# DTolm/VkResample

Measured on AMD Instinct MI355X. Metric: frames/s, 2048x1024->4096x2048 fp32 FFT upscale (R2C+zero-pad+C2R+sharpen), higher is better.
Workload: dtype f32; 1 GPU; 2048x1024->4096x2048 -u 2 -p 0, 1024 frames/step/GPU, ring of 8 resident planar fp32 frames/GPU; preset=config2, kernels=tuned, streams=3, device=AMD Radeon Graphics, wisdom=built-in only (private cache dir)

## Files before the change

vkresample_amd/csrc/fftup_info.hip:

```cpp
#include <hip/hip_runtime.h>

#include <cstdio>
#include <cstring>
#include <string>

#include "plan.hpp"

static thread_local std::string g_last_error;

int fail(int code, const std::string& msg)
{
    g_last_error = msg;
    return code;
}

static const char* device_label(const hipDeviceProp_t& prop) { return prop.name[0] ? prop.name : prop.gcnArchName; }

extern "C" {

int fftup_device_count(void)
{
    int n = 0;
    if (hipGetDeviceCount(&n) != hipSuccess) return 0;
    return n;
}

int fftup_device_name(int device, char* buf, size_t buflen)
{
    if (!buf || buflen == 0) return fail(FFTUP_E_INVALID_ARG, "null buffer");
    hipDeviceProp_t prop;
    if (device < 0 || device >= fftup_device_count()) return fail(FFTUP_E_NO_DEVICE, "bad device id");
    HIP_TRY(hipGetDeviceProperties(&prop, device));
    snprintf(buf, buflen, "%s", device_label(prop));
    return FFTUP_OK;
}

int fftup_device_pci_bus_id(int device, char* buf, size_t buflen)
{
    if (!buf || buflen < 16) return fail(FFTUP_E_INVALID_ARG, "buffer of at least 16 bytes needed");
    if (device < 0 || device >= fftup_device_count()) return fail(FFTUP_E_NO_DEVICE, "bad device id");
    HIP_TRY(hipDeviceGetPCIBusId(buf, (int)buflen, device));
    return FFTUP_OK;
}

int fftup_plan_describe(const fftup_plan* P, char* buf, size_t buflen)
{
    if (!P || !buf || !buflen) return fail(FFTUP_E_INVALID_ARG, "null argument");
    std::string s;
    using Family = fftup_plan::Family;
    const std::string half = P->half ? ", half storage" : "", tiles = std::to_string(P->TK);
    const std::string resampled = " (size-generic kernels, " + std::to_string(P->ncols) + " spectrum columns, LDS ping-pong, run-time radix lists, column tiles of " + tiles + ")" + half;
    const std::string rows_cols = ", rows " + std::to_string(P->W) + "->" + std::to_string(P->uW) + ", columns " + std::to_string(P->H) + "->" + std::to_string(P->uH);
    switch (P->family) {
    case Family::dct:
        s = std::string(P->down ? "downscale: dct: size-generic DCT-II / truncate / DCT-III kernels" : "dct: size-generic DCT-II / zero-pad / DCT-III kernels")
            + " (LDS ping-pong, run-time radix lists, column tiles of " + tiles + " column pairs)" + half;
        break;
    case Family::view: {
        char t[320];
        snprintf(t, sizeof t, "view%s: chirp-z resampling, rows %u->%u origin %.17g span %.17g (kmax %d, L=%u), columns %u->%u origin %.17g span %.17g (kmax %d, L=%u)",
                 P->mirror ? ", mirror (even reflection, period 2N)" : "", P->W, P->uW, P->vw.origin_x, P->vw.span_x, P->vx.kmax, P->vx.L, P->H, P->uH, P->vw.origin_y, P->vw.span_y, P->vy.kmax, P->vy.L);
        s = t + resampled;
        break;
    }
    case Family::odd:
        if (P->exact) s = "exact size: exact trigonometric resampling" + rows_cols + (P->align == FFTUP_ALIGN_CENTRE ? ", pixel centres aligned" : ", pixel 0 on pixel 0") + resampled;
        else s = std::string(P->down ? "downscale: " : "") + "odd sizes: exact trigonometric resampling" + rows_cols + resampled;
        break;
    case Family::down:
        s = "downscale: size-generic kernels, spectrum cropped to " + std::to_string(P->ncols) + " columns at the row stage (LDS ping-pong, "
            "run-time radix lists, column tiles of " + tiles + ")" + half;
        break;
    case Family::mixed_jit: s = "specialised at plan time: " + fftup_jit::describe(P->jit->choice); break;
    case Family::tuned:
        s = "ahead-of-time power-of-two kernels (radix 8, 8 points per thread; fused C2R+sharpen " + std::string(P->fused ? "on" : "off") + ")"
            + "; column kernel with digit-swap exchanges";
        break;
    case Family::mixed_aot:
        s = std::string("ahead-of-time mixed-radix kernels: ") + (P->mixed == 1 ? "row 15*8*16, col 9*10*12, fused 16*16*15" : "row 5*16*16, col 9*8*10, fused 16*16*10");
        break;
    case Family::cplx: s = "size-generic kernels, non-R2C path (full complex transforms)"; break;
    case Family::generic: case Family::f64:
        s = std::string("size-generic kernels (") + ((P->inplaceF || P->inplaceI || P->inplaceC) ? "in place in one LDS buffer" : "LDS ping-pong") + ", run-time radix lists"
            + (P->poly ? ", polyphase column pass)" : ")")
            + (P->dbl ? ", double" : "");
        break;
    }
    auto four = [&](const char* what, const fftup_plan::Four& f) {
        if (f.on) s += std::string("; ") + what + " in four steps " + std::to_string(f.n1) + "*" + std::to_string(f.n2) + " (tiles of " + std::to_string(f.tka) + " / " + std::to_string(f.tkb) + ")";
    };
    four("forward rows", P->fourF); four("inverse rows", P->fourI); four("forward columns", P->colF); four("inverse columns", P->colI);
    if (P->bz && P->family == Family::view) {
        if (P->bzW.L) s += "; forward rows bluestein L=" + std::to_string(P->bzW.L);
        if (P->bzH.L) s += "; forward columns bluestein L=" + std::to_string(P->bzH.L);
    }
    else if (P->bz) {
        auto axis = [&](const char* what, uint32_t n, uint32_t un, const BzPlan& f, const BzPlan& i) {
            if (!f.L && !i.L) return;
            s += std::string("; ") + what + " " + std::to_string(n) + "->" + std::to_string(un) + " bluestein L=" + (f.L ? std::to_string(f.L) : std::string("-")) + "/"
                 + (i.L ? std::to_string(i.L) : std::string("-"));
        };
        axis("rows", P->W, P->uW, P->bzW, P->bzUW);
        axis("columns", P->H, P->uH, P->bzH, P->bzUH);
        s += "; column tiles of " + std::to_string(P->TK);
    }
    if (P->u8out) s += "; fused 8-bit RGB store";
    snprintf(buf, buflen, "%s", s.c_str());
    return FFTUP_OK;
}

int fftup_plan_info(const fftup_plan* P, fftup_info* info)
{
    if (!P || !info) return fail(FFTUP_E_INVALID_ARG, "null argument");
    memset(info, 0, sizeof *info);
    info->out_width = P->uW;
    info->out_height = P->uH;
    info->num_kernels = P->fused ? 3 : 4;
    info->tuned = P->mixed == 3 ? 2 : ((P->tuned || P->mixed) ? 1 : 0);
    const double C = 3.0, W = P->W, H = P->H, uW = P->uW, uH = P->uH;
    const bool fused_u8 = fuse_u8(P);
    const double b_in = fused_u8 ? 1.0 : (double)P->esz;
    const double b_r = (double)P->esz, b_out = P->u8out ? 1.0 : b_r, b_c = (double)P->csz;
    const double in = C * W * H * b_in;
    const double S1 = C * P->ncols * H * b_c;
    const double S2 = C * P->ncols * uH * b_c;
    const double R = C * uW * uH * (P->cplx ? b_c : b_r);
    const double o = C * uW * uH * b_out;
    info->alg_bytes_per_frame = in + 2 * S1 + 2 * S2 + 2 * R + o;
    info->kernel_alg_bytes[0] = in + S1;
    info->kernel_alg_bytes[1] = S1 + S2;
    info->kernel_alg_bytes[2] = P->fused ? S2 + 2 * R + o : S2 + R;
    info->kernel_alg_bytes[3] = P->fused ? 0.0 : R + o;
    {
        const bool poly = (P->tuned || P->mixed) && P->U >= 2;
        const double S2w = poly ? S1 * (P->U - 1) : S2;
        const double halo = P->fused ? (double)(P->pairs_per_strip + 1) / P->pairs_per_strip : 1.0;
        info->kernel_min_bytes[0] = in + S1;
        info->kernel_min_bytes[1] = S1 + S2w;
        info->kernel_min_bytes[2] = P->fused ? S2 * halo + o : S2 + R;
        info->kernel_min_bytes[3] = P->fused ? 0.0 : R + o;
    }
    if (P->dct) {
        const double D1 = C * W * H * 4.0, D2 = C * W * uH * 4.0;
        info->alg_bytes_per_frame = in + 2 * D1 + 2 * D2 + 2 * R + o;
        const double k[FFTUP_NUM_KERNELS] = {in + D1, D1 + D2, D2 + R, R + o};
        for (int i = 0; i < FFTUP_NUM_KERNELS; i++) info->kernel_alg_bytes[i] = info->kernel_min_bytes[i] = k[i];
    }
    info->device_bytes = P->device_bytes;
    info->abi_version = FFTUP_ABI_VERSION;
    info->u8_store = P->u8out ? 1 : 0;
    snprintf(info->device_name, sizeof info->device_name, "%s", device_label(P->prop));
    const bool crop_rows = P->exact ? P->uW < P->W : P->down, crop_cols = P->exact ? P->uH < P->H : P->down;
    const bool is_dct = P->family == fftup_plan::Family::dct, is_cplx = P->family == fftup_plan::Family::cplx;
    snprintf(info->kernel_names[0], 64, is_dct ? "dct_row" : crop_rows ? "row_r2c_crop" : is_cplx ? "row_c2c" : "row_r2c");
    snprintf(info->kernel_names[1], 64, is_dct ? (P->down ? "dct_col_crop_idct" : "dct_col_pad_idct") : crop_cols ? "col_fwd_crop_inv" : "col_fwd_pad_inv");
    snprintf(info->kernel_names[2], 64, is_dct ? "idct_row" : P->fused ? "row_c2r_sharpen" : (is_cplx ? "row_c2c_inv" : "row_c2r"));
    snprintf(info->kernel_names[3], 64, P->fused ? "-" : "sharpen");
    if (P->family == fftup_plan::Family::odd)
        for (int i = 0; i < 3; i++) strncat(info->kernel_names[i], "_odd", 63 - strlen(info->kernel_names[i]));
    if (P->family == fftup_plan::Family::view) {
        snprintf(info->kernel_names[0], 64, P->mirror ? "row_r2c_mirror" : "row_r2c_odd");
        snprintf(info->kernel_names[1], 64, P->mirror ? "col_view_mirror" : "col_view");
        snprintf(info->kernel_names[2], 64, P->mirror ? "row_view_c2r_mirror" : "row_view_c2r");
    }
    const bool kbz[3] = {P->bzW.L != 0, P->bzH.L != 0 || P->bzUH.L != 0, P->bzUW.L != 0};
    for (int i = 0; i < (P->family == fftup_plan::Family::view ? 2 : 3); i++)
        if (kbz[i]) strncat(info->kernel_names[i], "_bz", 63 - strlen(info->kernel_names[i]));
    return FFTUP_OK;
}

const char* fftup_strerror(int code)
{
    switch (code) {
    case FFTUP_OK: return "success";
    case FFTUP_E_INVALID_ARG: return "invalid argument";
    case FFTUP_E_UNSUPPORTED_SIZE: return "unsupported size (not 2,3,5,7-smooth)";
    case FFTUP_E_UNSUPPORTED_PRECISION: return "unsupported precision";
    case FFTUP_E_NO_DEVICE: return "no usable HIP device";
    case FFTUP_E_HIP: return "HIP runtime error";
    case FFTUP_E_OUT_OF_MEMORY: return "out of device memory";
    case FFTUP_E_NO_INPUT: return "no input uploaded / nothing executed";
    case FFTUP_E_INCOMPLETE: return "incomplete (image not found)";
    case FFTUP_E_WOULD_BLOCK: return "the call would wait for the calling thread itself";
    case FFTUP_E_OVERFLOW: return "an internal buffer bound was exceeded";
    default: return "unknown error";
    }
}

const char* fftup_last_error(void) { return g_last_error.c_str(); }
const char* fftup_version(void) { return "fftup 0.7.0 (gfx950, ABI 2)"; }

}
```

vkresample_amd/csrc/fftup_launch.hip:

```cpp
#include <hip/hip_runtime.h>

#include <algorithm>
#include <cmath>
#include <cstdio>
#include <cstdlib>
#include <cstring>
#include <string>
#include <type_traits>
#include <vector>

#include "plan.hpp"
#include "kernels_generic.hpp"
#include "kernels_pow2.hpp"
#include "kernels_mixed.hpp"
#include "kernels_dswap.hpp"
#include "kernels_dct.hpp"
#include "kernels_downscale.hpp"
#include "kernels_bluestein.hpp"
#include "kernels_odd.hpp"
#include "kernels_view.hpp"
#include "kernels_mirror.hpp"
#include "kernels_view_tables.hpp"
#include "kernels_path.hpp"
#include "kernels_device_io.hpp"
#include "mirror_tables.hpp"

using namespace fftup;
using Family = fftup_plan::Family;

int kernels_generic_max_threads(bool dbl) { return dbl ? GenericMaxThreads<double2>::value : GenericMaxThreads<float2>::value; }
int kernels_aot_mixed_plan(uint32_t W, uint32_t H)
{
    if (W == MixedCfg1080::W && H == MixedCfg1080::H) return 1;
    if (W == MixedCfg720::W && H == MixedCfg720::H) return 2;
    return 0;
}
size_t kernels_tuned_col_lds(uint32_t H) { return sizeof(float2) * (size_t)lswz_size((int)H * TUNED_TK); }

struct ViewTables { int kmax; const float2 *pre, *post, *bhat; };
struct Frame { hipStream_t st; float2 *S1, *S2; void *R, *T4; const void* in; long in_row, in_plane; int kind; void* out;
               int ncols, NT; float upsq; ViewTables vx, vy; };
static Frame resolve(const fftup_plan* P, const FrameRun& r)
{
    const fftup_plan::Lane& l = P->lanes[r.lane];
    Frame f{l.stream, l.S1, l.S2, l.R, l.T4, P->in_planar[r.in_slot], (long)P->W, (long)P->in_plane_stride, P->in_kind[r.in_slot], r.out,
            P->ncols, P->NT, P->upsq, {P->vx.kmax, P->vx.pre, P->vx.post, P->vx.bhat}, {P->vy.kmax, P->vy.pre, P->vy.post, P->vy.bhat}};
    if (r.in) { f.in = r.in->in; f.in_row = r.in->in_row; f.in_plane = r.in->kind == 2 ? 0 : r.in->in_plane; f.kind = r.in->kind; }
    else if (f.kind == 2) { f.in = P->in_u8[r.in_slot]; f.in_row = 3l * P->W; f.in_plane = 0; }
    return f;
}
template <class Q> static void set_in(const Frame& f, Q& q) { q.in = f.in; q.in_row_stride = f.in_row; q.in_plane_stride = f.in_plane; }
static bool runs(Pass pass, Pass k) { return pass == Pass::all || pass == k; }

template <class... A> struct Kern { void (*fn)(A...); unsigned block; size_t lds; };
template <class... A> static Kern<A...> kern(void (*fn)(A...), int block, size_t lds) { return {fn, (unsigned)block, lds}; }
template <class T> struct type_c { using type = T; };
template <class... A> static void launch(const Kern<A...>& k, dim3 grid, hipStream_t st, const typename type_c<A>::type&... a)
{
    void* args[] = {const_cast<void*>((const void*)&a)...};
    (void)hipLaunchKernel((const void*)k.fn, grid, dim3(k.block), args, k.lds, st);
}
template <typename C> struct FourKerns { Kern<Row4Params<C>> a, b; };

template <int MAX = 8, class F> static auto with_tile(int tk, F&& f)
{
    if constexpr (MAX > 1) {
        if (tk == MAX) return f(std::integral_constant<int, MAX>{});
        return with_tile<MAX / 2>(tk, f);
    }
    else return f(std::integral_constant<int, 1>{});
}
template <class F> static auto with_flag(bool b, F&& f) { return b ? f(std::true_type{}) : f(std::false_type{}); }
template <class F> static auto with_mode(bool half, int kind, F&& f)
{
    if (kind == 2) return half ? f(std::integral_constant<int, IN_U8_F16>{}) : f(std::integral_constant<int, IN_U8_F32>{});
    return half ? f(std::integral_constant<int, IN_F16>{}) : f(std::integral_constant<int, IN_F32>{});
}
template <class F> static auto with_mixed_cfg(const fftup_plan* P, F&& f) { return P->mixed == 1 ? f(type_c<MixedCfg1080>{}) : f(type_c<MixedCfg720>{}); }

static Kern<RowR2CParams> generic_row_kernel(const fftup_plan* P, int kind)
{
    return with_mode(P->half, kind, [&](auto m) { return kern(k_row_r2c<m()>, P->thrW, P->ldsRowF); });
}
template <class F> static auto generic_c2r_kernel(const fftup_plan* P, F&& f)
{
    return with_flag(P->half, [&](auto h) {
        if (P->bzUW.L) return f(kern(k_row_c2r_bz<h()>, P->thrUW, P->ldsRowI), P->bzUW);
        return f(kern(k_row_c2r<h()>, P->thrUW, P->ldsRowI));
    });
}
template <typename C> static Kern<ColParamsT<C>> col_kernel(const fftup_plan* P)
{
    return with_tile(P->TK, [&](auto tk) {
        if (P->poly) return kern(k_col_poly<tk(), C>, P->thrCol, P->ldsCol);
        if constexpr (sizeof(scalar_t<C>) == 8) {
            if (P->inplaceC) return kern(k_col<tk(), C, true>, P->thrCol, P->ldsCol);
        }
        return kern(k_col<tk(), C, false>, P->thrCol, P->ldsCol);
    });
}
template <typename C, class F> static auto columns_kernel(const fftup_plan* P, F&& f)
{
    if constexpr (sizeof(scalar_t<C>) == 4) {
        if (P->bzH.L || P->bzUH.L) return with_tile(P->TK, [&](auto tk) { return f(kern(k_col_bz<tk()>, P->thrCol, P->ldsCol), P->bzH, P->bzUH); });
    }
    return f(col_kernel<C>(P));
}
static Kern<RowR2CParamsT<double2>> f64_row_kernel(const fftup_plan* P)
{
    return with_flag(P->inplaceF, [&](auto ip) { return kern(k_row_r2c<IN_F64, double2, ip()>, P->thrW, P->ldsRowF); });
}
static Kern<RowC2RParamsT<double2>> f64_c2r_kernel(const fftup_plan* P)
{
    return with_flag(P->inplaceI, [&](auto ip) { return kern(k_row_c2r<false, double2, ip()>, P->thrUW, P->ldsRowI); });
}
template <typename C> static Kern<RowR2CParamsT<C>> c2c_fwd_kernel(const fftup_plan* P, int kind)
{
    if constexpr (sizeof(scalar_t<C>) == 8) return kern(k_row_c2c_fwd<IN_F64, C, false>, P->thrW, P->ldsRowF);
    else return with_mode(P->half, kind, [&](auto m) {
        if (P->inplaceF) return kern(k_row_c2c_fwd<m(), C, true>, 1024, P->ldsRowF);
        return kern(k_row_c2c_fwd<m(), C, false>, P->thrW, P->ldsRowF);
    });
}
template <typename C> static Kern<RowC2RParamsT<C>> c2c_inv_kernel(const fftup_plan* P)
{
    if constexpr (sizeof(scalar_t<C>) == 8) return kern(k_row_c2c_inv<C, false, false>, P->thrUW, P->ldsRowI);
    else return with_flag(P->half, [&](auto h) {
        if (P->inplaceI) return kern(k_row_c2c_inv<C, h(), true>, 1024, P->ldsRowI);
        return kern(k_row_c2c_inv<C, h(), false>, P->thrUW, P->ldsRowI);
    });
}
template <typename C, int DIR, int MODE, int OUT> static FourKerns<C> four_kernels(const fftup_plan::Four& f)
{
    return {with_tile<16>(f.tka, [&](auto t) { return kern(k_row4_a<DIR, t(), MODE, C>, f.thrA, f.ldsA); }),
            with_tile<16>(f.tkb, [&](auto t) { return kern(k_row4_b<DIR, t(), OUT, C>, f.thrB, f.ldsB); })};
}
template <typename C> static FourKerns<C> four_fwd_kernels(const fftup_plan* P, int kind)
{
    if constexpr (sizeof(scalar_t<C>) == 8) return four_kernels<C, +1, IN_F64, OUT4_TILES>(P->fourF);
    else return with_mode(P->half, kind, [&](auto m) { return four_kernels<C, +1, m(), OUT4_TILES>(P->fourF); });
}
template <typename C> static FourKerns<C> four_inv_kernels(const fftup_plan* P)
{
    if constexpr (sizeof(scalar_t<C>) == 4) {
        if (P->half) return four_kernels<C, -1, IN4_TILES, OUT4_HALF>(P->fourI);
    }
    return four_kernels<C, -1, IN4_TILES, OUT4_DENSE>(P->fourI);
}
template <typename C> static FourKerns<C> four_col_kernels(const fftup_plan* P, bool inverse)
{
    return inverse ? four_kernels<C, -1, IN4_DENSE_SHIFT, OUT4_DENSE>(P->colI) : four_kernels<C, +1, IN4_DENSE, OUT4_DENSE>(P->colF);
}
static Kern<DctRowParams> dct_row_kernel(const fftup_plan* P, int kind)
{
    return with_mode(P->half, kind, [&](auto m) { return kern(k_dct_row<m()>, P->thrW, P->ldsRowF); });
}
static Kern<DctColParams> dct_col_kernel(const fftup_plan* P) { return with_tile(P->TK, [&](auto tk) { return kern(k_dct_col<tk()>, P->thrCol, P->ldsCol); }); }
static Kern<IdctRowParams> idct_row_kernel(const fftup_plan* P) { return with_flag(P->half, [&](auto h) { return kern(k_idct_row<h()>, P->thrUW, P->ldsRowI); }); }
static Kern<DownRowParams> crop_row_kernel(const fftup_plan* P, int kind)
{
    return with_flag(P->bzW.L != 0, [&](auto bz) { return with_mode(P->half, kind, [&](auto m) { return kern(k_row_r2c_crop<m(), bz()>, P->thrW, P->ldsRowF); }); });
}
static Kern<DownColParams> crop_col_kernel(const fftup_plan* P)
{
    return with_flag(P->bzH.L || P->bzUH.L, [&](auto bz) { return with_tile(P->TK, [&](auto tk) { return kern(k_col_crop<tk(), bz()>, P->thrCol, P->ldsCol); }); });
}
static Kern<OddRowParams> odd_row_kernel(const fftup_plan* P, int kind)
{
    return with_mode(P->half, kind, [&](auto m) { return kern(k_row_r2c_odd<m()>, P->thrW, P->ldsRowF); });
}
static Kern<OddColParams> odd_col_kernel(const fftup_plan* P) { return with_tile(P->TK, [&](auto tk) { return kern(k_col_odd<tk()>, P->thrCol, P->ldsCol); }); }
static Kern<OddC2RParams> odd_c2r_kernel(const fftup_plan* P) { return with_flag(P->half, [&](auto h) { return kern(k_row_c2r_odd<h()>, P->thrUW, P->ldsRowI); }); }
static bool resampling_rows(const fftup_plan* P) { return P->family == Family::generic && P->bzW.L != 0; }
static Kern<ViewColParams> view_col_kernel(const fftup_plan* P) { return with_tile(P->TK, [&](auto tk) { return kern(k_col_view<tk()>, P->thrCol, P->ldsCol); }); }
static Kern<ViewC2RParams> view_c2r_kernel(const fftup_plan* P) { return with_flag(P->half, [&](auto h) { return kern(k_row_view_c2r<h()>, P->thrUW, P->ldsRowI); }); }
static Kern<MirrorRowParams> mirror_row_kernel(const fftup_plan* P, int kind)
{
    return with_mode(P->half, kind, [&](auto m) { return kern(k_row_r2c_mirror<m()>, P->thrW, P->ldsRowF); });
}
static Kern<MirrorColParams> mirror_col_kernel(const fftup_plan* P) { return with_tile(P->TK, [&](auto tk) { return kern(k_col_view_mirror<tk()>, P->thrCol, P->ldsCol); }); }
static Kern<MirrorC2RParams> mirror_c2r_kernel(const fftup_plan* P) { return with_flag(P->half, [&](auto h) { return kern(k_row_view_c2r_mirror<h()>, P->thrUW, P->ldsRowI); }); }
static Kern<RowR2CTParams> tuned_row_kernel(const fftup_plan* P, int kind)
{
    return with_mode(P->half, kind, [&](auto m) {
        switch (P->W) {
        case 512: return kern(k_row_r2c_t<512, m(), TUNED_TK>, 512 / 8, 0);
        case 1024: return kern(k_row_r2c_t<1024, m(), TUNED_TK>, 1024 / 8, 0);
        default: return kern(k_row_r2c_t<2048, m(), TUNED_TK>, 2048 / 8, 0);
        }
    });
}
static Kern<ColTParams> tuned_col_kernel(const fftup_plan* P)
{
    switch (P->H) {
    case 256: return kern(k_col_v<TUNED_TK, 256>, 128, 8192);
    case 512: return kern(k_col_v<TUNED_TK, 512>, 256, 16384);
    default: return kern(k_col_v<TUNED_TK, 1024>, 512, 32768);
    }
}
static Kern<RowC2RTParams> tuned_c2r_kernel(const fftup_plan* P)
{
    return with_flag(P->half, [&](auto h) {
        switch (P->uW) {
        case 1024: return kern(k_row_c2r_t<1024, h(), TUNED_TK, true>, 1024 / 8, 0);
        case 2048: return kern(k_row_c2r_t<2048, h(), TUNED_TK, true>, 2048 / 8, 0);
        default: return kern(k_row_c2r_t<4096, h(), TUNED_TK, true>, 4096 / 8, 0);
        }
    });
}
static Kern<RowR2CTParams> mixed_row_kernel(const fftup_plan* P, int kind)
{
    return with_mixed_cfg(P, [&](auto c) {
        using CFG = typename decltype(c)::type;
        return with_mode(P->half, kind, [&](auto m) { return kern(k_row_r2c_m<CFG, m()>, CFG::ROW_T, 0); });
    });
}
static Kern<ColTParams> mixed_col_kernel(const fftup_plan* P)
{
    return with_mixed_cfg(P, [&](auto c) { using CFG = typename decltype(c)::type; return kern(k_col_m<CFG>, 4 * CFG::COL_TPC, P->ldsCol); });
}
static Kern<RowC2RParams> mixed_c2r_kernel(const fftup_plan* P)
{
    return with_mixed_cfg(P, [&](auto c) {
        using CT = typename decltype(c)::type::CT;
        return with_flag(P->half, [&](auto h) { return kern(k_row_c2r_ct<CT, h()>, CT::T, P->ldsRowI); });
    });
}
template <class PL> static Kern<FusedParams> fused_kernel_of(const fftup_plan* P)
{
    return with_flag(P->half, [&](auto h) {
        if (P->u8out) return kern(k_c2r_sharpen_g<PL, h(), TUNED_TK, 2, 4, true>, PL::T, FusedGLds<PL>::TOTAL);
        return kern(k_c2r_sharpen_g<PL, h(), TUNED_TK>, PL::T, FusedGLds<PL>::TOTAL);
    });
}
static Kern<FusedParams> fused_kernel(const fftup_plan* P)
{
    if (P->family == Family::mixed_aot) return with_mixed_cfg(P, [&](auto c) { return fused_kernel_of<typename decltype(c)::type::FUSED>(P); });
    switch (P->uW) {
    case 1024: return fused_kernel_of<FusedPlanPow2<1024>>(P);
    case 2048: return fused_kernel_of<FusedPlanPow2<2048>>(P);
    default: return fused_kernel_of<FusedPlanPow2<4096>>(P);
    }
}

struct AllowLds {
    hipError_t err = hipSuccess;
    template <class... A, class... X> void operator()(const Kern<A...>& k, const X&...)
    {
        if (err == hipSuccess) err = hipFuncSetAttribute((const void*)k.fn, hipFuncAttributeMaxDynamicSharedMemorySize, (int)k.lds);
    }
    template <typename C> void operator()(const FourKerns<C>& k) { (*this)(k.a); (*this)(k.b); }
};
template <typename C> static void allow_columns(const fftup_plan* P, AllowLds& allow)
{
    if (P->colF.on) { allow(four_col_kernels<C>(P, false)); allow(four_col_kernels<C>(P, true)); }
    else columns_kernel<C>(P, allow);
}
template <typename C> static void allow_cplx(const fftup_plan* P, AllowLds& allow)
{
    for (int kind : {1, 2}) { if (P->fourF.on) allow(four_fwd_kernels<C>(P, kind)); else allow(c2c_fwd_kernel<C>(P, kind)); }
    allow_columns<C>(P, allow);
    if (P->fourI.on) allow(four_inv_kernels<C>(P)); else allow(c2c_inv_kernel<C>(P));
}
int kernels_set_attributes(fftup_plan* P)
{
    AllowLds allow;
    switch (P->family) {
    case Family::generic:
        for (int kind : {1, 2}) { if (resampling_rows(P)) allow(odd_row_kernel(P, kind)); else allow(generic_row_kernel(P, kind)); }
        allow_columns<float2>(P, allow);
        generic_c2r_kernel(P, allow);
        break;
    case Family::f64: allow(f64_row_kernel(P)); allow_columns<double2>(P, allow); allow(f64_c2r_kernel(P)); break;
    case Family::cplx: if (P->dbl) allow_cplx<double2>(P, allow); else allow_cplx<float2>(P, allow); break;
    case Family::dct: for (int kind : {1, 2}) allow(dct_row_kernel(P, kind)); allow(dct_col_kernel(P)); allow(idct_row_kernel(P)); break;
    case Family::down: for (int kind : {1, 2}) allow(crop_row_kernel(P, kind)); allow(crop_col_kernel(P)); generic_c2r_kernel(P, allow); break;
    case Family::odd: for (int kind : {1, 2}) allow(odd_row_kernel(P, kind)); allow(odd_col_kernel(P)); allow(odd_c2r_kernel(P)); break;
    case Family::view:
        if (P->mirror) { for (int kind : {1, 2}) allow(mirror_row_kernel(P, kind)); allow(mirror_col_kernel(P)); allow(mirror_c2r_kernel(P)); }
        else { for (int kind : {1, 2}) allow(odd_row_kernel(P, kind)); allow(view_col_kernel(P)); allow(view_c2r_kernel(P)); }
        break;
    case Family::tuned: allow(tuned_col_kernel(P)); allow(fused_kernel(P)); break;
    case Family::mixed_aot: allow(mixed_col_kernel(P)); allow(mixed_c2r_kernel(P)); allow(fused_kernel(P)); break;
    case Family::mixed_jit:
        if (P->jit->choice.row_kind == 2) for (int kind : {1, 2}) allow(generic_row_kernel(P, kind));
        break;
    }
    if (allow.err != hipSuccess) return fail(FFTUP_E_HIP, std::string("hipFuncSetAttribute(hipFuncAttributeMaxDynamicSharedMemorySize): ") + hipGetErrorString(allow.err));
    return FFTUP_OK;
}

void launch_unpack_from(fftup_plan* P, const uint8_t* rgb, size_t row_stride_bytes, void* planes, hipStream_t st)
{
    dim3 grid((P->W + 255) / 256, P->H);
    if (P->dbl)
        hipLaunchKernelGGL(k_unpack_u8_f64, grid, dim3(256), 0, st, rgb, (long)row_stride_bytes, (double*)planes,
                           (int)P->W, (int)P->H, (long)P->in_plane_stride);
    else if (P->half)
        hipLaunchKernelGGL(k_unpack_u8<true>, grid, dim3(256), 0, st, rgb, (long)row_stride_bytes, planes,
                           (int)P->W, (int)P->H, (long)P->in_plane_stride);
    else
        hipLaunchKernelGGL(k_unpack_u8<false>, grid, dim3(256), 0, st, rgb, (long)row_stride_bytes, planes,
                           (int)P->W, (int)P->H, (long)P->in_plane_stride);
}
void launch_unpack(fftup_plan* P, uint32_t slot, hipStream_t st) { launch_unpack_from(P, P->in_u8[slot], (size_t)3 * P->W, P->in_planar[slot], st); }

void launch_pack(fftup_plan* P, uint32_t slot, uint8_t* dst, hipStream_t st)
{
    dim3 grid(P->dbl ? (P->uW + 255) / 256 : (P->uW + 1023) / 1024, P->uH);
    const int wrap = (P->cfg.flags & FFTUP_FLAG_U8_WRAP) ? 1 : 0;
    if (P->dbl) hipLaunchKernelGGL(k_pack_u8_f64, grid, dim3(256), 0, st, (const double*)P->out[slot], dst, (int)P->uW, (int)P->uH, wrap);
    else if (P->half) hipLaunchKernelGGL(k_pack_u8<true>, grid, dim3(256), 0, st, P->out[slot], dst, (int)P->uW, (int)P->uH, wrap);
    else hipLaunchKernelGGL(k_pack_u8<false>, grid, dim3(256), 0, st, P->out[slot], dst, (int)P->uW, (int)P->uH, wrap);
}

void launch_pack_to(fftup_plan* P, const void* planes, uint8_t* rgb, size_t row_stride_bytes, hipStream_t st)
{
    dim3 grid(P->dbl ? (P->uW + 255) / 256 : (P->uW + 1023) / 1024, P->uH);
    const int wrap = (P->cfg.flags & FFTUP_FLAG_U8_WRAP) ? 1 : 0;
    if (P->dbl) hipLaunchKernelGGL(k_pack_u8_f64_strided, grid, dim3(256), 0, st, (const double*)planes, rgb, (long)row_stride_bytes, (int)P->uW, (int)P->uH, wrap);
    else if (P->half) hipLaunchKernelGGL(k_pack_u8_strided<true>, grid, dim3(256), 0, st, planes, rgb, (long)row_stride_bytes, (int)P->uW, (int)P->uH, wrap);
    else hipLaunchKernelGGL(k_pack_u8_strided<false>, grid, dim3(256), 0, st, planes, rgb, (long)row_stride_bytes, (int)P->uW, (int)P->uH, wrap);
}

void launch_copy_rows(const void* src, size_t src_row, size_t src_plane, void* dst, size_t dst_row, size_t dst_plane,
                      size_t row_bytes, uint32_t rows, uint32_t planes, int gran, hipStream_t st)
{
    CopyRowsParams p{};
    p.src = (const uint8_t*)src; p.dst = (uint8_t*)dst; p.src_row = (long)src_row; p.src_plane = (long)src_plane;
    p.dst_row = (long)dst_row; p.dst_plane = (long)dst_plane; p.row_bytes = (long)row_bytes;
    const dim3 grid((unsigned)((row_bytes / 16 + 2 + 255) / 256), rows, planes);
    switch (gran) {
    case 8: hipLaunchKernelGGL(k_copy_rows<8>, grid, dim3(256), 0, st, p); break;
    case 4: hipLaunchKernelGGL(k_copy_rows<4>, grid, dim3(256), 0, st, p); break;
    case 2: hipLaunchKernelGGL(k_copy_rows<2>, grid, dim3(256), 0, st, p); break;
    default: hipLaunchKernelGGL(k_copy_rows<1>, grid, dim3(256), 0, st, p); break;
    }
}

static unsigned pass_planes()
{
    const char* e = fftup_jit::experiment("planes");
    return e ? (unsigned)std::max(1, std::min(3, atoi(e))) : 3u;
}

static unsigned fused_grid(const fftup_plan* P, int pairs_per_strip)
{
    const int ppp = (int)P->uH / 2;
    if (P->u8out) return (unsigned)(((ppp + pairs_per_strip - 1) / pairs_per_strip + 7) / 8 * 24);
    return (unsigned)((3 * ppp + pairs_per_strip - 1) / pairs_per_strip);
}
static FusedParams fused_params(const fftup_plan* P, const Frame& f)
{
    FusedParams p{};
    p.S1 = f.S1; p.odd_delta = (unsigned)(f.S2 - f.S1);
    if (P->U == 1) { p.S1 = f.S2; p.odd_delta = 0; }
    p.out = f.out; p.tw = P->twUW; p.uH = (int)P->uH; p.NT = P->NT;
    p.pairs_per_strip = P->pairs_per_strip; p.upsq = P->upsq; p.coef = P->coef;
    p.u8_wrap = (P->cfg.flags & FFTUP_FLAG_U8_WRAP) ? 1 : 0;
    return p;
}

static bool fast_sharpen_ok(const fftup_plan* P) { return !P->dbl && P->uW % 256 == 0 && P->uH % 16 == 0; }

static void launch_sharpen_fast(const fftup_plan* P, const Frame& f)
{
    SharpenTParams p{};
    p.R = f.R; p.out = f.out; p.uW = (int)P->uW; p.uH = (int)P->uH; p.upsq = f.upsq; p.coef = P->coef;
    dim3 grid(P->uW / 256, P->uH / 16, 3), block(64, 4);
    if (P->half) hipLaunchKernelGGL((k_sharpen_t<true, 4>), grid, block, 0, f.st, p);
    else hipLaunchKernelGGL((k_sharpen_t<false, 4>), grid, block, 0, f.st, p);
}

static void launch_sharpen(const fftup_plan* P, const Frame& f)
{
    if (fast_sharpen_ok(P)) { launch_sharpen_fast(P, f); return; }
    SharpenParams p{};
    p.R = f.R; p.out = f.out; p.uW = (int)P->uW; p.uH = (int)P->uH; p.upsq = f.upsq; p.coef = P->coef;
    dim3 grid((P->uW + 1023) / 1024, P->uH, 3), block(256);
    if (P->half) hipLaunchKernelGGL(k_sharpen<true>, grid, block, 0, f.st, p);
    else hipLaunchKernelGGL(k_sharpen<false>, grid, block, 0, f.st, p);
}

static int frame_status(hipError_t jit = hipSuccess)
{
    hipError_t e = hipGetLastError();
    if (e == hipSuccess) e = jit;
    if (e != hipSuccess) return fail(FFTUP_E_HIP, std::string("kernel launch: ") + hipGetErrorString(e));
    return FFTUP_OK;
}

template <class Rows, class Cols, class Inv>
static int launch_four_passes(const fftup_plan* P, const Frame& f, Pass pass, Rows rows, Cols cols, Inv inv)
{
    if (runs(pass, Pass::rows)) rows(P, f);
    if (runs(pass, Pass::columns)) cols(P, f);
    if (runs(pass, Pass::inverse)) inv(P, f);
    if (runs(pass, Pass::sharpen)) launch_sharpen(P, f);
    return frame_status();
}

static void dct_rows(const fftup_plan* P, const Frame& f)
{
    DctRowParams p{};
    p.S1 = (float*)f.S1; p.tw = P->twW; p.rot = P->rotW; p.plan = P->planW; p.W = (int)P->W; p.H = (int)P->H;
    set_in(f, p);
    launch(dct_row_kernel(P, f.kind), dim3(P->H / 2, 3), f.st, p);
}
static void dct_cols(const fftup_plan* P, const Frame& f)
{
    DctColParams p{};
    p.S1 = (const float*)f.S1; p.S2 = (float*)f.S2;
    p.twH = P->twH; p.twUH = P->twUH; p.rotH = P->rotH; p.rotUH = P->rotUH; p.planH = P->planH; p.planUH = P->planUH;
    p.W = (int)P->W; p.H = (int)P->H; p.uH = (int)P->uH; p.inv_norm = (float)(1.0 / (double)P->H);
    launch(dct_col_kernel(P), dim3((P->W / 2 + P->TK - 1) / P->TK, 3), f.st, p);
}
static void dct_inv(const fftup_plan* P, const Frame& f)
{
    IdctRowParams p{};
    p.S2 = (const float*)f.S2; p.R = f.R; p.tw = P->twUW; p.rot = P->rotUW; p.plan = P->planUW;
    p.W = (int)P->W; p.uW = (int)P->uW; p.uH = (int)P->uH;
    p.inv_norm = (float)(1.0 / ((double)P->W * (double)P->upsq));
    launch(idct_row_kernel(P), dim3(P->uH / 2, 3), f.st, p);
}

static void down_rows(const fftup_plan* P, const Frame& f)
{
    DownRowParams p{};
    p.S1 = f.S1; p.tw = P->twW; p.plan = P->planW; p.W = (int)P->W; p.H = (int)P->H;
    p.TK = P->TK; p.NT = P->NT; p.h = (int)P->uW / 2; p.bz = P->bzW;
    set_in(f, p);
    launch(crop_row_kernel(P, f.kind), dim3(P->H / 2, 3), f.st, p);
}
static void down_cols(const fftup_plan* P, const Frame& f)
{
// ... 45 lines not shown
    CztPlan z{};
    z.L = (int32_t)a.L; z.K = 2 * t.kmax + 1; z.M = (int32_t)M; z.plan = a.planL; z.tw = a.tw; z.pre = t.pre; z.post = t.post; z.bhat = t.bhat;
    return z;
}
static void view_cols(const fftup_plan* P, const Frame& f)
{
    ViewColParams p{};
    p.S1 = f.S1; p.S2 = f.S2; p.twH = P->twH; p.planH = P->planH;
    p.H = (int)P->H; p.uH = (int)P->uH; p.NT = f.NT; p.ncols = f.ncols; p.kmax = f.vy.kmax; p.bzH = P->bzH; p.z = czt_plan(P->vy, f.vy, P->uH);
    launch(view_col_kernel(P), dim3(f.NT, 3), f.st, p);
}
static void view_inv(const fftup_plan* P, const Frame& f)
{
    ViewC2RParams p{};
    p.S2 = f.S2; p.R = f.R; p.uW = (int)P->uW; p.uH = (int)P->uH;
    p.TK = P->TK; p.NT = f.NT; p.kmax = f.vx.kmax; p.z = czt_plan(P->vx, f.vx, P->uW);
    launch(view_c2r_kernel(P), dim3((P->uH + 1) / 2, 3), f.st, p);
}

static void mirror_rows(const fftup_plan* P, const Frame& f)
{
    MirrorRowParams p{};
    p.S1 = f.S1; p.tw = P->twW; p.plan = P->planW; p.W = (int)P->W; p.H = (int)P->H;
    p.TK = P->TK; p.NT = f.NT; p.ncols = f.ncols; p.bz = P->bzW;
    set_in(f, p);
    launch(mirror_row_kernel(P, f.kind), dim3((P->H + 1) / 2, 3), f.st, p);
}
static void mirror_cols(const fftup_plan* P, const Frame& f)
{
    MirrorColParams p{};
    p.S1 = f.S1; p.S2 = f.S2; p.twH = P->twH; p.planH = P->planH;
    p.H = (int)P->H; p.uH = (int)P->uH; p.NT = f.NT; p.ncols = f.ncols; p.kmax = f.vy.kmax; p.bzH = P->bzH; p.z = czt_plan(P->vy, f.vy, P->uH);
    p.rot = P->rotH;
    launch(mirror_col_kernel(P), dim3(f.NT, 3), f.st, p);
}
static void mirror_inv(const fftup_plan* P, const Frame& f)
{
    MirrorC2RParams p{};
    p.S2 = f.S2; p.R = f.R; p.W = (int)P->W; p.uW = (int)P->uW; p.uH = (int)P->uH;
    p.TK = P->TK; p.NT = f.NT; p.kmax = f.vx.kmax; p.z = czt_plan(P->vx, f.vx, P->uW); p.rot = P->rotW;
    launch(mirror_c2r_kernel(P), dim3((P->uH + 1) / 2, 3), f.st, p);
}

template <typename C> static void launch_four(const FourKerns<C>& k, const fftup_plan::Four& f, const Row4Params<C>& q, int rows, hipStream_t st)
{
    launch(k.a, dim3(rows, f.n2 / f.tka, 3), st, q);
    launch(k.b, dim3(rows, f.n1 / f.tkb, 3), st, q);
}
template <typename C> static void launch_columns(const fftup_plan* P, const Frame& f)
{
    using S = scalar_t<C>;
    if (!P->colF.on) {
        ColParamsT<C> p{};
        p.S1 = (const C*)f.S1; p.S2 = (C*)f.S2; p.twH = (const C*)P->twH; p.twUH = (const C*)P->twUH;
        p.planH = P->planH; p.planUH = P->planUH;
        p.W = (int)P->W; p.H = (int)P->H; p.uH = (int)P->uH; p.NT = P->NT; p.ncols = P->ncols; p.zly = P->zly; p.zry = P->zry;
        p.inv_norm = (S)(1.0 / (double)P->uH);
        columns_kernel<C>(P, [&](auto k, const auto&... z) { launch(k, dim3(P->NT, 3), f.st, p, z...); });
        return;
    }
    Row4Params<C> q{};
    const fftup_plan::Four &s = P->colF, &g = P->colI;
    q.spec = (const C*)f.S1; q.T = (C*)f.T4; q.R = f.S1;
    q.tw1 = (const C*)P->colFtw.tw1; q.tw2 = (const C*)P->colFtw.tw2; q.twN = (const C*)P->twH; q.plan1 = s.p1; q.plan2 = s.p2;
    q.N = (int)P->H; q.N1 = s.n1; q.N2 = s.n2; q.rows = P->ncols; q.W = (int)P->H; q.TK = 1; q.NT = P->ncols; q.inv_norm = (S)1;
    launch_four(four_col_kernels<C>(P, false), s, q, P->ncols, f.st);
    q.R = f.S2; q.tw1 = (const C*)P->colItw.tw1; q.tw2 = (const C*)P->colItw.tw2; q.twN = (const C*)P->twUH; q.plan1 = g.p1; q.plan2 = g.p2;
    q.N = (int)P->uH; q.N1 = g.n1; q.N2 = g.n2; q.zlx = P->zly; q.zrx = P->zry; q.inv_norm = (S)(1.0 / (double)P->uH);
    launch_four(four_col_kernels<C>(P, true), g, q, P->ncols, f.st);
}

static int launch_frame_f64(const fftup_plan* P, const Frame& f, Pass pass)
{
    if (runs(pass, Pass::rows)) {
        RowR2CParamsT<double2> p{};
        p.S1 = (double2*)f.S1; p.tw = (const double2*)P->twW; p.plan = P->planW; p.W = (int)P->W; p.H = (int)P->H;
        p.TK = P->TK; p.NT = P->NT;
        set_in(f, p);
        launch(f64_row_kernel(P), dim3(P->H / 2, 3), f.st, p);
    }
    if (runs(pass, Pass::columns)) launch_columns<double2>(P, f);
    if (runs(pass, Pass::inverse)) {
        RowC2RParamsT<double2> p{};
        p.S1 = (const double2*)f.S1; p.S2 = (const double2*)f.S2; p.R = f.R; p.tw = (const double2*)P->twUW; p.plan = P->planUW;
        p.W = (int)P->W; p.uW = (int)P->uW; p.uH = (int)P->uH; p.TK = P->TK; p.NT = P->NT; p.zlx = P->zlx; p.zrx = P->zrx;
        p.inv_norm = 1.0 / (double)P->uW; p.poly = P->poly;
        launch(f64_c2r_kernel(P), dim3(P->uH / 2, 3), f.st, p);
    }
    if (runs(pass, Pass::sharpen)) {
        SharpenParams p{};
        p.R = f.R; p.out = f.out; p.uW = (int)P->uW; p.uH = (int)P->uH; p.upsq = P->upsq; p.coef = P->coef;
        const dim3 sgrid((P->uW + 511) / 512, (P->uH + SHARPEN_F64_RPT - 1) / SHARPEN_F64_RPT, 3);
        const char* ex = fftup_jit::experiment("f64_exact_sharpen");
        if (ex && atoi(ex)) {
            if (P->uW % 2 == 0) hipLaunchKernelGGL((k_sharpen_f64<true, true>), sgrid, dim3(64, 4), 0, f.st, p);
            else hipLaunchKernelGGL((k_sharpen_f64<false, true>), sgrid, dim3(64, 4), 0, f.st, p);
        }
        else if (P->uW % 2 == 0) hipLaunchKernelGGL(k_sharpen_f64<true>, sgrid, dim3(64, 4), 0, f.st, p);
        else hipLaunchKernelGGL(k_sharpen_f64<false>, sgrid, dim3(64, 4), 0, f.st, p);
    }
    return frame_status();
}

template <typename C> static int launch_frame_cplx(const fftup_plan* P, const Frame& f, Pass pass)
{
    using S = scalar_t<C>;
    if (runs(pass, Pass::rows) && P->fourF.on) {
        Row4Params<C> q{};
        const fftup_plan::Four& s = P->fourF;
        q.T = (C*)f.T4; q.S1 = (C*)f.S1; q.tw1 = (const C*)P->fourFtw.tw1; q.tw2 = (const C*)P->fourFtw.tw2; q.twN = (const C*)P->twW;
        q.plan1 = s.p1; q.plan2 = s.p2; q.N = (int)P->W; q.N1 = s.n1; q.N2 = s.n2; q.rows = (int)P->H; q.W = (int)P->W; q.TK = P->TK; q.NT = P->NT;
        set_in(f, q);
        launch_four(four_fwd_kernels<C>(P, f.kind), s, q, (int)P->H, f.st);
    } else if (runs(pass, Pass::rows)) {
        RowR2CParamsT<C> p{};
        p.S1 = (C*)f.S1; p.tw = (const C*)P->twW; p.plan = P->planW; p.W = (int)P->W; p.H = (int)P->H;
        p.TK = P->TK; p.NT = P->NT;
        set_in(f, p);
        launch(c2c_fwd_kernel<C>(P, f.kind), dim3(P->H, 3), f.st, p);
    }
    if (runs(pass, Pass::columns)) launch_columns<C>(P, f);
    if (runs(pass, Pass::inverse)) {
        if (P->fourI.on) {
            Row4Params<C> q{};
            const fftup_plan::Four& s = P->fourI;
            q.spec = (const C*)f.S2; q.T = (C*)f.T4; q.R = f.R;
            q.tw1 = (const C*)P->fourItw.tw1; q.tw2 = (const C*)P->fourItw.tw2; q.twN = (const C*)P->twUW; q.plan1 = s.p1; q.plan2 = s.p2;
            q.N = (int)P->uW; q.N1 = s.n1; q.N2 = s.n2; q.rows = (int)P->uH; q.W = (int)P->W; q.TK = P->TK; q.NT = P->NT; q.zlx = P->zlx; q.zrx = P->zrx;
            q.inv_norm = (S)(1.0 / (double)P->uW);
            launch_four(four_inv_kernels<C>(P), s, q, (int)P->uH, f.st);
        } else {
            RowC2RParamsT<C> p{};
            p.S2 = (const C*)f.S2; p.R = f.R; p.tw = (const C*)P->twUW; p.plan = P->planUW;
            p.W = (int)P->W; p.uW = (int)P->uW; p.uH = (int)P->uH; p.TK = P->TK; p.NT = P->NT; p.zlx = P->zlx; p.zrx = P->zrx;
            p.inv_norm = (S)(1.0 / (double)P->uW);
            launch(c2c_inv_kernel<C>(P), dim3(P->uH, 3), f.st, p);
        }
    }
    if (runs(pass, Pass::sharpen)) {
        SharpenParams p{};
        p.R = f.R; p.out = f.out; p.uW = (int)P->uW; p.uH = (int)P->uH; p.upsq = P->upsq; p.coef = P->coef;
        const dim3 grid((P->uW + 255) / 256, P->uH, 3);
        bool done = false;
        if constexpr (sizeof(S) == 4) {
            if (P->half) { hipLaunchKernelGGL((k_sharpen_c<C, true>), grid, dim3(256), 0, f.st, p); done = true; }
        }
        if (!done) hipLaunchKernelGGL((k_sharpen_c<C>), grid, dim3(256), 0, f.st, p);
    }
    return frame_status();
}

static int launch_frame_tuned(const fftup_plan* P, const Frame& f, Pass pass)
{
    if (runs(pass, Pass::rows)) {
        RowR2CTParams p{};
        p.S1 = f.S1; p.tw = P->twW; p.H = (int)P->H; p.NT = P->NT;
        set_in(f, p);
        launch(tuned_row_kernel(P, f.kind), dim3(P->H / 2, pass_planes()), f.st, p);
    }
    if (runs(pass, Pass::columns)) {
        ColTParams p{};
        p.S1 = f.S1; p.S2 = f.S2; p.twH = P->twH; p.twUH = P->twUH; p.W = (int)P->W; p.NT = P->NT;
        p.zly = P->zly; p.zry = P->zry;
        launch(tuned_col_kernel(P), dim3(P->NT, pass_planes()), f.st, p);
    }
    if (runs(pass, Pass::inverse) && P->fused) {
        const FusedParams p = fused_params(P, f);
        launch(fused_kernel(P), dim3(fused_grid(P, p.pairs_per_strip)), f.st, p);
    } else if (runs(pass, Pass::inverse) || pass == Pass::presharpen_tap) {
        RowC2RTParams p{};
        p.S1 = f.S1; p.S2 = f.S2; p.R = f.R; p.tw = P->twUW; p.uH = (int)P->uH; p.NT = P->NT;
        launch(tuned_c2r_kernel(P), dim3(P->uH / 2, 3), f.st, p);
    }
    if (runs(pass, Pass::sharpen) && !P->fused) launch_sharpen_fast(P, f);
    return frame_status();
}

static int launch_frame_generic(const fftup_plan* P, const Frame& f, Pass pass)
{
    const bool jit = P->family == Family::mixed_jit, aot = P->family == Family::mixed_aot;
    hipError_t jerr = hipSuccess;
    auto keep_first = [&](hipError_t e) { if (jerr == hipSuccess) jerr = e; };
    if (runs(pass, Pass::rows)) {
        const dim3 grid(P->H / 2, 3);
        if (resampling_rows(P)) odd_rows(P, f);
        else if (aot || (jit && P->jit->choice.row_kind != 2)) {
            RowR2CTParams q{};
            q.S1 = f.S1; q.tw = P->twW; q.H = (int)P->H; q.NT = P->NT;
            set_in(f, q);
            if (aot) launch(mixed_row_kernel(P, f.kind), grid, f.st, q);
            else keep_first(fftup_jit::launch(P->jit->fn[f.kind == 2 ? fftup_jit::K_ROW_U8 : fftup_jit::K_ROW_PLANAR], grid, dim3(P->jit->choice.row_block), 0, f.st, q));
        } else {
            RowR2CParams p{};
            p.S1 = f.S1; p.tw = P->twW; p.plan = P->planW; p.W = (int)P->W; p.H = (int)P->H;
            p.TK = P->TK; p.NT = P->NT;
            set_in(f, p);
            launch(generic_row_kernel(P, f.kind), grid, f.st, p);
        }
    }
    if (runs(pass, Pass::columns) && (jit || aot)) {
        ColTParams q{};
        q.S1 = f.S1; q.S2 = f.S2; q.twH = P->twH; q.twUH = P->twUH; q.W = (int)P->W; q.NT = P->NT;
        q.zly = P->zly; q.zry = P->zry;
        if (jit) {
            const auto& ch = P->jit->choice;
            const dim3 jgrid(P->NT * (ch.col_kind >= 3 ? 4 / ch.col_cols : 1), 3);
            keep_first(fftup_jit::launch(P->jit->fn[fftup_jit::K_COL], jgrid, dim3(ch.col_block), P->ldsCol, f.st, q));
        }
        else launch(mixed_col_kernel(P), dim3(P->NT, 3), f.st, q);
    }
    else if (runs(pass, Pass::columns)) launch_columns<float2>(P, f);
    if (runs(pass, Pass::inverse) && P->fused) {
        const FusedParams fp = fused_params(P, f);
        const dim3 grid(fused_grid(P, fp.pairs_per_strip));
        if (jit) keep_first(fftup_jit::launch(P->jit->fn[fftup_jit::K_FUSED], grid, dim3(P->jit->choice.fused_t), P->jit->choice.fused_lds, f.st, fp));
        else launch(fused_kernel(P), grid, f.st, fp);
    } else if (runs(pass, Pass::inverse) || pass == Pass::presharpen_tap) {
        RowC2RParams p{};
        p.S1 = f.S1; p.S2 = f.S2; p.R = f.R; p.tw = P->twUW; p.plan = P->planUW; p.W = (int)P->W; p.uW = (int)P->uW;
        p.uH = (int)P->uH; p.TK = P->TK; p.NT = P->NT; p.zlx = P->zlx; p.zrx = P->zrx;
        p.inv_norm = 1.0f / (float)P->uW; p.poly = P->poly && !P->mixed;
        const dim3 grid(P->uH / 2, 3);
        if (jit) {
            if (P->U == 1) p.S1 = p.S2;
            keep_first(fftup_jit::launch(P->jit->fn[fftup_jit::K_C2R_CT], grid, dim3(P->jit->choice.ct_t), P->ldsRowI, f.st, p));
        }
        else if (aot) launch(mixed_c2r_kernel(P), grid, f.st, p);
        else generic_c2r_kernel(P, [&](auto k, const auto&... z) { launch(k, grid, f.st, p, z...); });
    }
    if (runs(pass, Pass::sharpen) && !P->fused) launch_sharpen(P, f);
    return frame_status(jerr);
}

static int launch_family(const fftup_plan* P, const Frame& f, Pass pass)
{
    switch (P->family) {
    case Family::cplx: return P->dbl ? launch_frame_cplx<double2>(P, f, pass) : launch_frame_cplx<float2>(P, f, pass);
    case Family::f64: return launch_frame_f64(P, f, pass);
    case Family::dct: return launch_four_passes(P, f, pass, dct_rows, dct_cols, dct_inv);
    case Family::down: return launch_four_passes(P, f, pass, down_rows, down_cols, down_inv);
    case Family::odd: return launch_four_passes(P, f, pass, odd_rows, odd_cols, odd_inv);
    case Family::view:
        if (P->mirror) return launch_four_passes(P, f, pass, mirror_rows, mirror_cols, mirror_inv);
        return launch_four_passes(P, f, pass, odd_rows, view_cols, view_inv);
    case Family::tuned: return launch_frame_tuned(P, f, pass);
    case Family::generic: case Family::mixed_aot: case Family::mixed_jit: break;
    }
    return launch_frame_generic(P, f, pass);
}
static Kern<ViewTabParams> view_tables_kernel(const fftup_plan* P)
{
    return kern(k_view_tables, VT_THREADS, sizeof(double2) * (size_t)lpad_size((int)std::max(P->vx.L, P->vy.L)));
}
int kernels_allow_view_tables(const fftup_plan* P)
{
    for (uint32_t L : {P->vx.L, P->vy.L}) {
        if (L > (uint32_t)VT_MAX_L) return fail(FFTUP_E_UNSUPPORTED_SIZE, "k_view_tables: convolution length above " + std::to_string(VT_MAX_L));
        const StagePlan sp = make_stage_plan(L);
        for (int s = 0; s < sp.nstages; s++)
            if (!stage_fits_inplace((int)L, sp.radix[s], VT_THREADS, VT_PT)) return fail(FFTUP_E_UNSUPPORTED_SIZE, "k_view_tables: a stage does not fit its registers");
    }
    AllowLds allow;
    allow(view_tables_kernel(P));
    if (allow.err != hipSuccess) return fail(FFTUP_E_HIP, std::string("hipFuncSetAttribute(hipFuncAttributeMaxDynamicSharedMemorySize): ") + hipGetErrorString(allow.err));
    return FFTUP_OK;
}
static void frame_view(fftup_plan* P, int lane, const fftup_view& v, const fftup_shift* shift, Frame& f)
{
    fftup_plan::ViewTabs& t = P->vtabs[lane];
    struct Ax { const fftup_plan::ViewAxis* a; uint32_t N, M; double o, sp; ViewTables* out; };
    const Ax ax[2] = {{&P->vx, P->W, P->uW, v.origin_x, v.span_x, &f.vx}, {&P->vy, P->H, P->uH, v.origin_y, v.span_y, &f.vy}};
    ViewTabParams p{};
    for (int i = 0; i < 2; i++) {
        const Ax& x = ax[i];
        ViewTabAxis& q = p.ax[i];
        q.n = (int32_t)(P->mirror ? 2 * x.N : x.N); q.M = (int32_t)x.M; q.L = (int32_t)x.a->L;
        q.kmax = P->mirror ? fftup_viewtab::mirror_kmax_of(x.N, x.M, x.sp) : fftup_viewtab::kmax_of(x.N, x.M, x.sp);
        q.chirp = t.span[i] != x.sp;
        const fftup_viewphase::Pair o = fftup_viewphase::origin_of(x.o, (double)q.n, P->mirror);
        q.o_hi = o.hi; q.o_lo = o.lo; q.span = x.sp; q.plan = x.a->planL; q.tw = P->vroots[i];
        q.origin = x.o; q.mirror = P->mirror ? 1 : 0; q.shift = shift ? (i ? &shift->dy : &shift->dx) : nullptr;
        q.pre = t.pre[i]; q.post = t.post[i]; q.bhat = t.bhat[i];
        t.span[i] = x.sp; t.kmax[i] = q.kmax;
        *x.out = {q.kmax, q.pre, q.post, q.bhat};
    }
    t.built = true;
    f.ncols = P->mirror ? fftup_viewtab::mirror_ncols(P->W, f.vx.kmax) : f.vx.kmax + 1;
    f.NT = (f.ncols + P->TK - 1) / P->TK;
    const float u = view_factor(v, P->uW, P->uH);
    f.upsq = const_via_percent_f((double)(u * u), P->half);
    const char* ex = fftup_jit::experiment("view_tables_time");
    const bool timed = ex && atoi(ex) != 0;
    if (timed) (void)hipEventRecord(P->ev0, f.st);
    launch(view_tables_kernel(P), dim3(2), f.st, p);
    if (timed) {
        float ms = 0;
        (void)hipEventRecord(P->ev1, f.st);
        if (hipEventSynchronize(P->ev1) == hipSuccess && hipEventElapsedTime(&ms, P->ev0, P->ev1) == hipSuccess)
            fprintf(stderr, "fftup: k_view_tables %.3f us (chirp tables rebuilt: x %d, y %d)\n", (double)ms * 1e3, p.ax[0].chirp, p.ax[1].chirp);
    }
}

int launch_frame(fftup_plan* P, const FrameRun& r)
{
    Frame f = resolve(P, r);
    const bool tap = r.pass == Pass::presharpen_tap;
    if (f.kind == 0 && !tap) return fail(FFTUP_E_NO_INPUT, "no input uploaded for this slot");
    if (r.view) {
        if (P->family != Family::view || (size_t)r.lane >= P->vtabs.size() || !P->vtabs[r.lane].pre[0]) return fail(FFTUP_E_INVALID_ARG, "a frame with a view of its own: not a view plan, or its lane has no tables");
        frame_view(P, r.lane, *r.view, r.shift, f);
    }
    const int rc = launch_family(P, f, r.pass);
    if (rc && r.view) P->vtabs[r.lane].span[0] = P->vtabs[r.lane].span[1] = 0;
    if (tap || runs(r.pass, Pass::inverse)) { P->last_lane = r.lane; P->R_valid = !(P->fused && !tap); }
    return rc;
}

int launch_shift_path(const fftup_shift* in, fftup_shift* out, uint32_t n, uint32_t mode, float sigma, float min_peak, hipStream_t st)
{
    const Kern<ShiftPathParams> k = kern(k_shift_path, SP_THREADS, shift_path_lds((int)n, fftup_shiftpath::radius_of((double)sigma)));
    AllowLds allow;
    allow(k);
    if (allow.err != hipSuccess) return fail(FFTUP_E_HIP, std::string("hipFuncSetAttribute(hipFuncAttributeMaxDynamicSharedMemorySize): ") + hipGetErrorString(allow.err));
    launch(k, dim3(1), st, ShiftPathParams{(const float*)in, (float*)out, (int32_t)n, mode, sigma, min_peak});
    const hipError_t e = hipGetLastError();
    if (e != hipSuccess) return fail(FFTUP_E_HIP, std::string("fftup_shift_path: kernel launch: ") + hipGetErrorString(e));
    return FFTUP_OK;
}

__global__ void __launch_bounds__(256) k_checksum(const uint32_t* __restrict__ w, size_t n, unsigned long long* sum)
{
    unsigned long long acc = 0;
    for (size_t i = (size_t)blockIdx.x * 256 + threadIdx.x; i < n; i += (size_t)gridDim.x * 256) acc += w[i];
#pragma unroll
    for (int o = 32; o > 0; o >>= 1) acc += __shfl_down(acc, o);
    if ((threadIdx.x & 63) == 0) atomicAdd(sum, acc);
}

void launch_checksum(fftup_plan* P, uint32_t slot, hipStream_t st)
{
    const size_t nbytes = (size_t)3 * P->uW * P->uH * (P->u8out ? 1 : P->esz), nwords = nbytes / 4;
    hipLaunchKernelGGL(k_checksum, dim3(1024), dim3(256), 0, st, (const uint32_t*)P->out[slot], nwords, (unsigned long long*)P->d_sum);
    if (nbytes & 3)
        hipLaunchKernelGGL(k_checksum_tail, dim3(1), dim3(64), 0, st, (const uint8_t*)P->out[slot] + 4 * nwords, (int)(nbytes & 3), (unsigned long long*)P->d_sum);
}

#ifdef FFTUP_PLANE_STAMPS
extern "C" __attribute__((visibility("default"))) int fftup_debug_plane_stamps(unsigned long long* out)
{
    return out && hipMemcpyFromSymbol(out, HIP_SYMBOL(fftup::g_plane_stamps), sizeof(unsigned long long) * 3 * 2048 * 3) != hipSuccess;
}
#endif
```

vkresample_amd/csrc/fftup_plan.hip:

```cpp
#include <hip/hip_runtime.h>

#include <algorithm>
#include <cmath>
#include <complex>
#include <cstdio>
#include <cstdlib>
#include <cstring>
#include <memory>
#include <string>
#include <vector>

#include "plan.hpp"
#include "mirror_tables.hpp"
#include "view_tables.hpp"

using namespace fftup;

int dev_alloc(fftup_plan* P, void** ptr, size_t bytes)
{
    hipError_t e = hipMalloc(ptr, bytes);
    if (e != hipSuccess) {
        *ptr = nullptr;
        return fail(FFTUP_E_OUT_OF_MEMORY, std::string("hipMalloc(") + std::to_string(bytes) + "): " + hipGetErrorString(e));
    }
// ... 40 lines not shown
static int make_bluestein(fftup_plan* P, BzPlan* z, uint32_t n, uint32_t L)
{
    std::vector<std::complex<double>> w(n), b(L, std::complex<double>(0.0, 0.0));
    for (uint64_t k = 0; k < n; k++) w[k] = std::polar(1.0, M_PI * (double)((k * k) % (2 * (uint64_t)n)) / (double)n);
    for (uint32_t k = 0; k < n; k++) {
        b[k] = std::conj(w[k]);
        if (k) b[L - k] = std::conj(w[k]);
    }
    host_fft(b);
    std::vector<float2> hc(n), hb(L);
    for (uint32_t k = 0; k < n; k++) hc[k] = make_float2((float)w[k].real(), (float)w[k].imag());
    for (uint32_t k = 0; k < L; k++) hb[k] = make_float2((float)(b[k].real() / (double)L), (float)(b[k].imag() / (double)L));
    float2 *dc = nullptr, *db = nullptr, *dt = nullptr;
    if (int rc = upload_table(P, &dc, hc)) return rc;
    if (int rc = upload_table(P, &db, hb)) return rc;
    if (int rc = make_twiddles(P, &dt, L)) return rc;
    z->L = (int32_t)L; z->plan = make_stage_plan(L); z->tw = dt; z->chirp = dc; z->bhat = db;
    return FFTUP_OK;
}

static int make_phases(fftup_plan* P, float2** dptr, uint32_t N, uint32_t M)
{
    *dptr = nullptr;
    if (N == M) return FFTUP_OK;
    const uint32_t n = std::min(N, M) / 2 + 1;
    const int64_t period = 2 * (int64_t)M * (int64_t)N;
    std::vector<float2> h(n);
    for (uint32_t k = 0; k < n; k++) {
        int64_t r = ((int64_t)k * ((int64_t)N - (int64_t)M)) % period;
        if (r > period / 2) r -= period;
        if (r < -period / 2) r += period;
        const double a = -M_PI * (double)r / ((double)M * (double)N);
        h[k] = make_float2((float)std::cos(a), (float)std::sin(a));
    }
    return upload_table(P, dptr, h);
}


static int view_apply(fftup_plan* P, const fftup_view& v, bool first)
{
    struct Ax { fftup_plan::ViewAxis* a; uint32_t N, M; double o, sp, sp_old; };
    const Ax ax[2] = {{&P->vx, P->W, P->uW, v.origin_x, v.span_x, P->vw.span_x}, {&P->vy, P->H, P->uH, v.origin_y, v.span_y, P->vw.span_y}};
    for (const Ax& x : ax) {
        fftup_viewtab::AxisTables t;
        const bool chirp = first || x.sp != x.sp_old;
        if (P->mirror) fftup_viewtab::make_mirror_axis(x.N, x.M, x.o, x.sp, x.a->L, t, chirp);
        else fftup_viewtab::make_axis(x.N, x.M, x.o, x.sp, x.a->L, t, chirp);
        x.a->kmax = t.kmax;
        HIP_TRY(hipMemcpy(x.a->pre, t.pre.data(), sizeof(float) * t.pre.size(), hipMemcpyHostToDevice));
        if (chirp) {
            HIP_TRY(hipMemcpy(x.a->post, t.post.data(), sizeof(float) * t.post.size(), hipMemcpyHostToDevice));
            HIP_TRY(hipMemcpy(x.a->bhat, t.bhat.data(), sizeof(float) * t.bhat.size(), hipMemcpyHostToDevice));
        }
    }
    P->vw = v;
    P->ncols = P->mirror ? fftup_viewtab::mirror_ncols(P->W, P->vx.kmax) : P->vx.kmax + 1;
    P->NT = (P->ncols + P->TK - 1) / P->TK;
    P->cfg.upscale = view_factor(v, P->uW, P->uH);
    P->upsq = const_via_percent_f((double)(P->cfg.upscale * P->cfg.upscale), P->half);
    return FFTUP_OK;
}


int view_frames_prepare(fftup_plan* P, int nl)
{
    if (P->vtabs.empty()) P->vtabs.resize(P->nlanes);
    const uint32_t len[4] = {P->W, P->H, P->uW, P->uH};
    const fftup_plan::ViewAxis* const axes[2] = {&P->vx, &P->vy};
    if (!P->vroots[0]) {
        if (int rc = kernels_allow_view_tables(P)) return rc;
        for (int i = 0; i < 2; i++) {
            float2* d = nullptr;
            if (int rc = upload_table(P, &d, roots<double2>(axes[i]->L))) return rc;
            P->vroots[i] = (double2*)d;
        }
    }
    for (int l = 0; l < nl; l++) {
        fftup_plan::ViewTabs& t = P->vtabs[l];
        for (int i = 0; i < 2 && !t.bhat[1]; i++) {
            if (int rc = dev_alloc(P, (void**)&t.pre[i], sizeof(float2) * (2 * (size_t)(P->mirror ? len[i] : len[i] / 2) + 1))) return rc;
            if (int rc = dev_alloc(P, (void**)&t.post[i], sizeof(float2) * len[2 + i])) return rc;
            if (int rc = dev_alloc(P, (void**)&t.bhat[i], sizeof(float2) * axes[i]->L)) return rc;
        }
    }
    return FFTUP_OK;
}


static void tune_fused(fftup_plan* P);
static bool jit_tune_enabled()
{
    const char* e = fftup_jit::experiment("jit_tune");
    return e && atoi(e) != 0;
}

static int open_device(fftup_plan* P)
{
    HIP_TRY(hipSetDevice(P->device));
    HIP_TRY(hipGetDeviceProperties(&P->prop, P->device));
    HIP_TRY(hipStreamCreateWithFlags(&P->stream, hipStreamNonBlocking));
    HIP_TRY(hipEventCreate(&P->ev0));
    HIP_TRY(hipEventCreate(&P->ev1));
    return FFTUP_OK;
}

static fftup_jit::Module* specialise(const fftup_plan* P, const DeviceFacts& dev)
{
    int DD = 1;
    const int D = plan_jit_factor(*P, &DD);
    fftup_jit::Choice ch;
    if (!D || !fftup_jit::choose((int)P->W, (int)P->H, D, P->half, stage_radices(P->planUW), ch, wisdom_device_key(*P, dev), true, DD)) return nullptr;
    ch.u8out = (P->cfg.flags & FFTUP_FLAG_FUSE_U8_STORE) != 0;
    std::string jerr;
    fftup_jit::Module* m = fftup_jit::load(ch, dev.arch, jerr);
    if (!m && getenv("FFTUP_JIT_VERBOSE")) fprintf(stderr, "fftup: run-time specialisation failed, size-generic kernels in use: %s\n", jerr.c_str());
    return m;
}

static int make_tables(fftup_plan* P)
{
    const uint32_t len[4] = {P->W, P->H, P->uW, P->uH};
    float2** const tw[4] = {&P->twW, &P->twH, &P->twUW, &P->twUH};
    for (int i = 0; i < 4; i++)
        if (int rc = make_twiddles(P, tw[i], len[i])) return rc;
    const std::pair<const fftup_plan::Four*, fftup_plan::FourTables*> fours[4] = {{&P->fourF, &P->fourFtw}, {&P->fourI, &P->fourItw}, {&P->colF, &P->colFtw}, {&P->colI, &P->colItw}};
    for (auto& f : fours) {
        if (!f.first->on) continue;
        if (int rc = make_twiddles(P, &f.second->tw1, (uint32_t)f.first->n1)) return rc;
        if (int rc = make_twiddles(P, &f.second->tw2, (uint32_t)f.first->n2)) return rc;
    }
    BzPlan* const bz[4] = {&P->bzW, &P->bzH, &P->bzUW, &P->bzUH};
    for (int i = 0; i < 4; i++)
        if (P->bzL[i])
            if (int rc = make_bluestein(P, bz[i], len[i], P->bzL[i])) return rc;
    if (P->exact && P->align == FFTUP_ALIGN_CENTRE) {
        if (int rc = make_phases(P, &P->phW, P->W, P->uW)) return rc;
        if (int rc = make_phases(P, &P->phH, P->H, P->uH)) return rc;
    }
    if (P->view) {
        fftup_plan::ViewAxis* const axes[2] = {&P->vx, &P->vy};
        for (int i = 0; i < 2; i++) {
            fftup_plan::ViewAxis& a = *axes[i];
            a.L = P->viewL[i]; a.planL = make_stage_plan(a.L);
            if (int rc = make_twiddles(P, &a.tw, a.L)) return rc;
            if (int rc = dev_alloc(P, (void**)&a.pre, sizeof(float2) * (2 * (size_t)(P->mirror ? len[i] : len[i] / 2) + 1))) return rc;
            if (int rc = dev_alloc(P, (void**)&a.post, sizeof(float2) * len[2 + i])) return rc;
            if (int rc = dev_alloc(P, (void**)&a.bhat, sizeof(float2) * a.L)) return rc;
        }
    }
    if (P->mirror) {
        if (int rc = make_rotations(P, &P->rotW, P->W)) return rc;
        if (int rc = make_rotations(P, &P->rotH, P->H)) return rc;
    }
    if (P->dct) {
        float2** const rot[4] = {&P->rotW, &P->rotH, &P->rotUW, &P->rotUH};
        for (int i = 0; i < 4; i++)
            if (int rc = make_rotations(P, rot[i], len[i])) return rc;
    }
    return FFTUP_OK;
}

static int alloc_spectra(fftup_plan* P, float2** s1, float2** s2)
{
    const size_t s1_elems = (size_t)3 * P->NT * P->H * P->TK;
    if ((P->tuned || P->mixed) && P->U >= 2) {
        int r = dev_alloc(P, (void**)s1, P->csz * (size_t)P->U * s1_elems);
        *s2 = r ? nullptr : *s1 + s1_elems;
        return r;
    }
    int r = dev_alloc(P, (void**)s1, P->csz * s1_elems);
    return r ? r : dev_alloc(P, (void**)s2, P->csz * 3 * (size_t)P->NT * P->uH * P->TK);
}

static int make_buffers(fftup_plan* P)
{
    const size_t esz = P->esz, out_pixels = (size_t)3 * P->uW * P->uH;
    P->in_plane_stride = (size_t)(P->W + 2) * P->H;
    P->in_planar.assign(P->ring, nullptr);
    P->in_u8.assign(P->ring, nullptr);
    P->in_kind.assign(P->ring, 0);
    P->out.assign(P->ring, nullptr);
    for (uint32_t s = 0; s < P->ring; s++) {
        if (int rc = dev_alloc(P, &P->in_planar[s], 3 * P->in_plane_stride * esz)) return rc;
        if (int rc = dev_alloc(P, (void**)&P->in_u8[s], (size_t)3 * P->W * P->H)) return rc;
        if (int rc = dev_alloc(P, &P->out[s], out_pixels * (P->u8out ? 1 : esz) + 8)) return rc;
    }
    P->r_bytes = out_pixels * (P->cplx ? (P->half ? 4 : P->csz) : esz);
    if (!P->u8out)
        if (int rc = dev_alloc(P, (void**)&P->out_u8, out_pixels + 8)) return rc;
    return FFTUP_OK;
}

static int make_lanes(fftup_plan* P)
{
    P->nlanes = lane_count();
    P->lanes.resize(P->nlanes);
    const size_t t4_bytes = P->csz * 3 * std::max(std::max(P->fourF.on ? (size_t)P->W * P->H : 0, P->fourI.on ? (size_t)P->uW * P->uH : 0),
                                                  P->colI.on ? (size_t)P->ncols * P->uH : 0);
    for (int l = 0; l < P->nlanes; l++) {
        fftup_plan::Lane& lane = P->lanes[l];
        if (l == 0) lane.stream = P->stream;
        else HIP_TRY(hipStreamCreateWithFlags(&lane.stream, hipStreamNonBlocking));
        HIP_TRY(hipEventCreateWithFlags(&lane.done, hipEventDisableTiming));
        if (int rc = alloc_spectra(P, &lane.S1, &lane.S2)) return rc;
        if (!P->fused)
            if (int rc = dev_alloc(P, &lane.R, P->r_bytes)) return rc;
        if (t4_bytes)
            if (int rc = dev_alloc(P, &lane.T4, t4_bytes)) return rc;
    }
    return FFTUP_OK;
}

struct PlanDestroyer { void operator()(fftup_plan* P) const { fftup_plan_destroy(P); } };

static int plan_create(fftup_plan** out, const PlanRequest& rq)
{
    if (!out || !rq.cfg) return fail(FFTUP_E_INVALID_ARG, "null argument");
    *out = nullptr;
    PlanGeometry G;
    if (int rc = plan_check(rq, G)) return rc;
    const int ndev = fftup_device_count();
    if (ndev <= 0) return fail(FFTUP_E_NO_DEVICE, "no HIP device available (this library has no CPU path)");
    if (G.cfg.device < 0 || G.cfg.device >= ndev) return fail(FFTUP_E_NO_DEVICE, "device id out of range");

    std::unique_ptr<fftup_plan, PlanDestroyer> owner(new fftup_plan());
    fftup_plan* const P = owner.get();
    static_cast<PlanGeometry&>(*P) = G;
    P->device = G.cfg.device;
    if (int rc = open_device(P)) return rc;
    const DeviceFacts dev = device_facts(P->prop);
    if (int rc = plan_geometry_columns(*P, dev)) return rc;
    P->jit = specialise(P, dev);
    if (int rc = plan_geometry_finish(*P, dev, P->jit ? &P->jit->choice : nullptr)) return rc;
    if (int rc = make_tables(P)) return rc;
    if (int rc = make_buffers(P)) return rc;
    if (int rc = make_lanes(P)) return rc;
    if (rq.view)
        if (int rc = view_apply(P, *rq.view, true)) return rc;
    if (int rc = kernels_set_attributes(P)) return rc;
    if (P->mixed == 3 && ((P->cfg.flags & FFTUP_FLAG_TUNE_PLAN) || jit_tune_enabled())) tune_fused(P);
    png_geometry(P);
    *out = owner.release();
    return FFTUP_OK;
}

extern "C" {

int fftup_plan_create(fftup_plan** out, const fftup_config* cfg) { return plan_create(out, {cfg, nullptr, 0, nullptr}); }

int fftup_plan_create_size(fftup_plan** out, const fftup_config* cfg, uint32_t out_width, uint32_t out_height, uint32_t align)
{
    const uint32_t size[2] = {out_width, out_height};
    return plan_create(out, {cfg, size, align, nullptr});
}

int fftup_plan_create_view(fftup_plan** out, const fftup_config* cfg, uint32_t out_width, uint32_t out_height, const fftup_view* view)
{
    if (out) *out = nullptr;
    if (!out || !cfg || !view) return fail(FFTUP_E_INVALID_ARG, "null argument");
    const uint32_t size[2] = {out_width, out_height};
    return plan_create(out, {cfg, size, FFTUP_ALIGN_CORNER, view});
}

int fftup_plan_set_view(fftup_plan* P, const fftup_view* view)
{
    if (!P || !view) return fail(FFTUP_E_INVALID_ARG, "null argument");
    if (!P->view) return fail(FFTUP_E_INVALID_ARG, "fftup_plan_set_view: not a view plan (fftup_plan_create_view makes one)");
    if (int rc = check_view("fftup_plan_set_view", view, P->uW, P->uH)) return rc;
    HIP_TRY(hipSetDevice(P->device));
    for (auto& lane : P->lanes) HIP_TRY(hipStreamSynchronize(lane.stream));
    return view_apply(P, *view, false);
}


int fftup_jit_check(uint32_t width, uint32_t height, float upscale, uint32_t precision, const char* arch, char* desc, size_t desclen)
{
    if (desc && desclen) desc[0] = 0;
    if (precision != 0 && precision != 2) return fail(FFTUP_E_UNSUPPORTED_PRECISION, "run-time specialised plans exist for -p 0 and -p 2");
    if (width < 2 || height < 2 || (width & 1) || (height & 1) || width > 65536 || height > 65536 || !is_smooth(width) || !is_smooth(height))
        return fail(FFTUP_E_UNSUPPORTED_SIZE, "sizes must be even and factor into 2,3,5,7");
    fftup_jit::Choice ch;
    if (!(upscale >= 1.0f && upscale <= 8.0f)) return fail(FFTUP_E_INVALID_ARG, "upscale out of range");
    const uint32_t uW = scaled_length(upscale, width), uH = scaled_length(upscale, height);
    int DD = 1, zly = 0, zry = 0;
    column_guard(upscale, uH, &zly, &zry);
    const int D = (uW & 1) || (uH & 1) || !is_smooth(uW) || !is_smooth(uH) || uW > 8192 ? 0 : jit_factor(upscale, width, height, uW, uH, zly, zry, &DD);
    if (!D || !fftup_jit::choose((int)width, (int)height, D, precision == 2, stage_radices(make_stage_plan(uW)), ch, "", true, DD))
        return fail(FFTUP_E_UNSUPPORTED_SIZE, "no specialised factorization for this size: the size-generic kernels run it");
    if (desc && desclen) snprintf(desc, desclen, "%s", fftup_jit::describe(ch).c_str());
    if (arch && !*arch) return FFTUP_OK;
    fftup_jit::Binary bin[2];
    std::string err;
    if (!fftup_jit::compile_both(ch, arch ? arch : "gfx950", bin, err)) return fail(FFTUP_E_HIP, err);
    return FFTUP_OK;
}

void fftup_plan_destroy(fftup_plan* P)
{
    if (!P) return;
    (void)hipSetDevice(P->device);
    if (P->stream) (void)hipStreamSynchronize(P->stream);
    for (size_t l = 0; l < P->lanes.size(); l++) {
        if (l && P->lanes[l].stream) { (void)hipStreamSynchronize(P->lanes[l].stream); (void)hipStreamDestroy(P->lanes[l].stream); }
        if (P->lanes[l].done) (void)hipEventDestroy(P->lanes[l].done);
    }
    for (auto& qs : P->q) {
        if (qs.done) (void)hipEventDestroy(qs.done);
        if (qs.png.copied) (void)hipEventDestroy(qs.png.copied);
        if (qs.png.meta_host) (void)hipHostFree(qs.png.meta_host);
        if (qs.png.parts_host) (void)hipHostFree(qs.png.parts_host);
    }
    if (P->png_copy) (void)hipStreamDestroy(P->png_copy);
    if (P->dio.start) (void)hipEventDestroy(P->dio.start);
    for (void* p : P->allocs) (void)hipFree(p);
    delete P->jit;
    if (P->ev0) (void)hipEventDestroy(P->ev0);
    if (P->ev1) (void)hipEventDestroy(P->ev1);
    if (P->stream) (void)hipStreamDestroy(P->stream);
    delete P;
}


}
static void tune_fused(fftup_plan* P)
{
    const DeviceFacts dev = device_facts(P->prop);
    const std::string& arch = dev.arch;
    const fftup_jit::Choice base = P->jit->choice;
    const std::string key = fftup_jit::fused_key(base, wisdom_device_key(*P, dev));
    std::string known;
    if (fftup_jit::experiment("jit_fused") || fftup_jit::wisdom_lookup(key, known)) return;
    const std::vector<int> kinds = P->in_kind;
    const int executed = P->executed;
    for (auto& k : P->in_kind) if (!k) k = 1;
    const uint32_t frames = 4 * (uint32_t)std::max(1, std::min(P->nlanes, (int)P->ring));
    auto time_plan = [&]() -> double {
        double best = 1e30, ms = 0;
        for (int rep = 0; rep < 3; rep++) {
            if (execute_ring_impl(P, frames, 0, &ms, nullptr, 1) != FFTUP_OK) return 1e30;
            if (rep > 0) best = std::min(best, ms / frames);
        }
        return best;
    };
    const double t_base = time_plan();
    if (t_base >= 1e30) {
        P->in_kind = kinds;
        P->executed = executed;
        return;
    }
    double t_best = t_base;
    fftup_jit::Module* const original = P->jit;
    fftup_jit::Module* best = nullptr;
    auto use = [&](fftup_jit::Module* m) { P->jit = m; P->pairs_per_strip = strip_length(*P, dev, m->choice.fused_t); };
    std::vector<fftup_jit::Choice> cands;
    {
        fftup_jit::Choice d;
        if (fftup_jit::choose(base.W, base.H, base.D, base.half, stage_radices(P->planUW), d, "", false, base.DD) &&
            fftup_jit::fused_value(d) != fftup_jit::fused_value(base)) {
            d.u8out = base.u8out;
            cands.push_back(d);
        }
// ... 27 lines not shown
```

vkresample_amd/csrc/kernels_dswap.hpp:

```cpp
#pragma once
#include "kernels_pow2.hpp"

namespace fftup {
__device__ __forceinline__ float2 cmul_tw_s(float2 z, float2 w)
{
    typedef float cf2 __attribute__((ext_vector_type(2)));
    const cf2 zv = {z.x, z.y}, wv = {w.x, w.y};
    cf2 t, r;
    asm("v_pk_mul_f32 %0, %1, %2 op_sel:[1,1] op_sel_hi:[1,0] neg_lo:[1,0]" : "=v"(t) : "v"(zv), "s"(wv));
    asm("v_pk_fma_f32 %0, %1, %2, %3 op_sel_hi:[0,1,1]" : "=v"(r) : "v"(zv), "s"(wv), "v"(t));
    return make_float2(r.x, r.y);
}

__device__ __forceinline__ void lane_transpose_hi3(float2 (&v)[8])
{
#define FFTUP_SWAP8(OP, A0, B0, A1, B1, A2, B2, A3, B3)                                                                         \
    asm volatile("s_nop 1\n\t" OP " %0, %1\n\t" OP " %2, %3\n\t" OP " %4, %5\n\t" OP " %6, %7\n\t" OP " %8, %9\n\t" OP         \
                 " %10, %11\n\t" OP " %12, %13\n\t" OP " %14, %15"                                                             \
                 : "+v"(v[A0].x), "+v"(v[B0].x), "+v"(v[A0].y), "+v"(v[B0].y), "+v"(v[A1].x), "+v"(v[B1].x), "+v"(v[A1].y),     \
                   "+v"(v[B1].y), "+v"(v[A2].x), "+v"(v[B2].x), "+v"(v[A2].y), "+v"(v[B2].y), "+v"(v[A3].x), "+v"(v[B3].x),     \
                   "+v"(v[A3].y), "+v"(v[B3].y))
    FFTUP_SWAP8("v_permlane32_swap_b32", 0, 4, 1, 5, 2, 6, 3, 7);
    FFTUP_SWAP8("v_permlane16_swap_b32", 0, 2, 1, 3, 4, 6, 5, 7);
#undef FFTUP_SWAP8
    float t0, t1, t2, t3, t4, t5, t6, t7;
    asm volatile(
        "s_nop 1\n\t"
        "v_mov_b32_dpp %16, %0 row_ror:8 row_mask:0xf bank_mask:0xf\n\t"
        "v_mov_b32_dpp %17, %2 row_ror:8 row_mask:0xf bank_mask:0xf\n\t"
        "v_mov_b32_dpp %18, %4 row_ror:8 row_mask:0xf bank_mask:0xf\n\t"
        "v_mov_b32_dpp %19, %6 row_ror:8 row_mask:0xf bank_mask:0xf\n\t"
        "v_mov_b32_dpp %20, %8 row_ror:8 row_mask:0xf bank_mask:0xf\n\t"
        "v_mov_b32_dpp %21, %10 row_ror:8 row_mask:0xf bank_mask:0xf\n\t"
        "v_mov_b32_dpp %22, %12 row_ror:8 row_mask:0xf bank_mask:0xf\n\t"
        "v_mov_b32_dpp %23, %14 row_ror:8 row_mask:0xf bank_mask:0xf\n\t"
        "v_mov_b32_dpp %0, %1 row_ror:8 row_mask:0xf bank_mask:0xc\n\t"
        "v_mov_b32_dpp %2, %3 row_ror:8 row_mask:0xf bank_mask:0xc\n\t"
        "v_mov_b32_dpp %4, %5 row_ror:8 row_mask:0xf bank_mask:0xc\n\t"
        "v_mov_b32_dpp %6, %7 row_ror:8 row_mask:0xf bank_mask:0xc\n\t"
        "v_mov_b32_dpp %8, %9 row_ror:8 row_mask:0xf bank_mask:0xc\n\t"
        "v_mov_b32_dpp %10, %11 row_ror:8 row_mask:0xf bank_mask:0xc\n\t"
        "v_mov_b32_dpp %12, %13 row_ror:8 row_mask:0xf bank_mask:0xc\n\t"
        "v_mov_b32_dpp %14, %15 row_ror:8 row_mask:0xf bank_mask:0xc\n\t"
        "v_mov_b32_dpp %1, %16 quad_perm:[0,1,2,3] row_mask:0xf bank_mask:0x3\n\t"
        "v_mov_b32_dpp %3, %17 quad_perm:[0,1,2,3] row_mask:0xf bank_mask:0x3\n\t"
        "v_mov_b32_dpp %5, %18 quad_perm:[0,1,2,3] row_mask:0xf bank_mask:0x3\n\t"
        "v_mov_b32_dpp %7, %19 quad_perm:[0,1,2,3] row_mask:0xf bank_mask:0x3\n\t"
        "v_mov_b32_dpp %9, %20 quad_perm:[0,1,2,3] row_mask:0xf bank_mask:0x3\n\t"
        "v_mov_b32_dpp %11, %21 quad_perm:[0,1,2,3] row_mask:0xf bank_mask:0x3\n\t"
        "v_mov_b32_dpp %13, %22 quad_perm:[0,1,2,3] row_mask:0xf bank_mask:0x3\n\t"
        "v_mov_b32_dpp %15, %23 quad_perm:[0,1,2,3] row_mask:0xf bank_mask:0x3"
        : "+v"(v[0].x), "+v"(v[1].x), "+v"(v[0].y), "+v"(v[1].y), "+v"(v[2].x), "+v"(v[3].x), "+v"(v[2].y), "+v"(v[3].y),
          "+v"(v[4].x), "+v"(v[5].x), "+v"(v[4].y), "+v"(v[5].y), "+v"(v[6].x), "+v"(v[7].x), "+v"(v[6].y), "+v"(v[7].y),
          "=&v"(t0), "=&v"(t1), "=&v"(t2), "=&v"(t3), "=&v"(t4), "=&v"(t5), "=&v"(t6), "=&v"(t7));
}

__device__ __forceinline__ void lane_swap_bit2(float2 (&v)[8])
{
    float t0, t1, t2, t3, t4, t5, t6, t7;
    asm volatile(
        "s_nop 1\n\t"
        "v_mov_b32 %16, %0\n\tv_mov_b32 %17, %2\n\tv_mov_b32 %18, %4\n\tv_mov_b32 %19, %6\n\t"
        "v_mov_b32 %20, %8\n\tv_mov_b32 %21, %10\n\tv_mov_b32 %22, %12\n\tv_mov_b32 %23, %14\n\t"
        "v_mov_b32_dpp %0, %1 row_shr:4 row_mask:0xf bank_mask:0xa\n\t"
        "v_mov_b32_dpp %2, %3 row_shr:4 row_mask:0xf bank_mask:0xa\n\t"
        "v_mov_b32_dpp %4, %5 row_shr:4 row_mask:0xf bank_mask:0xa\n\t"
        "v_mov_b32_dpp %6, %7 row_shr:4 row_mask:0xf bank_mask:0xa\n\t"
        "v_mov_b32_dpp %8, %9 row_shr:4 row_mask:0xf bank_mask:0xa\n\t"
        "v_mov_b32_dpp %10, %11 row_shr:4 row_mask:0xf bank_mask:0xa\n\t"
        "v_mov_b32_dpp %12, %13 row_shr:4 row_mask:0xf bank_mask:0xa\n\t"
        "v_mov_b32_dpp %14, %15 row_shr:4 row_mask:0xf bank_mask:0xa\n\t"
        "v_mov_b32_dpp %1, %16 row_shl:4 row_mask:0xf bank_mask:0x5\n\t"
        "v_mov_b32_dpp %3, %17 row_shl:4 row_mask:0xf bank_mask:0x5\n\t"
        "v_mov_b32_dpp %5, %18 row_shl:4 row_mask:0xf bank_mask:0x5\n\t"
        "v_mov_b32_dpp %7, %19 row_shl:4 row_mask:0xf bank_mask:0x5\n\t"
        "v_mov_b32_dpp %9, %20 row_shl:4 row_mask:0xf bank_mask:0x5\n\t"
        "v_mov_b32_dpp %11, %21 row_shl:4 row_mask:0xf bank_mask:0x5\n\t"
        "v_mov_b32_dpp %13, %22 row_shl:4 row_mask:0xf bank_mask:0x5\n\t"
        "v_mov_b32_dpp %15, %23 row_shl:4 row_mask:0xf bank_mask:0x5"
        : "+v"(v[0].x), "+v"(v[4].x), "+v"(v[0].y), "+v"(v[4].y), "+v"(v[1].x), "+v"(v[5].x), "+v"(v[1].y), "+v"(v[5].y),
          "+v"(v[2].x), "+v"(v[6].x), "+v"(v[2].y), "+v"(v[6].y), "+v"(v[3].x), "+v"(v[7].x), "+v"(v[3].y), "+v"(v[7].y),
          "=&v"(t0), "=&v"(t1), "=&v"(t2), "=&v"(t3), "=&v"(t4), "=&v"(t5), "=&v"(t6), "=&v"(t7));
}
__device__ __forceinline__ void wave_exchange(float2 (&v)[8], unsigned zbase, unsigned w, unsigned l)
{
    const unsigned aw = zbase + 8u * (w * 64u + l);
#pragma unroll
    for (int k = 0; k < 8; k++) { lds_f2raw r = {v[k].x, v[k].y}; *(lds_f2*)(size_t)(aw + 4096u * k) = r; }
    __syncthreads();
    const unsigned ar = zbase + 8u * (w * 512u + l);
#pragma unroll
    for (int m = 0; m < 8; m++) { const lds_f2raw r = *(const lds_f2*)(size_t)(ar + 512u * m); v[m] = make_float2(r.x, r.y); }
#pragma unroll
    for (int i = 0; i < 8; i += 2) asm volatile("" : "+v"(v[i].x), "+v"(v[i].y), "+v"(v[i + 1].x), "+v"(v[i + 1].y));
}

template <int WV, bool FWD>
__device__ __forceinline__ void wave_exchange_q(float2 (&v)[8], unsigned zbase, unsigned w, unsigned l)
{
    const unsigned a_k0 = zbase + 8u * (w * 64u + l);
    const unsigned a_m = zbase + 8u * (w * 512u + l);
#pragma unroll
    for (int k = 0; k < 8; k++) { lds_f2raw r = {v[k].x, v[k].y}; *(lds_f2*)(size_t)((FWD ? a_k0 + 512u * WV * k : a_m + 512u * k)) = r; }
    __syncthreads();
#pragma unroll
    for (int m = 0; m < 8; m++) { const lds_f2raw r = *(const lds_f2*)(size_t)((FWD ? a_m + 512u * m : a_k0 + 512u * WV * m)); v[m] = make_float2(r.x, r.y); }
#pragma unroll
    for (int i = 0; i < 8; i += 2) asm volatile("" : "+v"(v[i].x), "+v"(v[i].y), "+v"(v[i + 1].x), "+v"(v[i + 1].y));
}
template <int WV, int DIR> __device__ __forceinline__ void bfly_groups(float2 (&v)[8])
{
    if constexpr (WV == 8) bfly8_pk<DIR>(v);
    else if constexpr (WV == 4) {
#pragma unroll
        for (int b = 0; b < 2; b++) {
            pk2 a0 = {v[4 * b].x, v[4 * b].y}, a1 = {v[4 * b + 1].x, v[4 * b + 1].y}, a2 = {v[4 * b + 2].x, v[4 * b + 2].y}, a3 = {v[4 * b + 3].x, v[4 * b + 3].y};
            bfly4_pk<DIR>(a0, a1, a2, a3);
            v[4 * b] = make_float2(a0.x, a0.y); v[4 * b + 1] = make_float2(a1.x, a1.y);
            v[4 * b + 2] = make_float2(a2.x, a2.y); v[4 * b + 3] = make_float2(a3.x, a3.y);
        }
    } else {
#pragma unroll
        for (int b = 0; b < 4; b++) {
            const pk2 a = {v[2 * b].x, v[2 * b].y}, c = {v[2 * b + 1].x, v[2 * b + 1].y};
            const pk2 s0 = pk_add(a, c), s1 = pk_sub(a, c);
            v[2 * b] = make_float2(s0.x, s0.y); v[2 * b + 1] = make_float2(s1.x, s1.y);
        }
    }
}

template <int TK, int H = 1024>
__global__ void __launch_bounds__(H / 2, kColWaves) k_col_v(ColTParams p)
{
    static_assert(TK == 4, "four columns of H/8 threads: lane bits 0-1 = column, bits 2-5 and the wave = pp");
    static_assert(H == 1024 || H == 512 || H == 256, "8, 4 or 2 waves");
    constexpr int WV = H / 128, Q = 8 / WV, T = 64 * WV;
    extern __shared__ __attribute__((aligned(128))) char smem[];
    const unsigned zbase = lds_addr(smem);
    const int tid = threadIdx.x;
    const unsigned w = (unsigned)tid >> 6, l = (unsigned)tid & 63u;
    const int col = tid & 3, pp = tid >> 2;
    const int tile = blockIdx.x, c = blockIdx.y;
    const bool valid = tile * TK + col <= p.W / 2;
    const float2* src = p.S1 + ((long)c * p.NT + tile) * H * TK;
    const int wu = __builtin_amdgcn_readfirstlane((int)w);
    const int s1 = (int)(l >> 3), lb2 = (int)((l >> 2) & 1u), hh = (int)(l >> 2);
    const int kk = Q * wu + s1 / WV + 8 * (s1 % WV);
    const int kt = kk + 32 * WV * lb2;
    float2 v[8];
    stamp_begin(1, c);
#pragma unroll
    for (int i = 0; i < 8; i++) v[i] = valid ? src[tid + T * i] : make_float2(0.f, 0.f);
    float2 ta[Q][WV - 1];
#pragma unroll
    for (int b = 0; b < Q; b++)
#pragma unroll
        for (int m = 1; m < WV; m++) ta[b][m - 1] = p.twH[(16 * m * (Q * wu + b)) & (H - 1)];
    const float2 tb = p.twH[2 * kk], tc = p.twH[kt];
    const float2 tph = twid<-1>(p.twUH[kt]);
    bfly8_pk<+1>(v);
    if constexpr (WV == 8) wave_exchange(v, zbase, w, l);
    else wave_exchange_q<WV, true>(v, zbase, w, l);
#pragma unroll
    for (int b = 0; b < Q; b++)
#pragma unroll
        for (int m = 1; m < WV; m++) v[WV * b + m] = cmul_tw_s(v[WV * b + m], ta[b][m - 1]);
    bfly_groups<WV, +1>(v);
    lane_transpose_hi3(v);
    twiddle_powers<8>(v, tb);
    bfly8_pk<+1>(v);
    lane_swap_bit2(v);
    {
        v[4] = cmul_tw(v[4], tc);
        v[5] = cmul_tw(v[5], cmul_tw(tc, rot16<1>()));
        v[6] = cmul_tw(v[6], cmul_tw(tc, rot16<2>()));
        v[7] = cmul_tw(v[7], cmul_tw(tc, rot16<3>()));
#pragma unroll
        for (int r = 0; r < 4; r++) {
            const pk2 a = {v[r].x, v[r].y}, b = {v[r + 4].x, v[r + 4].y};
            const pk2 s0 = pk_add(a, b), s1_ = pk_sub(a, b);
            v[r] = make_float2(s0.x, s0.y); v[r + 4] = make_float2(s1_.x, s1_.y);
        }
    }
    {
        const float2 t1 = cmul_tw(tph, twid<-1>(rot32<1>())), t2 = cmul_tw(tph, twid<-1>(rot32<2>())), t3 = cmul_tw(tph, twid<-1>(rot32<3>()));
        const float2 tt[4] = {tph, t1, t2, t3};
#pragma unroll
        for (int r = 0; r < 4; r++) {
            v[r] = cmul_tw(v[r], tt[r]);
            const float2 u = cmul_tw(v[r + 4], tt[r]);
            const pk2 iu = pk_muli<1>(pk2{u.x, u.y});
            v[r + 4] = make_float2(iu.x, iu.y);
        }
    }
#pragma unroll
    for (int r = 0; r < 4; r++) {
        const pk2 a = {v[r].x, v[r].y}, b = {v[r + 4].x, v[r + 4].y};
        const pk2 s0 = pk_add(a, b), s1_ = pk_sub(a, b);
        v[r] = make_float2(s0.x, s0.y); v[r + 4] = make_float2(s1_.x, s1_.y);
    }
    lane_swap_bit2(v);
    {
        const float2 e = twid<-1>(rot16<1>());
        const float2 base = lb2 ? e : make_float2(1.f, 0.f);
        twiddle_powers<8>(v, base);
    }
    bfly8_pk<-1>(v);
    lane_transpose_hi3(v);
    {
        const float2 w1 = twid<-1>(p.twH[8 * hh]);
        if constexpr (WV == 8) twiddle_powers<8>(v, w1);
        else {
#pragma unroll
            for (int b = 0; b < Q; b++) twiddle_powers<WV>(&v[WV * b], w1);
        }
    }
    bfly_groups<WV, -1>(v);
    __syncthreads();
    if constexpr (WV == 8) wave_exchange(v, zbase, w, l);
    else wave_exchange_q<WV, false>(v, zbase, w, l);
    twiddle_powers<8>(v, twid<-1>(p.twH[pp]));
    bfly8_pk<-1>(v);
    float2* dst = p.S2 + ((long)c * p.NT + tile) * H * TK;
    constexpr float inv = 1.0f / (float)H;
    if (valid) {
#pragma unroll
        for (int i = 0; i < 8; i++) spec_store8(dst + tid + T * i, cscale(v[i], inv));
    }
    stamp_end(1, c);
}


}
```

vkresample_amd/csrc/kernels_pow2.hpp:

```cpp
#pragma once
#include <hip/hip_fp16.h>
#include <hip/hip_runtime.h>

#include <type_traits>

#include "fft_engine.hpp"
#include "kernels_generic.hpp"

namespace fftup {

constexpr int kColWaves = 8;

constexpr int ilog2c(int n) { return n <= 1 ? 0 : 1 + ilog2c(n / 2); }
constexpr int stage_radix(int N, int Ns, int RMAX = 8) { return (N / Ns >= RMAX) ? RMAX : (N / Ns); }

__device__ __forceinline__ int lswz(int i) { return i ^ ((i >> 3) & 15); }
__host__ __device__ constexpr int lswz_size(int n) { return (n + 15) & ~15; }
template <int TK> __device__ __forceinline__ int lidx(int idx, int col) { return lswz(idx * TK + col); }
constexpr int lswz_c(int i) { return i ^ ((i >> 3) & 15); }
typedef float lds_f2raw __attribute__((ext_vector_type(2)));
typedef __attribute__((address_space(3))) lds_f2raw lds_f2;
__device__ __forceinline__ unsigned lds_addr(const void* p) { return (unsigned)(unsigned long)(const __attribute__((address_space(3))) char*)p; }
__device__ __forceinline__ void lds_put(unsigned a0, int C, float2 v)
{
// ... 131 lines not shown
template <int SGN> __device__ __forceinline__ pk2 pk_muli(pk2 b)
{
    pk2 r;
    if constexpr (SGN > 0) asm("v_pk_add_f32 %0, 0, %1 op_sel:[0,1] op_sel_hi:[1,0] neg_lo:[0,1]" : "=v"(r) : "v"(b));
    else asm("v_pk_add_f32 %0, 0, %1 op_sel:[0,1] op_sel_hi:[1,0] neg_hi:[0,1]" : "=v"(r) : "v"(b));
    return r;
}
template <int DIR> __device__ __forceinline__ void bfly16_pk(float2* v)
{
    pk2 y[4][4];
#pragma unroll
    for (int n2 = 0; n2 < 4; n2++) {
#pragma unroll
        for (int n1 = 0; n1 < 4; n1++) y[n2][n1] = pk2{v[4 * n1 + n2].x, v[4 * n1 + n2].y};
        bfly4_pk<DIR>(y[n2][0], y[n2][1], y[n2][2], y[n2][3]);
    }
    y[1][1] = pk_rot16<DIR, 1>(y[1][1]); y[1][2] = pk_rot16<DIR, 2>(y[1][2]); y[1][3] = pk_rot16<DIR, 3>(y[1][3]);
    y[2][1] = pk_rot16<DIR, 2>(y[2][1]); y[2][2] = pk_muli<DIR>(y[2][2]);      y[2][3] = pk_rot16<DIR, 6>(y[2][3]);
    y[3][1] = pk_rot16<DIR, 3>(y[3][1]); y[3][2] = pk_rot16<DIR, 6>(y[3][2]); y[3][3] = pk_rot16<DIR, 9>(y[3][3]);
#pragma unroll
    for (int k1 = 0; k1 < 4; k1++) {
        bfly4_pk<DIR>(y[0][k1], y[1][k1], y[2][k1], y[3][k1]);
        v[k1] = make_float2(y[0][k1].x, y[0][k1].y); v[k1 + 4] = make_float2(y[1][k1].x, y[1][k1].y);
        v[k1 + 8] = make_float2(y[2][k1].x, y[2][k1].y); v[k1 + 12] = make_float2(y[3][k1].x, y[3][k1].y);
    }
}
template <int R, int DIR> __device__ __forceinline__ void bfly_reg(float2* v)
{
    if constexpr (R == 8) bfly8_pk<DIR>(v);
    else if constexpr (R == 16) bfly16_pk<DIR>(v);
    else if constexpr (R == 2 || R == 3 || R == 4 || R == 5 || R == 9 || R == 10 || R == 12 || R == 15) {
        pk2 z[R];
#pragma unroll
        for (int m = 0; m < R; m++) z[m] = pk2{v[m].x, v[m].y};
        bfly<R, DIR>(z);
#pragma unroll
        for (int m = 0; m < R; m++) v[m] = make_float2(z[m].x, z[m].y);
    } else bfly<R, DIR>(v);
}

template <int R> __device__ __forceinline__ void twiddle_powers(float2* v, float2 w1)
{
    if constexpr (R == 2) {
        v[1] = cmul_tw(v[1], w1);
    } else if constexpr (R == 4) {
        float2 w2 = cmul_tw(w1, w1), w3 = cmul_tw(w2, w1);
        v[1] = cmul_tw(v[1], w1); v[2] = cmul_tw(v[2], w2); v[3] = cmul_tw(v[3], w3);
    } else {
        float2 w2 = cmul_tw(w1, w1), w3 = cmul_tw(w2, w1), w4 = cmul_tw(w2, w2);
        float2 w5 = cmul_tw(w4, w1), w6 = cmul_tw(w3, w3), w7 = cmul_tw(w4, w3);
        v[1] = cmul_tw(v[1], w1); v[2] = cmul_tw(v[2], w2); v[3] = cmul_tw(v[3], w3); v[4] = cmul_tw(v[4], w4);
        v[5] = cmul_tw(v[5], w5); v[6] = cmul_tw(v[6], w6); v[7] = cmul_tw(v[7], w7);
        if constexpr (R == 16) {
            float2 w8 = cmul_tw(w4, w4);
            v[8] = cmul_tw(v[8], w8); v[9] = cmul_tw(v[9], cmul_tw(w8, w1)); v[10] = cmul_tw(v[10], cmul_tw(w5, w5));
            v[11] = cmul_tw(v[11], cmul_tw(w8, w3)); v[12] = cmul_tw(v[12], cmul_tw(w6, w6)); v[13] = cmul_tw(v[13], cmul_tw(w8, w5));
            v[14] = cmul_tw(v[14], cmul_tw(w7, w7)); v[15] = cmul_tw(v[15], cmul_tw(w8, w7));
        }
    }
}

template <int N, int E, int R, int Ns, int DIR, int B, bool PKB = true>
__device__ __forceinline__ void butterfly_b(float2 (&v)[E], float2 wbase)
{
    constexpr int Tc = N / E;
    constexpr int NB = E / R;
    if constexpr (B < NB) {
        float2 w[R];
#pragma unroll
        for (int m = 0; m < R; m++) w[m] = v[B + m * NB];
        if constexpr (Ns > 1) {
            float2 w1 = twid<DIR>(wbase);
            if constexpr (Ns > Tc && B > 0) w1 = cmul(w1, twid<DIR>(rot32<B * (32 / E)>()));
            twiddle_powers<R>(w, w1);
        }
        if constexpr (PKB) bfly_reg<R, DIR>(w);
        else bfly<R, DIR>(w);
#pragma unroll
        for (int m = 0; m < R; m++) v[B + m * NB] = w[m];
        butterfly_b<N, E, R, Ns, DIR, B + 1, PKB>(v, wbase);
    }
}

template <int N, int E, int R, int Ns, int DIR, bool PKB = true>
__device__ __forceinline__ void reg_butterflies(float2 (&v)[E], float2 wbase)
{
    constexpr int Tc = N / E;
    static_assert(Ns <= Tc || Ns * R == N, "per-butterfly twiddle offsets are only derived for the last stage");
    butterfly_b<N, E, R, Ns, DIR, 0, PKB>(v, wbase);
}

template <int N, int E, int R, int Ns, int TK>
__device__ __forceinline__ void reg_scatter(const float2 (&v)[E], float2* __restrict__ buf, int p, int col)
{
    constexpr int Tc = N / E;
    constexpr int NB = E / R;
    const unsigned base = lds_addr(buf);
#pragma unroll
    for (int b = 0; b < NB; b++) {
        const int j = p + b * Tc;
        const int k = j & (Ns - 1);
        const int j0 = (j - k) * R + k;
        const unsigned a0 = base + 8u * (unsigned)lidx<TK>(j0, col);
#pragma unroll
        for (int q = 0; q < R; q++) lds_put(a0, lswz_c(q * Ns * TK), v[b + q * NB]);
    }
}

template <int N, int E, int TK>
__device__ __forceinline__ void reg_gather(float2 (&v)[E], const float2* __restrict__ buf, int p, int col)
{
    constexpr int Tc = N / E;
    const unsigned a0 = lds_addr(buf) + 8u * (unsigned)lidx<TK>(p, col);
#pragma unroll
    for (int i = 0; i < E; i++) v[i] = lds_get(a0, lswz_c(i * Tc * TK));
#pragma unroll
    for (int i = 0; i < E; i += 2) asm volatile("" : "+v"(v[i].x), "+v"(v[i].y), "+v"(v[i + 1].x), "+v"(v[i + 1].y));
}

template <int N, int E, int DIR, int TK, bool FINAL_TO_LDS, int S = 0, int RMAX = 8, bool WAVE = false>
__device__ __forceinline__ void reg_fft(float2 (&v)[E], float2* __restrict__ buf, int p, int col,
                                        const TwSet<N, E, RMAX>& tws)
{
    constexpr int Ns = stage_ns(N, S, RMAX);
    constexpr int R = stage_radix(N, Ns, RMAX);
    static_assert(E % R == 0, "radix must divide the per-thread point count");
    reg_butterflies<N, E, R, Ns, DIR>(v, tws.w[S > 0 ? S - 1 : 0]);
    constexpr bool last = (Ns * R == N);
    if constexpr (!last || FINAL_TO_LDS) {
        reg_scatter<N, E, R, Ns, TK>(v, buf, p, col);
        lds_sync<WAVE>();
    }
    if constexpr (!last) {
        reg_gather<N, E, TK>(v, buf, p, col);
        lds_sync<WAVE>();
        reg_fft<N, E, DIR, TK, FINAL_TO_LDS, S + 1, RMAX, WAVE>(v, buf, p, col, tws);
    }
}

template <int N, int E, int DIR, int S = 0>
__device__ __forceinline__ void reg_fft_pp(float2 (&v)[E], float2* __restrict__ c, float2* __restrict__ z, int p, const TwSet<N, E, 8>& tws, int p0)
{
    constexpr int Ns = stage_ns(N, S, 8);
    constexpr int R = stage_radix(N, Ns, 8);
    constexpr int NE = num_stages(N, 8) - 1;
    static_assert(E % R == 0, "radix must divide the per-thread point count");
    reg_butterflies<N, E, R, Ns, DIR>(v, tws.w[S > 0 ? S - 1 : 0]);
    if constexpr (Ns * R != N) {
        float2* __restrict__ b = ((NE - 1 - S) % 2 == 0) ? z : c;
        reg_scatter<N, E, R, Ns, 1>(v, b, S == 0 ? p0 : p, 0);
        __syncthreads();
        reg_gather<N, E, 1>(v, b, p, 0);
        reg_fft_pp<N, E, DIR, S + 1>(v, c, z, p, tws, p0);
    }
}

#ifdef FFTUP_PLANE_STAMPS
__device__ unsigned long long g_plane_stamps[3][2048][3];
__device__ __forceinline__ unsigned stamp_wg() { return blockIdx.x + blockIdx.y * gridDim.x; }
__device__ __forceinline__ void stamp_begin(int k, int c) { if (threadIdx.x == 0) { g_plane_stamps[k][stamp_wg()][0] = wall_clock64(); g_plane_stamps[k][stamp_wg()][2] = (unsigned long long)c; } }
__device__ __forceinline__ void stamp_end(int k, int) { __syncthreads(); if (threadIdx.x == 0) g_plane_stamps[k][stamp_wg()][1] = wall_clock64(); }
#else
__device__ __forceinline__ void stamp_begin(int, int) {}
__device__ __forceinline__ void stamp_end(int, int) {}
#endif

struct RowR2CTParams {
    const void* in;
    float2* S1;
    const float2* tw;
    long in_row_stride, in_plane_stride;
    int H, NT;
};

template <int MODE> __device__ __forceinline__ float load_px_t(const RowR2CTParams& p, int c, int y, int x)
{
    if constexpr (MODE == IN_F32) return ((const float*)p.in)[c * p.in_plane_stride + y * p.in_row_stride + x];
    else if constexpr (MODE == IN_F16) return __half2float(((const __half*)p.in)[c * p.in_plane_stride + y * p.in_row_stride + x]);
    else if constexpr (MODE == IN_U8_F32) return cvt_u8_f32(((const uint8_t*)p.in)[y * p.in_row_stride + 3l * x + c]);
    else return cvt_u8_f16(((const uint8_t*)p.in)[y * p.in_row_stride + 3l * x + c]);
}

template <int W, int TK>
__device__ __forceinline__ void row_unpack_store(const float2* __restrict__ buf, const RowR2CTParams& p, int c, int j, int tid)
{
    constexpr int T = W / 8;
    static_assert(TK == 4 || TK == 8, "tile width");
    constexpr int LPT = TK;
    const long tile_stride = (long)p.H * TK;
    float2* base = p.S1 + (long)c * p.NT * tile_stride + (long)(2 * j) * TK;
    constexpr int NTILE = (W / 2 + 1 + TK - 1) / TK;
    for (int g = tid; g < NTILE * LPT; g += T) {
        const int tile = g / LPT, l = g % LPT;
        const bool isB = l >= LPT / 2;
        const int kk = (l % (LPT / 2)) * 2;
        float2 o[2];
#pragma unroll
        for (int e = 0; e < 2; e++) {
            const int k = tile * TK + kk + e;
            float2 r = make_float2(0.f, 0.f);
            if (k <= W / 2) {
                float2 zk = buf[lswz(k)];
                float2 zn = buf[lswz((W - k) & (W - 1))];
                r = isB ? make_float2(0.5f * (zk.y + zn.y), 0.5f * (-zk.x + zn.x))
                        : make_float2(0.5f * (zk.x + zn.x), 0.5f * (zk.y - zn.y));
            }
            o[e] = r;
        }
        spec_store16(base + (long)tile * tile_stride + (isB ? TK : 0) + kk, o[0], o[1]);
    }
}

template <int W, int MODE, int TK>
__global__ void __launch_bounds__(W / 8) k_row_r2c_t(RowR2CTParams p)
{
    constexpr int E = 8, T = W / E;
    __shared__ __attribute__((aligned(128))) float2 buf[lswz_size(W)];
    const int tid = threadIdx.x, c = blockIdx.y;
    const int j = blockIdx.x;
    float2 v[E];
    TwSet<W, E> tws;
    stamp_begin(0, c);
    tws.load(p.tw, tid);
#pragma unroll
    for (int i = 0; i < E; i++)
        v[i] = make_float2(load_px_t<MODE>(p, c, 2 * j, tid + T * i), load_px_t<MODE>(p, c, 2 * j + 1, tid + T * i));
    reg_fft<W, E, +1, 1, true>(v, buf, tid, 0, tws);
    row_unpack_store<W, TK>(buf, p, c, j, tid);
    stamp_end(0, c);
}


struct ColTParams {
    const float2* S1;
    float2* S2;
    const float2 *twH, *twUH;
    int W, NT;
    int zly, zry;
};

template <int TK, int Tc, int I>
__device__ __forceinline__ void col_phase(float2 (&v)[8], const float2* __restrict__ buf, int pp, int col, float2 w)
{
    if constexpr (I < 8) {
        constexpr int q = (I < 4) ? I : I + 8;
        const float2 f = buf[lidx<TK>(pp + Tc * I, col)];
        const float2 t = (q == 0) ? w : cmul(w, twid<-1>(rot16<q>()));
        v[I] = cmul(f, t);
        col_phase<TK, Tc, I + 1>(v, buf, pp, col, w);
    }
}

template <int H, int TK>
__global__ void __launch_bounds__(TK* H / 8, kColWaves) k_col_t(ColTParams p)
{
    constexpr int Tc = H / 8;
    extern __shared__ __attribute__((aligned(128))) char smem[];
    float2* buf = (float2*)smem;
    const int tid = threadIdx.x;
    const int col = tid % TK, pp = tid / TK;
    const int tile = blockIdx.x, c = blockIdx.y;
    const bool valid = tile * TK + col <= p.W / 2;
    const float2* src = p.S1 + ((long)c * p.NT + tile) * H * TK;
    float2 v[8];
    TwSet<H, 8> tws;
    tws.load(p.twH, pp);
    const float2 ph = p.twUH[pp];
#pragma unroll
    for (int i = 0; i < 8; i++) v[i] = valid ? src[(pp + Tc * i) * TK + col] : make_float2(0.f, 0.f);
    reg_fft<H, 8, +1, TK, true>(v, buf, pp, col, tws);
    col_phase<TK, Tc, 0>(v, buf, pp, col, twid<-1>(ph));
    __syncthreads();
    reg_fft<H, 8, -1, TK, false>(v, buf, pp, col, tws);
    float2* dst = p.S2 + ((long)c * p.NT + tile) * H * TK;
    constexpr float inv = 1.0f / (float)H;
    if (valid) {
#pragma unroll
        for (int i = 0; i < 8; i++) spec_store8(dst + (pp + Tc * i) * TK + col, cscale(v[i], inv));
    }
}

struct RowC2RTParams {
    const float2* S1;
    const float2* S2;
    void* R;
    const float2* tw;
    int uH, NT;
};

template <int UW, bool HALF_OUT, int TK, bool WIDE>
__global__ void __launch_bounds__(UW / 8) k_row_c2r_t(RowC2RTParams p)
{
    constexpr int E = 8, T = UW / E;
    __shared__ __attribute__((aligned(128))) float2 buf[lswz_size(UW)];
    const int tid = threadIdx.x, j = blockIdx.x, c = blockIdx.y;
    const long tile_stride = (long)(p.uH / 2) * TK;
    const long roff = (long)c * p.NT * tile_stride + (long)j * TK;
    auto ldAB = [&](int k, float2& A, float2& B) {
        const long o = roff + (long)(k / TK) * tile_stride + (k % TK);
        A = p.S1[o];
        B = p.S2[o];
    };
    float2 v[E];
    float2 A, B;
    TwSet<UW, E> tws;
    tws.load(p.tw, tid);
// ... 107 lines not shown
{
    if constexpr (HALF) {
        using A = Arith<true>;
        float minlen = A::r(0.5f * A::r(mn0 + mn1));
        float maxlen = A::r(0.5f * A::r(mx0 + mx1));
        minlen = A::r(__fdiv_rn(minlen, A::r(1.0f - minlen)));
        maxlen = A::r(__fdiv_rn(A::r(1.0f - maxlen), maxlen));
        float scale = (minlen < maxlen) ? minlen : maxlen;
        scale = A::r(-coef * A::r(__fsqrt_rn(scale)));
        float s4 = A::r(A::r(A::r(N + Wv) + E) + S);
        float num = A::r(C + A::r(scale * s4));
        float den = A::r(1.0f + A::r(scale * 4.0f));
        return A::r(__fdiv_rn(num, den));
    } else {
        float minlen = 0.5f * (mn0 + mn1);
        float maxlen = 0.5f * (mx0 + mx1);
        float a = minlen * __builtin_amdgcn_rcpf(1.0f - minlen);
        float b = (1.0f - maxlen) * __builtin_amdgcn_rcpf(maxlen);
        float scale = (a < b) ? a : b;
        scale = -coef * __builtin_amdgcn_sqrtf(scale);
        float s4 = ((N + Wv) + E) + S;
        return (C + scale * s4) * __builtin_amdgcn_rcpf(1.0f + scale * 4.0f);
    }
}

__device__ __forceinline__ float sharpen_eval_fast(float s4, float C, float mn0, float mn1, float mx0, float mx1, float coef)
{
    const float mn = 0.5f * (mn0 + mn1), mx = 0.5f * (mx0 + mx1);
    const bool lo = (mn + mx) < 1.0f;
    const float n = lo ? mn : 1.0f - mx;
    const float d = lo ? 1.0f - mn : mx;
    const float scale = -coef * n * __builtin_amdgcn_rsqf(fmaxf(n * d, 1e-30f));
    return fmaf(scale, s4, C) * __builtin_amdgcn_rcpf(fmaf(scale, 4.0f, 1.0f));
}

typedef float f2v __attribute__((ext_vector_type(2)));
__device__ __forceinline__ f2v mk2(float a, float b) { f2v r; r.x = a; r.y = b; return r; }
__device__ __forceinline__ f2v sharpen_eval_pair(f2v N, f2v S, f2v WE, f2v C, f2v mn0, f2v mn1, f2v mx0, f2v mx1, float coef)
{
    const f2v two = mk2(2.0f, 2.0f);
    const f2v smn = mn0 + mn1, smx = mx0 + mx1;
    const f2v u = two - smx;
    const f2v n2 = mk2(fminf(smn.x, u.x), fminf(smn.y, u.y));
    const f2v d2 = two - n2;
    const f2v pr = __builtin_elementwise_fma(n2, d2, mk2(1e-30f, 1e-30f));
    const f2v r = n2 * mk2(__builtin_amdgcn_rsqf(pr.x), __builtin_amdgcn_rsqf(pr.y));
    const f2v s4 = (WE + N) + S;
    const f2v num = __builtin_elementwise_fma(mk2(-coef, -coef), r * s4, C);
    const f2v den = __builtin_elementwise_fma(mk2(-4.0f * coef, -4.0f * coef), r, mk2(1.0f, 1.0f));
    return num * mk2(__builtin_amdgcn_rcpf(den.x), __builtin_amdgcn_rcpf(den.y));
}

__device__ __forceinline__ float add1(float a, float b)
{
    float r;
    asm("v_add_f32 %0, %1, %2" : "=v"(r) : "v"(a), "v"(b));
    return r;
}
typedef float f4t __attribute__((ext_vector_type(4)));
struct TapRow {
    f4t q;
    float l, r;
    __device__ __forceinline__ float operator[](int k) const { return k == 0 ? l : k == 5 ? r : q[(k - 1) & 3]; }
    __device__ __forceinline__ f2v lo() const { return __builtin_shufflevector(q, q, 0, 1); }
    __device__ __forceinline__ f2v hi() const { return __builtin_shufflevector(q, q, 2, 3); }
};
__device__ __forceinline__ void sharpen_vminmax(const TapRow (&t)[4], int w, float (&vmn)[6], float (&vmx)[6])
{
#pragma unroll
    for (int i = 0; i < 6; i++) {
        vmn[i] = fminf(fminf(t[w][i], t[w + 1][i]), t[w + 2][i]);
        vmx[i] = fmaxf(fmaxf(t[w][i], t[w + 1][i]), t[w + 2][i]);
    }
}
__device__ __forceinline__ f4t sharpen_quad_packed(const TapRow (&t)[4], int w, const float (&vmn)[6], const float (&vmx)[6], float coef)
{
    const TapRow& c = t[w + 1];
    float mn0[4], mn1[4], mx0[4], mx1[4];
#pragma unroll
    for (int k = 0; k < 4; k++) {
        mn1[k] = fminf(fminf(vmn[k], vmn[k + 1]), vmn[k + 2]);
        mx1[k] = fmaxf(fmaxf(vmx[k], vmx[k + 1]), vmx[k + 2]);
        mn0[k] = fminf(fminf(vmn[k + 1], c[k]), c[k + 2]);
        mx0[k] = fmaxf(fmaxf(vmx[k + 1], c[k]), c[k + 2]);
    }
    const f2v r01 = sharpen_eval_pair(t[w].lo(), t[w + 2].lo(), mk2(add1(c[0], c[2]), add1(c[1], c[3])), c.lo(),
                                      mk2(mn0[0], mn0[1]), mk2(mn1[0], mn1[1]), mk2(mx0[0], mx0[1]), mk2(mx1[0], mx1[1]), coef);
    const f2v r23 = sharpen_eval_pair(t[w].hi(), t[w + 2].hi(), mk2(add1(c[2], c[4]), add1(c[3], c[5])), c.hi(),
                                      mk2(mn0[2], mn0[3]), mk2(mn1[2], mn1[3]), mk2(mx0[2], mx0[3]), mk2(mx1[2], mx1[3]), coef);
    return __builtin_shufflevector(r01, r23, 0, 1, 2, 3);
}

struct SharpenTParams {
    const void* R;
    void* out;
    int uW, uH;
    float upsq, coef;
};

template <bool HALF, int RPT>
__global__ void __launch_bounds__(256) k_sharpen_t(SharpenTParams p)
{
    const int lane = threadIdx.x;
    const int x0 = (blockIdx.x * 64 + lane) * 4;
    const int y0 = (blockIdx.y * 4 + threadIdx.y) * RPT;
    const int c = blockIdx.z;
    const int uW = p.uW;
    const long plane = (long)uW * p.uH;
    const long poff = c * plane;
    PxRow<HALF> ra, rb, rc;
    sharpen_load_row<HALF>(ra, p.R, poff, plane, uW, y0 > 0 ? y0 - 1 : 0, x0, lane, p.upsq);
    sharpen_load_row<HALF>(rb, p.R, poff, plane, uW, y0, x0, lane, p.upsq);
#pragma unroll
    for (int r = 0; r < RPT; r++) {
        const int y = y0 + r;
        sharpen_load_row<HALF>(rc, p.R, poff, plane, uW, y + 1, x0, lane, p.upsq);
        float o[4];
#pragma unroll
        for (int i = 0; i < 4; i++) {
            const float N = ra.L[1 + i], S = rc.L[1 + i], Wv = rb.L[i], C = rb.L[1 + i], E = rb.L[2 + i];
            float mn0 = fminf(fminf(N, S), fminf(fminf(Wv, C), E));
            float mx0 = fmaxf(fmaxf(N, S), fmaxf(fmaxf(Wv, C), E));
            float mn1 = fminf(mn0, fminf(fminf(ra.L[i], ra.L[2 + i]), fminf(rc.L[i], rc.L[2 + i])));
            float mx1 = fmaxf(mx0, fmaxf(fmaxf(ra.L[i], ra.L[2 + i]), fmaxf(rc.L[i], rc.L[2 + i])));
            if constexpr (HALF) o[i] = sharpen_eval<true>(N, S, Wv, E, C, mn1, mx1, mn0, mx0, p.coef);
            else o[i] = sharpen_eval_fast(((N + Wv) + E) + S, C, mn0, mn1, mx0, mx1, p.coef);
        }
        const long of = poff + (long)y * uW + x0;
        if constexpr (HALF) {
            __half2 h0 = __floats2half2_rn(o[0], o[1]), h1 = __floats2half2_rn(o[2], o[3]);
            typedef float f2v __attribute__((ext_vector_type(2)));
            f2v val = {*(float*)&h0, *(float*)&h1};
            __builtin_nontemporal_store(val, (f2v*)((__half*)p.out + of));
        } else {
            typedef float f4v __attribute__((ext_vector_type(4)));
            f4v val = {o[0], o[1], o[2], o[3]};
            __builtin_nontemporal_store(val, (f4v*)((float*)p.out + of));
        }
        ra = rb;
        rb = rc;
    }
}


struct FusedParams {
    const float2* S1;
    unsigned odd_delta;
    void* out;
    const float2* tw;
    int uH, NT;
    int pairs_per_strip;
    float upsq, coef;
    int u8_wrap;
};
__device__ __forceinline__ float absmin1(float x)
{
    float r;
    asm("v_min_f32_e64 %0, |%1|, 1.0" : "=v"(r) : "v"(x));
    return r;
}
template <bool HALF> __device__ __forceinline__ float to_L(float g, float upsq)
{
    using A = Arith<HALF>;
    if constexpr (HALF) g = __half2float(__float2half_rn(g));
    return fminf(fmaxf(fabsf(A::r(upsq * g)), 0.0f), 1.0f);
}

__device__ __forceinline__ float div_f32_newton(float a, float b)
{
    const float r = __builtin_amdgcn_rcpf(b);
    const float q = a * r;
    return fmaf(fmaf(-q, b, a), r, q);
}
__device__ __forceinline__ float sharpen_eval_half_fast(float N, float S, float Wv, float E, float C,
                                                        float mn0, float mn1, float mx0, float mx1, float coef)
{
    const __half one = __float2half_rn(1.0f), hlf = __float2half_rn(0.5f);
    const __half mn = __hmul(hlf, __hadd(__float2half_rn(mn0), __float2half_rn(mn1)));
    const __half mx = __hmul(hlf, __hadd(__float2half_rn(mx0), __float2half_rn(mx1)));
    const bool lo = (__half2float(mn) + __half2float(mx)) < 1.0f;
    const float n = __half2float(lo ? mn : __hsub(one, mx));
    const float d = __half2float(lo ? __hsub(one, mn) : mx);
    const float q = __half2float(__float2half_rn(div_f32_newton(n, d)));
    float rt = 0.f;
    if (q > 0.f) {
        const float rs = __builtin_amdgcn_rsqf(q);
        const float s0 = q * rs;
        rt = fmaf(fmaf(-s0, s0, q), 0.5f * rs, s0);
    }
    const __half scale = __hmul(__float2half_rn(-coef), __float2half_rn(rt));
    const __half s4 = __hadd(__hadd(__hadd(__float2half_rn(N), __float2half_rn(Wv)), __float2half_rn(E)), __float2half_rn(S));
    __half prod = __hmul(scale, s4);
    asm volatile("" : "+v"(prod));
    const __half num = __hadd(__float2half_rn(C), prod);
    const __half den = __hadd(one, __hmul(scale, __float2half_rn(4.0f)));
    return __half2float(__float2half_rn(div_f32_newton(__half2float(num), __half2float(den))));
}

template <bool HALF>
__device__ __forceinline__ void sharpen_quad(const float (&t)[3][6], float coef, float (&o)[4])
{
    float hmn[3][4], hmx[3][4];
#pragma unroll
    for (int r = 0; r < 3; r++)
#pragma unroll
        for (int i = 0; i < 4; i++) {
            hmn[r][i] = fminf(fminf(t[r][i], t[r][i + 1]), t[r][i + 2]);
            hmx[r][i] = fmaxf(fmaxf(t[r][i], t[r][i + 1]), t[r][i + 2]);
        }
#pragma unroll
    for (int i = 0; i < 4; i++) {
        const float N = t[0][i + 1], S = t[2][i + 1], Wv = t[1][i], C = t[1][i + 1], E = t[1][i + 2];
        const float mn0 = fminf(fminf(N, S), hmn[1][i]);
        const float mx0 = fmaxf(fmaxf(N, S), hmx[1][i]);
        const float mn1 = fminf(fminf(hmn[0][i], hmn[2][i]), mn0);
        const float mx1 = fmaxf(fmaxf(hmx[0][i], hmx[2][i]), mx0);
        if constexpr (HALF) o[i] = sharpen_eval_half_fast(N, S, Wv, E, C, mn0, mn1, mx0, mx1, coef);
        else o[i] = sharpen_eval_fast(((N + Wv) + E) + S, C, mn0, mn1, mx0, mx1, coef);
    }
}

typedef _Float16 h2v __attribute__((ext_vector_type(2)));
__device__ __forceinline__ h2v h2_bits(unsigned u) { return __builtin_bit_cast(h2v, u); }
__device__ __forceinline__ unsigned bits_h2(h2v h) { return __builtin_bit_cast(unsigned, h); }
__device__ __forceinline__ h2v h2_splat(float f) { const _Float16 x = (_Float16)f; h2v r = {x, x}; return r; }
__device__ __forceinline__ h2v pk_min3(h2v a, h2v b, h2v c)
{
    h2v r;
    asm("v_pk_minimum3_f16 %0, %1, %2, %3" : "=v"(r) : "v"(a), "v"(b), "v"(c));
    return r;
}
__device__ __forceinline__ h2v pk_max3(h2v a, h2v b, h2v c)
{
    h2v r;
    asm("v_pk_maximum3_f16 %0, %1, %2, %3" : "=v"(r) : "v"(a), "v"(b), "v"(c));
    return r;
}
__device__ __forceinline__ h2v pk_rcp_h(h2v b)
{
    h2v r;
    asm("v_rcp_f16_e32 %0, %1\n\ts_nop 0\n\tv_rcp_f16_sdwa %0, %1 dst_sel:WORD_1 dst_unused:UNUSED_PRESERVE src0_sel:WORD_1" : "=&v"(r) : "v"(b));
    return r;
}
__device__ __forceinline__ h2v pk_sqrt_h(h2v b)
{
    h2v r;
    asm("v_sqrt_f16_e32 %0, %1\n\ts_nop 0\n\tv_sqrt_f16_sdwa %0, %1 dst_sel:WORD_1 dst_unused:UNUSED_PRESERVE src0_sel:WORD_1" : "=&v"(r) : "v"(b));
    return r;
}
__device__ __forceinline__ h2v pk_div(h2v a, h2v b)
{
#pragma clang fp contract(off)
    const h2v rc = pk_rcp_h(b);
    const h2v q = a * rc;
    return __builtin_elementwise_fma(__builtin_elementwise_fma(-q, b, a), rc, q);
}
__device__ __forceinline__ h2v sharpen_eval_pair_half(h2v N, h2v S, h2v Wv, h2v E, h2v C, h2v mn0, h2v mn1, h2v mx0, h2v mx1, h2v ncoef)
{
#pragma clang fp contract(off)
    const h2v one = {(_Float16)1.0f, (_Float16)1.0f}, two = {(_Float16)2.0f, (_Float16)2.0f}, four = {(_Float16)4.0f, (_Float16)4.0f};
    const h2v smn = mn0 + mn1, smx = mx0 + mx1;
    const h2v u = two - smx;
    const h2v n2 = __builtin_elementwise_min(smn, u);
    const h2v d2 = two - n2;
    const h2v q = pk_div(n2, d2);
    const h2v r = pk_sqrt_h(q);
    const h2v scale = ncoef * r;
    const h2v s4 = ((N + Wv) + E) + S;
    const h2v prod = scale * s4;
    const h2v num = C + prod;
    const h2v den = __builtin_elementwise_fma(scale, four, one);
    return pk_div(num, den);
}
typedef _Float16 h4v __attribute__((ext_vector_type(4)));
__device__ __forceinline__ h4v h4_cat(h2v a, h2v b) { return __builtin_shufflevector(a, b, 0, 1, 2, 3); }
__device__ __forceinline__ h2v h4_lo(h4v a) { return __builtin_shufflevector(a, a, 0, 1); }
__device__ __forceinline__ h2v h4_hi(h4v a) { return __builtin_shufflevector(a, a, 2, 3); }
__device__ __forceinline__ h4v pk4_rcp_h(h4v b)
{
    h2v r0, r1;
    const h2v b0 = h4_lo(b), b1 = h4_hi(b);
    asm("v_rcp_f16_e32 %0, %2\n\tv_rcp_f16_e32 %1, %3\n\t"
        "v_rcp_f16_sdwa %0, %2 dst_sel:WORD_1 dst_unused:UNUSED_PRESERVE src0_sel:WORD_1\n\t"
        "v_rcp_f16_sdwa %1, %3 dst_sel:WORD_1 dst_unused:UNUSED_PRESERVE src0_sel:WORD_1" : "=&v"(r0), "=&v"(r1) : "v"(b0), "v"(b1));
    return h4_cat(r0, r1);
}
__device__ __forceinline__ h4v pk4_sqrt_h(h4v b)
{
    h2v r0, r1;
    const h2v b0 = h4_lo(b), b1 = h4_hi(b);
    asm("v_sqrt_f16_e32 %0, %2\n\tv_sqrt_f16_e32 %1, %3\n\t"
        "v_sqrt_f16_sdwa %0, %2 dst_sel:WORD_1 dst_unused:UNUSED_PRESERVE src0_sel:WORD_1\n\t"
        "v_sqrt_f16_sdwa %1, %3 dst_sel:WORD_1 dst_unused:UNUSED_PRESERVE src0_sel:WORD_1" : "=&v"(r0), "=&v"(r1) : "v"(b0), "v"(b1));
    return h4_cat(r0, r1);
}
__device__ __forceinline__ h4v pk4_div(h4v a, h4v b)
{
#pragma clang fp contract(off)
    const h4v rc = pk4_rcp_h(b);
    const h4v q = a * rc;
    return __builtin_elementwise_fma(__builtin_elementwise_fma(-q, b, a), rc, q);
}
__device__ __forceinline__ h4v sharpen_eval_quad_half(h4v N, h4v S, h4v Wv, h4v E, h4v C, h4v mn0, h4v mn1, h4v mx0, h4v mx1, h4v ncoef)
{
#pragma clang fp contract(off)
    const _Float16 f1 = (_Float16)1.0f, f2 = (_Float16)2.0f, f4 = (_Float16)4.0f;
// ... 158 lines not shown
            if constexpr (FINAL_TO_LDS) {
#pragma unroll
                for (int m = 0; m < R2; m++) g[m * NB2 * TK] = v[m];
            }
        }
        if constexpr (FINAL_TO_LDS) __syncthreads();
    }
};

template <int N, int DIR, int T, int TK, int... RS> struct MrFftNT {
    static constexpr int NST = sizeof...(RS);
    static constexpr int rs(int s) { constexpr int r[] = {RS...}; return r[s]; }
    static constexpr int ns(int s) { int n = 1; for (int i = 0; i < s; i++) n *= rs(i); return n; }
    static constexpr int bpt(int s) { return (N / rs(s) + T - 1) / T; }
    static constexpr int vn() { int m = 0; for (int s = 0; s < NST; s++) m = bpt(s) * rs(s) > m ? bpt(s) * rs(s) : m; return m; }
    static constexpr int mb() { int m = 0; for (int s = 0; s < NST; s++) m = bpt(s) > m ? bpt(s) : m; return m; }
    static constexpr int VN = vn(), MB = mb();
    static_assert(ns(NST) == N && bpt(0) == 1 && bpt(NST - 1) == 1, "radices multiply to N; one butterfly per thread at both ends");
    struct Tw { float2 w[NST - 1][MB]; };
    template <int S = 1> static __device__ __forceinline__ void load_tw(Tw& w, const float2* __restrict__ tw, int j)
    {
        if constexpr (S < NST) {
            constexpr int R = rs(S), Ns = ns(S), NB = N / R;
#pragma unroll
            for (int b = 0; b < bpt(S); b++) {
                const int jb = j + T * b;
                w.w[S - 1][b] = tw[((jb < NB ? jb : 0) % Ns) * (N / (Ns * R))];
            }
            load_tw<S + 1>(w, tw, j);
        }
    }
    static constexpr bool pow2(int n) { return (n & (n - 1)) == 0; }
    template <bool INPLACE, int S = 0>
    static __device__ __forceinline__ void run(float2 (&v)[VN], float2* __restrict__ c, float2* __restrict__ z, int j, const Tw& w, int col = 0)
    {
        if constexpr (S < NST) {
            constexpr int R = rs(S), Ns = ns(S), NB = N / R, BPT = bpt(S), NE = NST - 1;
            float2* __restrict__ const bin = (!INPLACE && (NE - S) % 2 == 0) ? z : c;
            float2* __restrict__ const bout = (!INPLACE && (NE - 1 - S) % 2 == 0) ? z : c;
            asm volatile("" : "+v"(j));
            if constexpr (S > 0) {
#pragma unroll
                for (int b = 0; b < BPT; b++) {
                    const int jb = j + T * b;
                    if (jb < NB) {
#pragma unroll
                        for (int m = 0; m < R; m++) v[b * R + m] = bin[lidx<TK>(jb + NB * m, col)];
                    }
                }
                if constexpr (INPLACE) __syncthreads();
            }
#pragma unroll
            for (int b = 0; b < BPT; b++) {
                const int jb = j + T * b;
                if (jb < NB) {
                    if constexpr (S > 0) twiddle_all<R>(&v[b * R], twid<DIR>(w.w[S > 0 ? S - 1 : 0][b]));
                    bfly_reg<R, DIR>(&v[b * R]);
                    if constexpr (S + 1 < NST) {
                        const int k = jb % Ns, j0 = (jb - k) * R + k;
                        if constexpr (pow2(R) && pow2(Ns)) {
                            const unsigned a0 = lds_addr(bout) + 8u * (unsigned)lidx<TK>(j0, col);
#pragma unroll
                            for (int m = 0; m < R; m++) lds_put(a0, lswz_c(m * Ns * TK), v[b * R + m]);
                        } else {
#pragma unroll
                            for (int m = 0; m < R; m++) bout[lidx<TK>(j0 + m * Ns, col)] = v[b * R + m];
                        }
                    }
                }
            }
            if constexpr (S + 1 < NST) {
                __syncthreads();
                run<INPLACE, S + 1>(v, c, z, j, w, col);
            }
        }
    }
};
template <int N, int DIR, int T, int... RS> using MrFftN = MrFftNT<N, DIR, T, 1, RS...>;

template <int UW_, int T_, int NBUF_, int WPE_, bool RR_, int... RS> struct FusedPlanN {
    using F = MrFftN<UW_, -1, T_, RS...>;
    static constexpr int UW = UW_, T = T_, R0 = F::rs(0), NB0 = UW / R0, EOUT = F::rs(F::NST - 1), SOUT = UW / EOUT, VN = F::VN;
    static constexpr size_t XB = sizeof(float2) * lswz_size(UW);
    static constexpr int NBUF = NBUF_;
    static constexpr bool RING_REGS = RR_;
    static constexpr int WPE = WPE_;
    static_assert(T >= NB0 && T >= SOUT, "one butterfly per thread at both ends");
    static_assert(NBUF == 2 || (F::NST - 1) % 2 == 1, "three buffers: the first exchange must go through z");
    static_assert(XB % 128 == 0, "lds_put needs 128-byte aligned buffers");
    using Tw = typename F::Tw;
    static constexpr bool MIRROR_SHARE = false;
    static __device__ __forceinline__ int first_index(int lt) { return lt < NB0 ? lt : NB0 - 1; }
    static __device__ __forceinline__ void load_tw(Tw& w, const float2* __restrict__ tw, int j) { F::load_tw(w, tw, j); }
    static __device__ __forceinline__ void fft(float2 (&v)[VN], float2* __restrict__ buf, float2* __restrict__ zbuf, int j, const Tw& w, int = 0)
    {
        Tw t = w;
#pragma unroll
        for (int st = 0; st < F::NST - 1; st++)
#pragma unroll
            for (int b = 0; b < F::MB; b++) asm volatile("" : "+v"(t.w[st][b].x), "+v"(t.w[st][b].y));
        F::template run<NBUF == 2>(v, buf, zbuf, j, t);
    }
};
template <int UW_, int R2_> struct FusedPlanMr16 {
    using F = MrFft<UW_, -1, 16, 16, R2_>;
    static constexpr int UW = UW_, T = 256, R0 = 16, NB0 = F::NB0, EOUT = R2_, SOUT = F::NB2, VN = F::VN;
    static_assert(F::NB2 == T && F::NB0 <= T && F::NB1 <= T, "one butterfly per thread and stage, all threads in the last one");
    static constexpr size_t XB = (sizeof(float2) * lpad_size(UW) + 15) & ~(size_t)15;
    using Tw = typename F::Tw;
    static __device__ __forceinline__ int first_index(int lt) { return lt < NB0 ? lt : NB0 - 1; }
    static __device__ __forceinline__ void load_tw(Tw& w, const float2* __restrict__ tw, int j) { F::load_tw(w, tw, j); }
    static constexpr int NBUF = 2;
    static constexpr bool RING_REGS = true;
    static constexpr int WPE = 2;
    static constexpr bool MIRROR_SHARE = false;
    static __device__ __forceinline__ void fft(float2 (&v)[VN], float2* __restrict__ buf, float2* __restrict__ zbuf, int j, const Tw& w, int = 0)
    {
        F::fft(v, buf, NBUF == 3 ? zbuf : buf, j, w);
    }
};
using FusedPlan3840x16 = FusedPlanMr16<3840, 15>;

template <class PL> struct FusedGLds {
    static constexpr size_t XB = PL::XB;
    static constexpr bool RR = PL::RING_REGS && (PL::UW + 4 * PL::T - 1) / (4 * PL::T) <= 4;
    static constexpr size_t NX = RR ? 1 : 2;
    static constexpr size_t ZOFF = NX * XB;
    static constexpr size_t RED = NX * XB;
    static constexpr size_t TOTAL = (NX + (PL::NBUF == 3 ? 1 : 0)) * XB + (PL::NBUF == 3 ? 0 : 32 * sizeof(float));
};

template <bool HALF, bool OUT_U8 = false>
__device__ __forceinline__ void deferred_pixel(const FusedParams& p, long of, float n0, float n1, float ne, float m0, float m1, float me,
                                               float s0, float s1, float se)
{
    if constexpr (HALF) {
        auto sp = [](float v) { const _Float16 x = (_Float16)v; h2v r = {x, x}; return r; };
        const h2v a0 = sp(n0), a1 = sp(n1), a2 = sp(ne), b0 = sp(m0), b1 = sp(m1), b2 = sp(me), c0 = sp(s0), c1 = sp(s1), c2 = sp(se);
        const h2v mn0 = pk_min3(a0, b0, c0), mn1 = pk_min3(a1, b1, c1), mn2 = pk_min3(a2, b2, c2);
        const h2v mx0 = pk_max3(a0, b0, c0), mx1 = pk_max3(a1, b1, c1), mx2 = pk_max3(a2, b2, c2);
        const h2v o = sharpen_eval_pair_half(a1, c1, b0, b2, b1, pk_min3(mn1, b0, b2), pk_min3(mn0, mn1, mn2),
                                             pk_max3(mx1, b0, b2), pk_max3(mx0, mx1, mx2), h2_splat(-p.coef));
        if constexpr (OUT_U8) ((uint8_t*)p.out)[of] = cvt_f_u8((float)o.x, p.u8_wrap);
        else ((_Float16*)p.out)[of] = o.x;
    } else {
        const float tt[3][6] = {{n0, n0, n1, ne, ne, ne}, {m0, m0, m1, me, me, me}, {s0, s0, s1, se, se, se}};
        float o[4];
        sharpen_quad<false>(tt, p.coef, o);
        if constexpr (OUT_U8) ((uint8_t*)p.out)[of] = cvt_f_u8(o[1], p.u8_wrap);
        else ((float*)p.out)[of] = o[1];
    }
}

template <class PL, bool HALF, int TK, int U = 2, int D = 2 * U, bool OUT_U8 = false, int DD = 1>
__global__ void __launch_bounds__(PL::T, PL::WPE) k_c2r_sharpen_g(FusedParams p)
{
    constexpr int UW = PL::UW, T = PL::T, R0 = PL::R0, NB0 = PL::NB0, NI = R0 * DD / D, KH = UW * DD / D;
    static_assert((R0 * DD) % D == 0, "the first radix must be a multiple of 2u");
    static_assert(UW % 4 == 0, "the sharpen passes work on quads of pixels");
    constexpr int EOUT = PL::EOUT, SOUT = PL::SOUT, VN = PL::VN;
    constexpr int NPASS = (UW + 4 * T - 1) / (4 * T);
    static_assert(KH == NB0 * NI, "the non-zero half spectrum must fill whole first-stage inputs");
    constexpr float inv = (1.0f / (float)U) / (float)UW;
    using L = FusedGLds<PL>;
    using LT = typename std::conditional<HALF, _Float16, float>::type;
    extern __shared__ __attribute__((aligned(128))) char smem[];
    float* red = (float*)(smem + L::RED);
    int lt = threadIdx.x;
    const int uH = p.uH;
    const int pairs_per_plane = uH / 2;
    const long plane = (long)UW * uH;
    typename PL::Tw tws;
    PL::load_tw(tws, p.tw, lt);

    int f0, f1;
    if constexpr (OUT_U8) {
        const int b = blockIdx.x, r = b >> 3;
        const int st = (r / 3) * 8 + (b & 7);
        const int j0u = st * p.pairs_per_strip;
        if (j0u >= pairs_per_plane) return;
        f0 = (r % 3) * pairs_per_plane + j0u;
        f1 = f0 + min(p.pairs_per_strip, pairs_per_plane - j0u);
    } else {
        f0 = blockIdx.x * p.pairs_per_strip;
        f1 = min(f0 + p.pairs_per_strip, 3 * pairs_per_plane);
    }
    while (f0 < f1) {
        const int c = f0 / pairs_per_plane;
        const int j0 = f0 - c * pairs_per_plane;
        const int j1 = min(j0 + (f1 - f0), pairs_per_plane);
        f0 += j1 - j0;
        const int y0 = 2 * j0, y1 = 2 * j1;
        const bool top = (y0 == 0);
        const int a0 = top ? 0 : y0 - 1;
        const int npairs = (j1 - j0) + 1;
        const unsigned tile_stride32 = (unsigned)(uH / U) * TK;
        const float2* base = p.S1 + (long)c * p.NT * (long)tile_stride32;
        auto koff = [&](int k) -> unsigned {
            return (__umul24((unsigned)k / TK, tile_stride32) + ((unsigned)k % TK)) * (unsigned)sizeof(float2);
        };
        typedef const __attribute__((address_space(1))) char* gptr_t;
        auto rowbase = [&](int row) -> gptr_t {
            const unsigned off = (((unsigned)row / U) * TK + ((unsigned)row % U) * p.odd_delta) * (unsigned)sizeof(float2);
            gptr_t r = (gptr_t)base + __builtin_amdgcn_readfirstlane(off);
            asm("" : "+s"(r));
            return r;
        };
        auto gload = [](gptr_t r, unsigned off) -> float2 {
            asm("" : "+v"(off));
            const lds_f2raw t = *(const __attribute__((address_space(1))) lds_f2raw*)(r + off);
            return make_float2(t.x, t.y);
        };
        auto S2at = [&](int k, int row) -> float2 { return gload(rowbase(row), koff(k)); };
        auto dc_im = [&](int row) -> float { return *(const __attribute__((address_space(1))) float*)(rowbase(row) + 4); };
        const bool need_corner = !top && (y1 + 1 < uH);
        const int rs = y1 + 1;

        constexpr bool MS = PL::MIRROR_SHARE;
        struct In { float2 a[NI], am[NI], b[NI], bm[NI]; float lka, lkb; };
        unsigned ko[NI], kom[NI];
        const int jj = PL::first_index(lt);
        {
#pragma unroll
            for (int m = 0; m < NI; m++) { ko[m] = koff(jj + NB0 * m); kom[m] = koff(KH - jj - NB0 * m); }
        }
        const bool ms_self = MS && lt < 64 && (lt & 31) == 0;
        auto load_pair = [&](int i) -> In {
            In in;
            const int a = a0 + 2 * i;
            const int ya = min(a, uH - 1), yb = min(a + 1, uH - 1);
            const gptr_t ra = rowbase(ya), rb = rowbase(yb);
            if constexpr (MS) {
#pragma unroll
                for (int m = 0; m < NI; m++) {
                    in.a[m] = gload(ra, ko[m]); in.b[m] = gload(rb, ko[m]);
                    asm volatile("" : "=v"(in.am[m].x), "=v"(in.am[m].y), "=v"(in.bm[m].x), "=v"(in.bm[m].y));
                }
                if (ms_self) {
#pragma unroll
                    for (int m = 0; m < NI; m++) { in.am[m] = gload(ra, kom[m]); in.bm[m] = gload(rb, kom[m]); }
                }
            } else {
#pragma unroll
                for (int m = 0; m < NI; m++) {
                    in.a[m] = gload(ra, ko[m]); in.am[m] = gload(ra, kom[m]);
                    in.b[m] = gload(rb, ko[m]); in.bm[m] = gload(rb, kom[m]);
                }
            }
            in.lka = dc_im(ya ^ 1);
            in.lkb = dc_im(yb ^ 1);
            return in;
        };
        auto settle = [](In& in) {
            __builtin_amdgcn_s_waitcnt(0x0F70);
#pragma unroll
            for (int m = 0; m < NI; m++)
                asm volatile("" : "+v"(in.a[m].x), "+v"(in.a[m].y), "+v"(in.am[m].x), "+v"(in.am[m].y), "+v"(in.b[m].x), "+v"(in.b[m].y),
                                  "+v"(in.bm[m].x), "+v"(in.bm[m].y));
            asm volatile("" : "+v"(in.lka), "+v"(in.lkb));
        };

        auto share = [&](In& in) __attribute__((always_inline)) {
            if constexpr (MS) {
                const int pl = (((lt & 63) ^ 32) << 2);
                auto part = [&](float2 z) -> float2 {
                    return make_float2(__builtin_bit_cast(float, __builtin_amdgcn_ds_bpermute(pl, __builtin_bit_cast(int, z.x))),
                                       __builtin_bit_cast(float, __builtin_amdgcn_ds_bpermute(pl, __builtin_bit_cast(int, z.y))));
                };
                if (!ms_self) {
#pragma unroll
                    for (int m = 0; m < NI; m++) { in.am[m] = part(in.a[NI - 1 - m]); in.bm[m] = part(in.b[NI - 1 - m]); }
                }
            }
        };
        if (need_corner) {
            float part = 0.f;
            for (int kk = lt + 1; kk <= KH; kk += T) part += S2at(kk, rs).x;
#pragma unroll
            for (int o = 32; o > 0; o >>= 1) part += __shfl_down(part, o);
            if ((lt & 63) == 0) red[lt >> 6] = part;
            if (lt == T - 1) {
                float2 d = S2at(0, rs), dp = S2at(0, rs ^ 1);
                red[16] = (rs & 1) ? d.x + dp.y : d.x - dp.y;
            }
        }
        In in = load_pair(0);
        settle(in);
        share(in);
        __syncthreads();
        float corner = 0.f;
        if (need_corner) {
            float sum = 0.f;
            for (int w2 = 0; w2 < (T + 63) / 64; w2++) sum += red[w2];
            corner = (red[16] + 2.0f * sum) * inv;
        }
        if constexpr (PL::NBUF == 3) __syncthreads();
        float pn0 = 0.f, pn1 = 0.f;
        constexpr bool RR = L::RR;
        using SavedRow = typename std::conditional<HALF, H2Row, TapRow>::type;
        SavedRow sv[RR ? NPASS : 1][2];
        float lprev0 = 0.f;
        if constexpr (RR) {
#pragma unroll
            for (int h = 0; h < NPASS; h++) sv[h][0] = sv[h][1] = SavedRow{};
        }

        for (int s = 0; s < npairs; s++) {
            const int a = a0 + 2 * s;
            float2* buf = (float2*)(smem + (RR ? 0 : (s & 1)) * L::XB);
            LT* cur = (LT*)buf;
            const LT* ring = (const LT*)(smem + ((s + 1) & 1) * L::XB);
            asm volatile("" : "+v"(lt));
            float2 v[VN];
#pragma unroll
            for (int m = 0; m < VN; m++) v[m] = make_float2(0.f, 0.f);
#pragma unroll
            for (int m = 0; m < NI; m++) {
                v[m] = cadd_i(in.a[m], in.b[m]);
                v[R0 - NI + m] = cadd_conj_i(in.am[m], in.bm[m]);
            }
            if (lt == 0) {
                v[NI] = make_float2(in.am[0].x - in.bm[0].y, in.am[0].y + in.bm[0].x);
                const int ya = min(a, uH - 1), yb = min(a + 1, uH - 1);
                v[0] = make_float2(in.a[0].x + ((ya & 1) ? in.lka : -in.lka), in.b[0].x + ((yb & 1) ? in.lkb : -in.lkb));
            }
            in = load_pair(min(s + 1, npairs - 1));
            PL::fft(v, buf, (float2*)(smem + L::ZOFF), lt, tws, jj);
            settle(in);
            share(in);
            if constexpr (HALF) {
                const h2v up2 = h2_splat(p.upsq), one2 = h2_splat(1.0f);
                if (SOUT == T || lt < SOUT) {
#pragma unroll
                    for (int i = 0; i < EOUT; i++) {
                        const f2v sv = mk2(v[i].x, v[i].y) * mk2(inv, inv);
                        const h2v g = {(_Float16)sv.x, (_Float16)sv.y};
                        const h2v Lv = __builtin_elementwise_min(h2_bits(bits_h2(up2 * g) & 0x7fff7fffu), one2);
                        cur[lt + SOUT * i] = Lv.x;
                        cur[UW + lt + SOUT * i] = Lv.y;
                    }
                }
            } else {
                const float ks = inv * p.upsq;
                if (SOUT == T || lt < SOUT) {
#pragma unroll
                    for (int i = 0; i < EOUT; i++) {
                        const f2v sv = mk2(v[i].x, v[i].y) * mk2(ks, ks);
                        cur[lt + SOUT * i] = absmin1(sv.x);
                        cur[UW + lt + SOUT * i] = absmin1(sv.y);
                    }
                }
            }
            __syncthreads();
            const float la0 = (float)cur[0], la1 = (float)cur[UW];
            constexpr int LT_LAST = (UW / 4 - 1) % T, H_LAST = (UW / 4 - 1) / T;
            auto finish_deferred = [&]() __attribute__((always_inline)) {
                if constexpr (RR) {
                    if (lt == LT_LAST) {
                        const SavedRow& R2 = sv[H_LAST][0];
                        const SavedRow& R1 = sv[H_LAST][1];
                        float r2a, r2b, r1a, r1b, r10;
                        if constexpr (HALF) { r2a = (float)R2.h23.x; r2b = (float)R2.h23.y; r1a = (float)R1.h23.x; r1b = (float)R1.h23.y; r10 = (float)R2.sc.y; }
                        else { r2a = R2.q.z; r2b = R2.q.w; r1a = R1.q.z; r1b = R1.q.w; r10 = R2.r; }
                        if (s > 0 && (a - 2) >= y0 && (a - 2) < y1 && a <= uH - 1)
                            deferred_pixel<HALF, OUT_U8>(p, OUT_U8 ? ((long)(a - 2) * UW + (UW - 1)) * 3 + c : c * plane + (long)(a - 2) * UW + (UW - 1),
                                                         pn0, pn1, (a - 2 == 0) ? r10 : lprev0, r2a, r2b, r10, r1a, r1b, la0);
                        if (a == 0) { pn0 = (float)cur[UW - 2]; pn1 = (float)cur[UW - 1]; }
                        else { pn0 = r1a; pn1 = r1b; }
                        lprev0 = la0;
                    }
                }
            };
            float lse = la1;
            {
                const int r2 = min(a + 2, uH - 1) - a;
                if (r2 == 0) lse = la0;
                else if (r2 > 1 && s == npairs - 1) lse = to_L<HALF>(corner, p.upsq);
            }
            auto rowp = [&](int r) -> const LT* { return r < 0 ? ring + (r + 2) * UW : cur + r * UW; };
            const bool out0 = (a - 1) >= y0 && (a - 1) < y1;
            const bool out1 = a >= y0 && a < y1;
            if constexpr (HALF) {
                if (out0 || out1 || RR) {
                    const h2v ncoef = h2_splat(-p.coef);
                    auto pass = [&](auto hc) __attribute__((always_inline)) {
                        const int h = hc;
                        const int x0 = 4 * (lt + T * h);
                        if (UW % (4 * T) != 0 && x0 >= UW) return;
                        const LT* rows[4] = {RR ? nullptr : rowp(-2), RR ? nullptr : ((a == 0) ? rowp(0) : rowp(-1)), rowp(0), rowp(1)};
                        uint2 q[4], ql[4], qr[4];
#pragma unroll
                        for (int r = 3; r >= (RR ? 2 : 0); r--) {
                            const LT* rp = rows[r] + x0;
                            q[r] = *(const uint2*)rp; ql[r] = *(const uint2*)(rp - 4); qr[r] = *(const uint2*)(rp + 4);
                        }
                        if constexpr (RR) { if (h == H_LAST) finish_deferred(); }
                        H2Row R[4];
#pragma unroll
                        for (int r = 3; r >= 0; r--) {
                            if constexpr (RR) {
                                if (r < 2) {
                                    R[r] = sv[h][r];
                                    if (r == 1 && a == 0) {
                                        asm volatile("");
                                        R[1].sa = R[2].sa; R[1].h01 = R[2].h01; R[1].sb = R[2].sb; R[1].h23 = R[2].h23; R[1].sc = R[2].sc;
                                    }
                                    continue;
                                }
                            }
                            if (r == 0 && !out0) {
                                R[0].sa = R[0].h01 = R[0].sb = R[0].h23 = R[0].sc = h2_splat(0.f);
                                continue;
                            }
                            asm volatile("" : "+v"(q[r].x), "+v"(q[r].y), "+v"(ql[r].x), "+v"(ql[r].y), "+v"(qr[r].x), "+v"(qr[r].y));
                            R[r].h01 = h2_bits(q[r].x);
                            R[r].h23 = h2_bits(q[r].y);
                            R[r].sa = h2_bits(__builtin_amdgcn_alignbit(q[r].x, ql[r].y, 16));
                            R[r].sb = h2_bits(__builtin_amdgcn_alignbit(q[r].y, q[r].x, 16));
                            R[r].sc = h2_bits(__builtin_amdgcn_alignbit(qr[r].x, q[r].y, 16));
                            if (x0 == 0) R[r].sa = h2_bits((bits_h2(R[r].h01) & 0xffffu) * 0x10001u);
                        }
                        if (x0 + 4 == UW) {
                            auto set_hi = [](h2v& d, float v) { d.y = (_Float16)v; };
                            if (a != 0) set_hi(R[1].sc, la0);
                            set_hi(R[3].sc, lse);
                        }
                        if constexpr (RR) { sv[h][0] = R[2]; sv[h][1] = R[3]; }
#pragma unroll
                        for (int w = 0; w < 2; w++) {
                            if (w == 0 ? !out0 : !out1) continue;
                            h2v o01, o23;
                            sharpen_quad_half(R[w], R[w + 1], R[w + 2], ncoef, o01, o23);
                            if constexpr (OUT_U8) {
                                uint8_t b8[4];
                                cvt4_h_u8(o01, o23, p.u8_wrap, b8);
                                uint8_t* d8 = (uint8_t*)p.out + ((long)(a - 1 + w) * UW * 3 + c) + (unsigned)x0 * 3u;
                                d8[0] = b8[0]; d8[3] = b8[1]; d8[6] = b8[2]; d8[9] = b8[3];
                                continue;
                            }
                            const long row_of = c * plane + (long)(a - 1 + w) * UW;
                            f2v val = {__builtin_bit_cast(float, o01), __builtin_bit_cast(float, o23)};
                            __builtin_nontemporal_store(val, (f2v*)((char*)((__half*)p.out + row_of) + (unsigned)x0 * 2u));
                        }
                    };
                    if constexpr (RR) {
                        pass(std::integral_constant<int, 0>{});
                        if constexpr (NPASS > 1) pass(std::integral_constant<int, 1>{});
                        if constexpr (NPASS > 2) pass(std::integral_constant<int, 2>{});
                        if constexpr (NPASS > 3) pass(std::integral_constant<int, 3>{});
                    } else {
#pragma unroll 1
                        for (int h = 0; h < NPASS; h++) pass(h);
                    }
                }
            } else {
            if (out0 || out1 || RR) {
                auto pass = [&](auto hc) __attribute__((always_inline)) {
                    const int h = hc;
                    const int x0 = 4 * (lt + T * h);
                    if (UW % (4 * T) != 0 && x0 >= UW) return;
                    const float* rows[4] = {RR ? nullptr : rowp(-2), RR ? nullptr : ((a == 0) ? rowp(0) : rowp(-1)), rowp(0), rowp(1)};
                    f4t q[4], ql[4], qr[4];
#pragma unroll
                    for (int r = 3; r >= (RR ? 2 : 0); r--) {
                        const float* rp = rows[r] + x0;
                        q[r] = *(const f4t*)rp; ql[r] = *(const f4t*)(rp - 4); qr[r] = *(const f4t*)(rp + 4);
                    }
                    if constexpr (RR) { if (h == H_LAST) finish_deferred(); }
                    TapRow t[4];
#pragma unroll
                    for (int r = 3; r >= 0; r--) {
                        if constexpr (RR) {
                            if (r < 2) {
                                t[r] = sv[h][r];
                                if (r == 1 && a == 0) {
                                    asm volatile("");
                                    t[1].q = t[2].q; t[1].l = t[2].l; t[1].r = t[2].r;
                                }
                                continue;
                            }
                        }
                        if (r == 0 && !out0) {
// ... 63 lines not shown
```

vkresample_amd/csrc/plan.hpp:

```cpp
#pragma once
#include <hip/hip_runtime.h>

#include <atomic>
#include <condition_variable>
#include <cstdint>
#include <initializer_list>
#include <mutex>
#include <string>
#include <thread>
#include <vector>

#include "../../include/fftup.h"
#include "bluestein_plan.hpp"
#include "fft_engine.hpp"
#include "jit.hpp"
#include "plan_rules.hpp"
#include "png_params.hpp"

using fftup::BzPlan;
using fftup::PngParams;

#define HIP_TRY(expr)                                                                              \
    do {                                                                                           \
        hipError_t _e = (expr);                                                                    \
        if (_e != hipSuccess)                                                                      \
            return fail(_e == hipErrorOutOfMemory ? FFTUP_E_OUT_OF_MEMORY : FFTUP_E_HIP,           \
                        std::string(#expr) + ": " + hipGetErrorString(_e));                        \
    } while (0)

struct EventList {
    std::vector<hipEvent_t> ev;
    ~EventList() { for (auto& e : ev) if (e) (void)hipEventDestroy(e); }
    int create(size_t n)
    {
        ev.assign(n, nullptr);
        for (auto& e : ev) {
            hipError_t r = hipEventCreate(&e);
            if (r != hipSuccess) { e = nullptr; return fail(FFTUP_E_HIP, std::string("hipEventCreate: ") + hipGetErrorString(r)); }
        }
        return FFTUP_OK;
    }
    hipEvent_t& operator[](size_t i) { return ev[i]; }
};

struct fftup_plan : PlanGeometry {
    int device = 0;
    hipStream_t stream = nullptr;
    hipEvent_t ev0 = nullptr, ev1 = nullptr;
    hipDeviceProp_t prop{};
    fftup_jit::Module* jit = nullptr;
    struct FourTables { float2 *tw1 = nullptr, *tw2 = nullptr; };
    FourTables fourFtw, fourItw, colFtw, colItw;
    BzPlan bzW{}, bzH{}, bzUW{}, bzUH{};
    float2 *phW = nullptr, *phH = nullptr;
    fftup_view vw{};
    struct ViewAxis { int kmax = 0; uint32_t L = 0; StagePlan planL{}; float2 *tw = nullptr, *pre = nullptr, *post = nullptr, *bhat = nullptr; };
    ViewAxis vx, vy;
    struct ViewTabs { float2 *pre[2] = {nullptr, nullptr}, *post[2] = {nullptr, nullptr}, *bhat[2] = {nullptr, nullptr};
                      double span[2] = {0, 0}; int kmax[2] = {0, 0}; bool built = false; };
    std::vector<ViewTabs> vtabs;
    double2* vroots[2] = {nullptr, nullptr};
    bool R_valid = false;

    std::vector<void*> in_planar;
    std::vector<uint8_t*> in_u8;
    std::vector<int> in_kind;
    struct Lane { hipStream_t stream = nullptr; float2 *S1 = nullptr, *S2 = nullptr; void* R = nullptr; hipEvent_t done = nullptr;
                  void* T4 = nullptr; };
    std::vector<Lane> lanes;
    int nlanes = 1;
    int last_lane = 0;
    std::vector<void*> out;
    uint8_t* out_u8 = nullptr;
    struct PngSlot { PngParams p{}; bool ready = false; unsigned long long* meta_host = nullptr; uint32_t* parts_host = nullptr; hipEvent_t copied = nullptr;
                     int state = 0; uint64_t ticket = 0; std::thread::id owner{}; uint8_t* dest = nullptr; size_t dest_cap = 0; };
    struct QSlot { uint8_t* out_u8 = nullptr; hipEvent_t done = nullptr; PngSlot png;
                   bool used = false; uint64_t ticket = 0; };
    std::vector<QSlot> q;
    std::atomic<uint64_t> q_next{0};
    uint32_t q_cursor = 0;
    std::mutex q_mu;
    std::condition_variable q_cv;
    hipStream_t png_copy = nullptr;
    int png_rpb = 0, png_nblocks = 0;
    size_t png_stream_bytes = 0;
    uint32_t* png_crc_shift = nullptr;
    bool png_foreign_collector = false;
    float2 *twW = nullptr, *twH = nullptr, *twUW = nullptr, *twUH = nullptr;
    float2 *rotW = nullptr, *rotH = nullptr, *rotUW = nullptr, *rotUH = nullptr;
    uint64_t device_bytes = 0;
    size_t r_bytes = 0;
    uint64_t* d_sum = nullptr;
    size_t in_plane_stride = 0;
    int executed = 0;

    struct DeviceIO { hipEvent_t start = nullptr; std::vector<void*> stage_in, scratch_out; };
    DeviceIO dio;
    bool dev_executed = false;

    std::vector<void*> allocs;
};

int dev_alloc(fftup_plan* P, void** ptr, size_t bytes);
int view_frames_prepare(fftup_plan* P, int nl);
inline DeviceFacts device_facts(const hipDeviceProp_t& prop)
{
    return {prop.sharedMemPerBlock ? prop.sharedMemPerBlock : 65536, prop.multiProcessorCount, prop.gcnArchName};
}
inline bool fuse_u8(const fftup_plan* P) { return (P->cfg.flags & FFTUP_FLAG_FUSE_U8_LOAD) && !P->dbl; }
inline int check_slot(fftup_plan* P, uint32_t slot)
{
    if (!P) return fail(FFTUP_E_INVALID_ARG, "null plan");
    if (slot >= P->ring) return fail(FFTUP_E_INVALID_ARG, "slot out of range");
    return FFTUP_OK;
}

int kernels_allow_view_tables(const fftup_plan* P);
int kernels_set_attributes(fftup_plan* P);
enum class Pass { rows, columns, inverse, sharpen, all, presharpen_tap };
struct DeviceInput { const void* in = nullptr; int kind = 0; long in_row = 0, in_plane = 0; };
struct FrameRun { int lane = 0; uint32_t in_slot = 0; void* out = nullptr; const DeviceInput* in = nullptr; Pass pass = Pass::all;
                  const fftup_view* view = nullptr; const fftup_shift* shift = nullptr; };
int launch_frame(fftup_plan* P, const FrameRun& r);
int launch_shift_path(const fftup_shift* in, fftup_shift* out, uint32_t n, uint32_t mode, float sigma, float min_peak, hipStream_t st);
void launch_unpack(fftup_plan* P, uint32_t slot, hipStream_t st);
void launch_pack(fftup_plan* P, uint32_t slot, uint8_t* dst, hipStream_t st);
void launch_checksum(fftup_plan* P, uint32_t slot, hipStream_t st);
void launch_unpack_from(fftup_plan* P, const uint8_t* rgb, size_t row_stride_bytes, void* planes, hipStream_t st);
void launch_pack_to(fftup_plan* P, const void* planes, uint8_t* rgb, size_t row_stride_bytes, hipStream_t st);
void launch_copy_rows(const void* src, size_t src_row, size_t src_plane, void* dst, size_t dst_row, size_t dst_plane,
                      size_t row_bytes, uint32_t rows, uint32_t planes, int gran, hipStream_t st);

int lanes_fork(fftup_plan* P, hipEvent_t ev, hipStream_t from, int first, int nl);
int lanes_join(fftup_plan* P, int first, int nl, std::initializer_list<hipStream_t> into, int rc);
int execute_ring_impl(fftup_plan* P, uint32_t n_frames, uint32_t first_slot, double* ms_total, double* kernel_ms, uint32_t stride);

int check_device_image(size_t esz, bool u8out, int device, const fftup_device_image& im, const char* side, uint32_t i, uint32_t w, uint32_t h, bool is_out);

int submit_frame(fftup_plan* P, const uint8_t* rgb_in, size_t in_stride, uint8_t* rgb_out, size_t out_stride, bool png, uint64_t* ticket);

void png_geometry(fftup_plan* P);
int png_slot_init(fftup_plan* P, fftup_plan::QSlot& Q);
int png_enqueue(fftup_plan* P, fftup_plan::QSlot& Q, hipStream_t cs, uint8_t* png_dest);
```

vkresample_amd/csrc/plan_rules.cpp:

```cpp
#include "plan_rules.hpp"

#include <algorithm>
#include <cmath>
#include <cstdio>
#include <cstdlib>

#include <hip/hip_fp16.h>

#include "mirror_tables.hpp"
#include "view_tables.hpp"

using namespace fftup;
using Four = PlanGeometry::Four;

static constexpr size_t LDS_GFX950 = (size_t)160 * 1024;

bool is_smooth(uint32_t n)
{
    if (n == 0) return false;
    for (uint32_t p : {2u, 3u, 5u, 7u})
        while (n % p == 0) n /= p;
    return n == 1;
}

// ... 333 lines not shown
{
    const uint32_t W = G.W, H = G.H, uW = G.uW, uH = G.uH;
    const char* const poly_e = fftup_jit::experiment("generic_poly");
    if (!G.cplx && !G.dct && !G.down && !G.odd && is_smooth(H) && uW == 2 * W && uH == 2 * H && G.zly == (int)(H / 2) && G.zry == (int)(uH - H / 2) && !(poly_e && atoi(poly_e) == 0)) {
        for (int tk : {8, 4, 2, 1}) {
            const size_t need = G.csz * (size_t)lpad_size((int)H * tk);
            const int thr = inplace_threads(G.planH, tk, COL_INPLACE_PT, kernels_generic_max_threads(G.dbl));
            if (thr && need <= lds_max / 2) { G.TK = tk; G.ldsCol = need; G.poly = true; G.thrCol = thr; break; }
        }
    }
    if (!G.TK && G.dbl && !G.cplx) {
        for (int tk : {8, 4, 2, 1}) {
            const size_t need = G.csz * (size_t)lpad_size((int)uH * tk);
            const int tmax = kernels_generic_max_threads(true);
            const int thr = std::max(inplace_threads(G.planH, tk, COL_INPLACE_PT, tmax), inplace_threads(G.planUH, tk, COL_INPLACE_PT, tmax));
            const bool ok = inplace_threads(G.planH, tk, COL_INPLACE_PT, tmax) && inplace_threads(G.planUH, tk, COL_INPLACE_PT, tmax) &&
                            need <= lds_max / 2 && (size_t)(H / 2) * tk <= (size_t)COL_INPLACE_PT * thr;
            if (ok) { G.TK = tk; G.ldsCol = need; G.inplaceC = true; G.thrCol = thr; break; }
        }
    }
    if (G.view) {
        G.viewL[0] = view_conv_length(W, uW, G.mirror); G.viewL[1] = view_conv_length(H, uH, G.mirror);
        G.TK = view_col_tk(H, uH, G.mirror);
        G.ldsCol = 2 * G.csz * (size_t)lpad_size((int)(std::max(lds_length(H, G.TK), G.viewL[1]) * (uint32_t)G.TK));
        if (G.ldsCol > lds_max) return fail(FFTUP_E_UNSUPPORTED_SIZE, "fftup_plan_create_view: this device's LDS does not hold the column transform");
    }
    if (!G.TK && (G.odd || !is_smooth(H) || !is_smooth(uH))) {
        G.TK = bluestein_col_tk(H, uH);
        G.ldsCol = 2 * G.csz * (size_t)lpad_size((int)(std::max(std::max(H, uH), std::max(lds_length(H, G.TK), lds_length(uH, G.TK))) * (uint32_t)G.TK));
        if (G.ldsCol > lds_max) return fail(FFTUP_E_UNSUPPORTED_SIZE, "FFTUP_FLAG_ANY_SIZE: this device's LDS does not hold the column transform");
    }
    if (!G.TK) for (int tk : {8, 4, 2, 1}) {
        size_t need = 2 * G.csz * (size_t)lpad_size((int)std::max(H, uH) * tk);
        if (need <= lds_max) { G.TK = tk; G.ldsCol = need; break; }
    }
    return FFTUP_OK;
}

static bool aot_enabled()
{
    const char* const aot_e = fftup_jit::experiment("aot");
    return !(aot_e && atoi(aot_e) == 0);
}

int plan_geometry_columns(PlanGeometry& G, const DeviceFacts& dev)
{
    const uint32_t W = G.W, H = G.H, uW = G.uW, uH = G.uH;
    const float u = G.cfg.upscale;
    G.zlx = (int)(W / 2);
    G.zrx = G.cplx ? (int)(uint32_t)((2 * u - 1) * (float)uW / (2 * u)) : (int)(uW / 2);
    G.zly = G.zry = 0;
    if (!G.down && !G.exact) column_guard(u, uH, &G.zly, &G.zry);

    G.planW = make_stage_plan(W);
    G.planH = make_stage_plan(H);
    G.planUW = make_stage_plan(uW);
    G.planUH = make_stage_plan(uH);

    const bool aot_u2 = aot_enabled() && !G.dbl && !G.cplx && !G.dct && !G.down && !G.exact && !(G.cfg.flags & FFTUP_FLAG_GENERIC_KERNELS) && uW == 2 * W && uH == 2 * H;
    G.tuned = aot_u2 && (W == 512 || W == 1024 || W == 2048) && (H == 256 || H == 512 || H == 1024);
    G.TK = 0;
    if (G.tuned) {
        G.TK = TUNED_TK;
        G.ldsCol = kernels_tuned_col_lds(H);
    }
    else if (int rc = choose_column_tile(G, dev.lds_bytes)) return rc;
    if (!G.TK && G.dct) return fail(FFTUP_E_UNSUPPORTED_SIZE, "FFTUP_FLAG_DCT: the columns do not fit the LDS (no four-step DCT)");
    if (!G.TK && G.down) return fail(FFTUP_E_UNSUPPORTED_SIZE, "FFTUP_FLAG_DOWNSCALE: the columns do not fit the LDS (no four-step downscale)");
    if (!G.TK) {
        G.TK = 1; G.ldsCol = 0;
        if (!make_four(G, G.colF, H) || !make_four(G, G.colI, uH))
            return fail(FFTUP_E_UNSUPPORTED_SIZE, "column too long: no four-step split of the height fits the LDS");
    }
    if (aot_u2 && !G.tuned && G.TK >= 4) G.mixed = kernels_aot_mixed_plan(W, H);
    if (G.mixed) { G.TK = 4; G.ldsCol = sizeof(float2) * (size_t)H * 4; }
    return FFTUP_OK;
}

int plan_jit_factor(const PlanGeometry& G, int* DD)
{
    *DD = 1;
    if (G.dbl || G.cplx || G.dct || G.down || G.bz || G.odd || G.tuned || G.mixed || (G.cfg.flags & (FFTUP_FLAG_GENERIC_KERNELS | FFTUP_FLAG_UNFUSED_SHARPEN)) || !jit_enabled())
        return 0;
    return jit_factor(G.cfg.upscale, G.W, G.H, G.uW, G.uH, G.zly, G.zry, DD);
}

static int choose_family(PlanGeometry& G)
{
    const bool resampled = G.odd || G.view || G.bz, own = G.tuned || G.mixed;
    if ((G.cplx && (G.dct || G.down || resampled)) || (G.dbl && (G.dct || G.down || resampled)) || (G.dct && resampled) ||
        (own && (G.cplx || G.dbl || G.dct || G.down || resampled)) || (G.tuned && G.mixed))
        return fail(FFTUP_E_INVALID_ARG, "internal: the plan rules let two kernel families claim this plan");
    using Family = PlanGeometry::Family;
    G.family = G.cplx ? Family::cplx : G.dbl ? Family::f64 : G.dct ? Family::dct : G.view ? Family::view : G.odd ? Family::odd : G.down ? Family::down
               : G.tuned ? Family::tuned : G.mixed == 3 ? Family::mixed_jit : G.mixed ? Family::mixed_aot : Family::generic;
    return FFTUP_OK;
}

static int row_buffers(PlanGeometry& G, size_t lds_max)
{
    const uint32_t W = G.W, uW = G.uW;
    G.ldsRowF = 2 * G.csz * (size_t)lpad_size((int)W);
    G.ldsRowI = 2 * G.csz * (size_t)lpad_size((int)uW);
    if (G.bz) {
        G.ldsRowF = 2 * G.csz * (size_t)lpad_size((int)lds_length(W, 1));
        G.ldsRowI = 2 * G.csz * (size_t)lpad_size((int)lds_length(uW, 1));
        if (G.ldsRowF > lds_max) return fail(FFTUP_E_UNSUPPORTED_SIZE, "FFTUP_FLAG_ANY_SIZE: this device's LDS does not hold the row transform");
    }
    if (G.cplx) {
        G.inplaceF = rows_fit(W, G.dbl) == 1; G.inplaceI = rows_fit(uW, G.dbl) == 1;
        if (G.inplaceF) G.ldsRowF /= 2;
        if (G.inplaceI) G.ldsRowI /= 2;
        if (!rows_fit(W, G.dbl)) { make_four(G, G.fourF, W); G.ldsRowF = 0; }
        if (!rows_fit(uW, G.dbl)) { make_four(G, G.fourI, uW); G.ldsRowI = 0; }
    }
    if (G.view) G.ldsRowI = 2 * G.csz * (size_t)lpad_size((int)G.viewL[0]);
    if (G.ldsRowI > lds_max) return fail(FFTUP_E_UNSUPPORTED_SIZE, "upscaled width too large for LDS");
    return FFTUP_OK;
}

static void choose_threads(PlanGeometry& G)
{
    const uint32_t W = G.W, H = G.H, uW = G.uW, uH = G.uH;
    const int tmax = kernels_generic_max_threads(G.dbl);
    G.thrW = fft_threads((int)W, tmax);
    G.thrUW = fft_threads((int)uW, tmax);
    if (!(G.poly || G.inplaceC)) G.thrCol = fft_threads((int)std::max(H, uH) * G.TK, tmax);
    if (G.bz) {
        G.thrW = fft_threads((int)lds_length(W, 1), tmax);
        G.thrUW = fft_threads((int)lds_length(uW, 1), tmax);
        if (!G.poly) G.thrCol = fft_threads((int)std::max(lds_length(H, G.TK), lds_length(uH, G.TK)) * G.TK, tmax);
    }
    if (G.view) {
        G.thrUW = fft_threads((int)G.viewL[0], tmax);
        G.thrCol = fft_threads((int)std::max(lds_length(H, G.TK), G.viewL[1]) * G.TK, tmax);
    }
    if (G.dbl && !G.cplx) {
        const int tf = inplace_threads(G.planW, 1, 8, tmax), ti = inplace_threads(G.planUW, 1, 8, tmax);
        if (tf) { G.inplaceF = true; G.thrW = tf; G.ldsRowF /= 2; }
        if (ti) { G.inplaceI = true; G.thrUW = ti; G.ldsRowI /= 2; }
    }
}

int plan_geometry_finish(PlanGeometry& G, const DeviceFacts& dev, const fftup_jit::Choice* jit)
{
    if (jit) {
        G.mixed = 3; G.U = jit->U; G.TK = 4; G.ldsCol = jit->col_lds;
        G.colF = Four{}; G.colI = Four{};
    }
    if (G.tuned || G.mixed) G.poly = false;
    if (int rc = choose_family(G)) return rc;
    G.fused = (G.tuned || G.mixed) && !(G.cfg.flags & FFTUP_FLAG_UNFUSED_SHARPEN);
    G.u8out = G.fused && (G.cfg.flags & FFTUP_FLAG_FUSE_U8_STORE);
    G.pairs_per_strip = strip_length(G, dev, fused_threads(G, jit));
    G.NT = (G.ncols + G.TK - 1) / G.TK;
    if (int rc = row_buffers(G, dev.lds_bytes)) return rc;
    choose_threads(G);
    const uint32_t len[4] = {G.W, G.H, G.uW, G.uH};
    for (int i = 0; i < 4; i++)
        if (G.bz && !is_smooth(len[i]) && !(G.view && i >= 2)) G.bzL[i] = lds_length(len[i], (i & 1) ? G.TK : 1);
    G.upsq = const_via_percent_f((double)(G.cfg.upscale * G.cfg.upscale), G.half);
    G.coef = const_via_percent_f((double)G.cfg.sharpen, G.half);
    return FFTUP_OK;
}

static uint32_t pow2_floor(uint32_t v)
{
    uint32_t p = 1;
    while (p <= v / 2) p *= 2;
    return v ? p : 0;
}

int align_geometry(const fftup_align_config& c, AlignGeometry& G)
{
    const char* who = "fftup_align_create: ";
    if (c.width == 0 || c.height == 0) return fail(FFTUP_E_INVALID_ARG, std::string(who) + "width and height must be > 0");
    if (c.width > (1u << 16) || c.height > (1u << 16)) return fail(FFTUP_E_INVALID_ARG, std::string(who) + "width/height above 65536");
    if (c.precision == 1) return fail(FFTUP_E_UNSUPPORTED_PRECISION, std::string(who) + "precision must be 0 (float planes) or 2 (half planes): there are no -p 1 frames");
    if (c.precision > 2) return fail(FFTUP_E_UNSUPPORTED_PRECISION, std::string(who) + "precision must be 0 (float planes) or 2 (half planes)");
    if (c.decimate != 0 && c.decimate != 1 && c.decimate != 2 && c.decimate != 4 && c.decimate != 8)
        return fail(FFTUP_E_INVALID_ARG, std::string(who) + "decimate " + std::to_string(c.decimate) + " must be 1, 2, 4 or 8 (0: automatic)");
    const uint32_t win[2] = {c.window_w, c.window_h};
    for (int a = 0; a < 2; a++)
        if (win[a] && (win[a] < 16 || win[a] > 1024 || (win[a] & (win[a] - 1))))
            return fail(FFTUP_E_INVALID_ARG, std::string(who) + (a ? "window_h " : "window_w ") + std::to_string(win[a]) + " must be a power of two in [16, 1024] (0: automatic)");
    if (!(c.band == 0.0f || (c.band > 0.0f && c.band <= 1.0f))) return fail(FFTUP_E_INVALID_ARG, std::string(who) + "band must lie in (0, 1] (0: 0.5)");
    if (c.upsample && (c.upsample < 4 || c.upsample > 64)) return fail(FFTUP_E_INVALID_ARG, std::string(who) + "upsample " + std::to_string(c.upsample) + " must lie in [4, 64] (0: 32)");
    if (c.max_batch > 65535) return fail(FFTUP_E_INVALID_ARG, std::string(who) + "max_batch must be <= 65535");
    G.W = c.width; G.H = c.height; G.precision = c.precision;
    G.band = c.band == 0.0f ? 0.5f : c.band;
    G.kappa = c.upsample ? c.upsample : 32;
    G.max_batch = c.max_batch ? c.max_batch : 16;
    G.d = c.decimate;
    if (!G.d) {
        G.d = 8;
        for (uint32_t d : {1u, 2u, 4u, 8u})
            if (pow2_floor(c.width / d) <= 1024 && pow2_floor(c.height / d) <= 1024) { G.d = d; break; }
    }
    if (c.width / G.d < 16 || c.height / G.d < 16)
        return fail(FFTUP_E_INVALID_ARG, std::string(who) + "a frame of " + std::to_string(c.width) + "x" + std::to_string(c.height) + " has fewer than 16 decimated pixels on an axis (d = " + std::to_string(G.d) + ")");
    G.nx = c.window_w ? c.window_w : std::min(1024u, pow2_floor(c.width / G.d));
    G.ny = c.window_h ? c.window_h : std::min(1024u, pow2_floor(c.height / G.d));
    if ((uint64_t)G.nx * G.d > c.width) return fail(FFTUP_E_INVALID_ARG, std::string(who) + "window_w * d = " + std::to_string((uint64_t)G.nx * G.d) + " exceeds the frame's width " + std::to_string(c.width));
    if ((uint64_t)G.ny * G.d > c.height) return fail(FFTUP_E_INVALID_ARG, std::string(who) + "window_h * d = " + std::to_string((uint64_t)G.ny * G.d) + " exceeds the frame's height " + std::to_string(c.height));
    G.crop_x = (c.width - G.nx * G.d) / 2;
    G.crop_y = (c.height - G.ny * G.d) / 2;
    G.band_kx = (uint32_t)std::floor((double)G.band * (double)G.nx / 2.0);
    G.band_ky = (uint32_t)std::floor((double)G.band * (double)G.ny / 2.0);
    G.Kx = G.band_kx < G.nx / 2 ? 2 * G.band_kx + 1 : G.nx;
    G.Ky = G.band_ky < G.ny / 2 ? 2 * G.band_ky + 1 : G.ny;
    return FFTUP_OK;
}
```

vkresample_amd/csrc/plan_rules.hpp:

```cpp
#pragma once
#include <cstdint>
#include <string>
#include <vector>

#include "../../include/fftup.h"
#include "fft_engine.hpp"
#include "jit_choose.hpp"

using fftup::StagePlan;

static constexpr int TUNED_TK = 4;

int fail(int code, const std::string& msg);

int kernels_generic_max_threads(bool dbl);
int kernels_aot_mixed_plan(uint32_t W, uint32_t H);
size_t kernels_tuned_col_lds(uint32_t H);

struct DeviceFacts { size_t lds_bytes = 0; int compute_units = 0; std::string arch; };

struct PlanRequest { const fftup_config* cfg = nullptr; const uint32_t* size = nullptr; uint32_t align = 0; const fftup_view* view = nullptr; };

struct PlanGeometry {
    fftup_config cfg{};
    uint32_t W = 0, H = 0, uW = 0, uH = 0;
    uint32_t ring = 1;
    bool half = false;
    bool dbl = false;
    size_t esz = 4, csz = 8;

    int TK = 8, NT = 0;
    int zlx = 0, zrx = 0, zly = 0, zry = 0;
    StagePlan planW{}, planH{}, planUW{}, planUH{};
    int thrW = 0, thrCol = 0, thrUW = 0;
    size_t ldsRowF = 0, ldsCol = 0, ldsRowI = 0;
    float upsq = 0, coef = 0;
    enum class Family { generic, tuned, mixed_aot, mixed_jit, cplx, f64, dct, down, odd, view };
    Family family = Family::generic;
    bool tuned = false;
    bool fused = false;
    bool u8out = false;
    int mixed = 0;
    int U = 2;
    bool cplx = false;
    bool dct = false;
    bool down = false;
    bool poly = false;
    bool inplaceC = false;
    bool inplaceF = false, inplaceI = false;
    struct Four { bool on = false; int n1 = 0, n2 = 0, tka = 1, tkb = 1;
                  StagePlan p1{}, p2{}; size_t ldsA = 0, ldsB = 0; int thrA = 64, thrB = 64; };
    Four fourF, fourI;
    Four colF, colI;
    uint32_t bzL[4] = {0, 0, 0, 0};
    bool bz = false;
    bool odd = false;
    bool exact = false;
    uint32_t align = 0;
    bool view = false;
    uint32_t viewL[2] = {0, 0};
    bool mirror = false;
    int ncols = 0;
    int pairs_per_strip = 6;
};

int plan_check(const PlanRequest& rq, PlanGeometry& G);
int plan_geometry_columns(PlanGeometry& G, const DeviceFacts& dev);
int plan_jit_factor(const PlanGeometry& G, int* DD);
int plan_geometry_finish(PlanGeometry& G, const DeviceFacts& dev, const fftup_jit::Choice* jit);

int strip_length(const PlanGeometry& G, const DeviceFacts& dev, int fused_threads);
std::string wisdom_device_key(const PlanGeometry& G, const DeviceFacts& dev);
int lane_count();

bool is_smooth(uint32_t n);
StagePlan make_stage_plan(uint32_t n);
std::vector<int> stage_radices(const StagePlan& p);
uint32_t scaled_length(float upscale, uint32_t n);
void column_guard(float upscale, uint32_t uH, int* zly, int* zry);
int jit_factor(float upscale, uint32_t W, uint32_t H, uint32_t uW, uint32_t uH, int zly, int zry, int* DD);
int check_view(const char* who, const fftup_view* v, uint32_t uW, uint32_t uH);
float view_factor(const fftup_view& v, uint32_t uW, uint32_t uH);

struct AlignGeometry {
    uint32_t W = 0, H = 0, precision = 0, nx = 0, ny = 0, d = 1, crop_x = 0, crop_y = 0, kappa = 32, band_kx = 0, band_ky = 0;
    uint32_t Kx = 0, Ky = 0, max_batch = 16;
    float band = 0.5f;
};
int align_geometry(const fftup_align_config& c, AlignGeometry& G);
float const_via_percent_f(double v, bool half);
```

Baseline: 15940 frames/s.

## Add columns-first path: real column FFT, row transforms fused into c2r sharpen

Adds a columns-first schedule for the tuned 2048x1024 fused path. The column FFT and zero-pad inverse run directly on the real planar image into a real buffer, and a small kernel computes a Nyquist correction from a cotangent table. The fused kernel then does both the forward and inverse row transforms plus sharpen, so the separate row R2C launch and its complex spectrum round trip go away. In exchange the fused kernel carries an extra forward row FFT per strip, a correction term and new per-lane buffers. Tap frames fall back to the classic path by replaying the last input.

```diff
diff --git a/vkresample_amd/csrc/fftup_info.hip b/vkresample_amd/csrc/fftup_info.hip
--- a/vkresample_amd/csrc/fftup_info.hip
+++ b/vkresample_amd/csrc/fftup_info.hip
@@ -105,6 +105,7 @@
         s += "; column tiles of " + std::to_string(P->TK);
     }
     if (P->u8out) s += "; fused 8-bit RGB store";
+    if (P->columns_first) s += "; columns first: column pass on the real image, both row transforms in the fused kernel (two launches per frame)";
     snprintf(buf, buflen, "%s", s.c_str());
     return FFTUP_OK;
 }
@@ -140,6 +141,14 @@
         info->kernel_min_bytes[2] = P->fused ? S2 * halo + o : S2 + R;
         info->kernel_min_bytes[3] = P->fused ? 0.0 : R + o;
     }
+    if (P->columns_first) {
+        const double Yr = C * W * H * 4.0, halo = (double)(P->pairs_per_strip + 1) / P->pairs_per_strip;
+        info->kernel_alg_bytes[1] += info->kernel_alg_bytes[0];
+        info->kernel_alg_bytes[0] = 0.0;
+        info->kernel_min_bytes[0] = 0.0;
+        info->kernel_min_bytes[1] = in + Yr;
+        info->kernel_min_bytes[2] = (in + Yr) * halo + o;
+    }
     if (P->dct) {
         const double D1 = C * W * H * 4.0, D2 = C * W * uH * 4.0;
         info->alg_bytes_per_frame = in + 2 * D1 + 2 * D2 + 2 * R + o;
@@ -156,6 +165,7 @@
     snprintf(info->kernel_names[1], 64, is_dct ? (P->down ? "dct_col_crop_idct" : "dct_col_pad_idct") : crop_cols ? "col_fwd_crop_inv" : "col_fwd_pad_inv");
     snprintf(info->kernel_names[2], 64, is_dct ? "idct_row" : P->fused ? "row_c2r_sharpen" : (is_cplx ? "row_c2c_inv" : "row_c2r"));
     snprintf(info->kernel_names[3], 64, P->fused ? "-" : "sharpen");
+    if (P->columns_first) snprintf(info->kernel_names[0], 64, "-");
     if (P->family == fftup_plan::Family::odd)
         for (int i = 0; i < 3; i++) strncat(info->kernel_names[i], "_odd", 63 - strlen(info->kernel_names[i]));
     if (P->family == fftup_plan::Family::view) {
diff --git a/vkresample_amd/csrc/fftup_launch.hip b/vkresample_amd/csrc/fftup_launch.hip
--- a/vkresample_amd/csrc/fftup_launch.hip
+++ b/vkresample_amd/csrc/fftup_launch.hip
@@ -39,15 +39,21 @@
 
 struct ViewTables { int kmax; const float2 *pre, *post, *bhat; };
 struct Frame { hipStream_t st; float2 *S1, *S2; void *R, *T4; const void* in; long in_row, in_plane; int kind; void* out;
-               int ncols, NT; float upsq; ViewTables vx, vy; };
+               int ncols, NT; float upsq; ViewTables vx, vy;
+               float *Yr, *nyqN, *nyqCorr; bool classic; };
 static Frame resolve(const fftup_plan* P, const FrameRun& r)
 {
     const fftup_plan::Lane& l = P->lanes[r.lane];
     Frame f{l.stream, l.S1, l.S2, l.R, l.T4, P->in_planar[r.in_slot], (long)P->W, (long)P->in_plane_stride, P->in_kind[r.in_slot], r.out,
-            P->ncols, P->NT, P->upsq, {P->vx.kmax, P->vx.pre, P->vx.post, P->vx.bhat}, {P->vy.kmax, P->vy.pre, P->vy.post, P->vy.bhat}};
-    if (r.in) { f.in = r.in->in; f.in_row = r.in->in_row; f.in_plane = r.in->kind == 2 ? 0 : r.in->in_plane; f.kind = r.in->kind; }
+            P->ncols, P->NT, P->upsq, {P->vx.kmax, P->vx.pre, P->vx.post, P->vx.bhat}, {P->vy.kmax, P->vy.pre, P->vy.post, P->vy.bhat},
+            l.Yr, l.nyqN, l.nyqCorr, false};
+    if (r.in) { f.in = r.in->in; f.in_row = r.in->in_row; f.in_plane = r.in->kind == 2 ? 0 : r.in->in_plane; f.kind = r.in->kind; f.classic = true; }
     else if (f.kind == 2) { f.in = P->in_u8[r.in_slot]; f.in_row = 3l * P->W; f.in_plane = 0; }
     return f;
+}
+static bool columns_first_frame(const fftup_plan* P, const Frame& f)
+{
+    return P->columns_first && !f.classic && f.kind == 1 && f.in_row % 2 == 0 && f.in_plane % 2 == 0 && ((uintptr_t)f.in & 7) == 0;
 }
 template <class Q> static void set_in(const Frame& f, Q& q) { q.in = f.in; q.in_row_stride = f.in_row; q.in_plane_stride = f.in_plane; }
 static bool runs(Pass pass, Pass k) { return pass == Pass::all || pass == k; }
@@ -240,6 +246,24 @@
     case 1024: return fused_kernel_of<FusedPlanPow2<1024>>(P);
     case 2048: return fused_kernel_of<FusedPlanPow2<2048>>(P);
     default: return fused_kernel_of<FusedPlanPow2<4096>>(P);
+    }
+}
+static Kern<ColRealParams> cf_col_kernel(const fftup_plan* P)
+{
+    switch (P->H) {
+    case 256: return kern(k_col_real_v<256>, 128, 8192);
+    case 512: return kern(k_col_real_v<512>, 256, 16384);
+    default: return kern(k_col_real_v<1024>, 512, 32768);
+    }
+}
+static Kern<NyqRowParams> cf_nyq_kernel(const fftup_plan* P) { return kern(k_col_nyq_row, 256, sizeof(float) * ((size_t)P->W + P->W / 2)); }
+template <class PL> static Kern<FusedParams> cf_fused_kernel_of() { return kern(k_c2r_sharpen_g<PL, false, TUNED_TK, 2, 4, false, 1, true>, PL::T, FusedGLds<PL>::TOTAL); }
+static Kern<FusedParams> cf_fused_kernel(const fftup_plan* P)
+{
+    switch (P->uW) {
+    case 1024: return cf_fused_kernel_of<FusedPlanPow2<1024>>();
+    case 2048: return cf_fused_kernel_of<FusedPlanPow2<2048>>();
+    default: return cf_fused_kernel_of<FusedPlanPow2<4096>>();
     }
 }
 
@@ -280,7 +304,10 @@
         if (P->mirror) { for (int kind : {1, 2}) allow(mirror_row_kernel(P, kind)); allow(mirror_col_kernel(P)); allow(mirror_c2r_kernel(P)); }
         else { for (int kind : {1, 2}) allow(odd_row_kernel(P, kind)); allow(view_col_kernel(P)); allow(view_c2r_kernel(P)); }
         break;
-    case Family::tuned: allow(tuned_col_kernel(P)); allow(fused_kernel(P)); break;
+    case Family::tuned:
+        allow(tuned_col_kernel(P)); allow(fused_kernel(P));
+        if (P->columns_first) { allow(cf_col_kernel(P)); allow(cf_nyq_kernel(P)); allow(cf_fused_kernel(P)); }
+        break;
     case Family::mixed_aot: allow(mixed_col_kernel(P)); allow(mixed_c2r_kernel(P)); allow(fused_kernel(P)); break;
     case Family::mixed_jit:
         if (P->jit->choice.row_kind == 2) for (int kind : {1, 2}) allow(generic_row_kernel(P, kind));
@@ -632,6 +659,22 @@
 
 static int launch_frame_tuned(const fftup_plan* P, const Frame& f, Pass pass)
 {
+    if (columns_first_frame(P, f) && pass != Pass::presharpen_tap) {
+        if (runs(pass, Pass::columns)) {
+            ColRealParams p{};
+            p.in = (const float*)f.in; p.in_row_stride = f.in_row; p.in_plane_stride = f.in_plane;
+            p.Yr = f.Yr; p.N = f.nyqN; p.twH = P->twH; p.twUH = P->twUH; p.W = (int)P->W;
+            launch(cf_col_kernel(P), dim3(P->W / 8, 3), f.st, p);
+            const NyqRowParams q{f.nyqN, P->nyqCot, f.nyqCorr, (int)P->W, 1.0f / (float)P->H};
+            launch(cf_nyq_kernel(P), dim3(P->W / 256, 3), f.st, q);
+        }
+        if (runs(pass, Pass::inverse)) {
+            FusedParams p = fused_params(P, f);
+            p.img = (const float*)f.in; p.img_row = f.in_row; p.img_plane = f.in_plane; p.Yr = f.Yr; p.corr = f.nyqCorr;
+            launch(cf_fused_kernel(P), dim3(fused_grid(P, p.pairs_per_strip)), f.st, p);
+        }
+        return frame_status();
+    }
     if (runs(pass, Pass::rows)) {
         RowR2CTParams p{};
         p.S1 = f.S1; p.tw = P->twW; p.H = (int)P->H; p.NT = P->NT;
@@ -790,6 +833,17 @@
         if (P->family != Family::view || (size_t)r.lane >= P->vtabs.size() || !P->vtabs[r.lane].pre[0]) return fail(FFTUP_E_INVALID_ARG, "a frame with a view of its own: not a view plan, or its lane has no tables");
         frame_view(P, r.lane, *r.view, r.shift, f);
     }
+    if (P->columns_first) {
+        fftup_plan::LastInput& li = P->cf_last[r.lane];
+        if (tap && li.kind) {
+            Frame g = f;
+            g.in = li.in; g.in_row = li.in_row; g.in_plane = li.in_plane; g.kind = li.kind; g.classic = true;
+            if (int rc2 = launch_family(P, g, Pass::rows)) return rc2;
+            if (int rc2 = launch_family(P, g, Pass::columns)) return rc2;
+        } else if (!tap && runs(r.pass, Pass::inverse)) {
+            li = columns_first_frame(P, f) ? fftup_plan::LastInput{f.in, f.in_row, f.in_plane, f.kind} : fftup_plan::LastInput{};
+        }
+    }
     const int rc = launch_family(P, f, r.pass);
     if (rc && r.view) P->vtabs[r.lane].span[0] = P->vtabs[r.lane].span[1] = 0;
     if (tap || runs(r.pass, Pass::inverse)) { P->last_lane = r.lane; P->R_valid = !(P->fused && !tap); }
diff --git a/vkresample_amd/csrc/fftup_plan.hip b/vkresample_amd/csrc/fftup_plan.hip
--- a/vkresample_amd/csrc/fftup_plan.hip
+++ b/vkresample_amd/csrc/fftup_plan.hip
@@ -216,6 +216,13 @@
         if (int rc = make_rotations(P, &P->rotW, P->W)) return rc;
         if (int rc = make_rotations(P, &P->rotH, P->H)) return rc;
     }
+    if (P->columns_first) {
+        std::vector<float> h(P->W / 2);
+        for (uint32_t j = 0; j < P->W / 2; j++) h[j] = (float)(2.0 / ((double)P->W * (double)P->H) / std::tan(M_PI * (double)(2 * j + 1) / (double)P->W));
+        float2* d = nullptr;
+        if (int rc = upload_table(P, &d, h)) return rc;
+        P->nyqCot = (const float*)d;
+    }
     if (P->dct) {
         float2** const rot[4] = {&P->rotW, &P->rotH, &P->rotUW, &P->rotUH};
         for (int i = 0; i < 4; i++)
@@ -259,6 +266,7 @@
 {
     P->nlanes = lane_count();
     P->lanes.resize(P->nlanes);
+    P->cf_last.assign(P->nlanes, {});
     const size_t t4_bytes = P->csz * 3 * std::max(std::max(P->fourF.on ? (size_t)P->W * P->H : 0, P->fourI.on ? (size_t)P->uW * P->uH : 0),
                                                   P->colI.on ? (size_t)P->ncols * P->uH : 0);
     for (int l = 0; l < P->nlanes; l++) {
@@ -271,6 +279,11 @@
             if (int rc = dev_alloc(P, &lane.R, P->r_bytes)) return rc;
         if (t4_bytes)
             if (int rc = dev_alloc(P, &lane.T4, t4_bytes)) return rc;
+        if (P->columns_first) {
+            if (int rc = dev_alloc(P, (void**)&lane.Yr, sizeof(float) * 3 * (size_t)P->W * P->H)) return rc;
+            if (int rc = dev_alloc(P, (void**)&lane.nyqN, sizeof(float) * 3 * (size_t)P->W)) return rc;
+            if (int rc = dev_alloc(P, (void**)&lane.nyqCorr, sizeof(float) * 3 * ((size_t)P->W + 4))) return rc;
+        }
     }
     return FFTUP_OK;
 }
diff --git a/vkresample_amd/csrc/kernels_dswap.hpp b/vkresample_amd/csrc/kernels_dswap.hpp
--- a/vkresample_amd/csrc/kernels_dswap.hpp
+++ b/vkresample_amd/csrc/kernels_dswap.hpp
@@ -129,28 +129,18 @@
     }
 }
 
-template <int TK, int H = 1024>
-__global__ void __launch_bounds__(H / 2, kColWaves) k_col_v(ColTParams p)
-{
-    static_assert(TK == 4, "four columns of H/8 threads: lane bits 0-1 = column, bits 2-5 and the wave = pp");
-    static_assert(H == 1024 || H == 512 || H == 256, "8, 4 or 2 waves");
-    constexpr int WV = H / 128, Q = 8 / WV, T = 64 * WV;
-    extern __shared__ __attribute__((aligned(128))) char smem[];
-    const unsigned zbase = lds_addr(smem);
-    const int tid = threadIdx.x;
+template <int H, bool REAL>
+__device__ __forceinline__ void col_v_transforms(float2 (&v)[8], unsigned zbase, int tid, const float2* __restrict__ twH,
+                                                 const float2* __restrict__ twUH, float2& nyq)
+{
+    constexpr int WV = H / 128, Q = 8 / WV;
     const unsigned w = (unsigned)tid >> 6, l = (unsigned)tid & 63u;
-    const int col = tid & 3, pp = tid >> 2;
-    const int tile = blockIdx.x, c = blockIdx.y;
-    const bool valid = tile * TK + col <= p.W / 2;
-    const float2* src = p.S1 + ((long)c * p.NT + tile) * H * TK;
+    const int pp = tid >> 2;
+    struct { const float2 *twH, *twUH; } p = {twH, twUH};
     const int wu = __builtin_amdgcn_readfirstlane((int)w);
     const int s1 = (int)(l >> 3), lb2 = (int)((l >> 2) & 1u), hh = (int)(l >> 2);
     const int kk = Q * wu + s1 / WV + 8 * (s1 % WV);
     const int kt = kk + 32 * WV * lb2;
-    float2 v[8];
-    stamp_begin(1, c);
-#pragma unroll
-    for (int i = 0; i < 8; i++) v[i] = valid ? src[tid + T * i] : make_float2(0.f, 0.f);
     float2 ta[Q][WV - 1];
 #pragma unroll
     for (int b = 0; b < Q; b++)
@@ -182,6 +172,10 @@
             v[r] = make_float2(s0.x, s0.y); v[r + 4] = make_float2(s1_.x, s1_.y);
         }
     }
+    if constexpr (REAL) {
+        nyq = v[4];
+        if (tid < 4) v[4] = make_float2(0.f, 0.f);
+    }
     {
         const float2 t1 = cmul_tw(tph, twid<-1>(rot32<1>())), t2 = cmul_tw(tph, twid<-1>(rot32<2>())), t3 = cmul_tw(tph, twid<-1>(rot32<3>()));
         const float2 tt[4] = {tph, t1, t2, t3};
@@ -221,6 +215,27 @@
     else wave_exchange_q<WV, false>(v, zbase, w, l);
     twiddle_powers<8>(v, twid<-1>(p.twH[pp]));
     bfly8_pk<-1>(v);
+}
+
+template <int TK, int H = 1024>
+__global__ void __launch_bounds__(H / 2, kColWaves) k_col_v(ColTParams p)
+{
+    static_assert(TK == 4, "four columns of H/8 threads: lane bits 0-1 = column, bits 2-5 and the wave = pp");
+    static_assert(H == 1024 || H == 512 || H == 256, "8, 4 or 2 waves");
+    constexpr int WV = H / 128, T = 64 * WV;
+    extern __shared__ __attribute__((aligned(128))) char smem[];
+    const unsigned zbase = lds_addr(smem);
+    const int tid = threadIdx.x;
+    const int col = tid & 3;
+    const int tile = blockIdx.x, c = blockIdx.y;
+    const bool valid = tile * TK + col <= p.W / 2;
+    const float2* src = p.S1 + ((long)c * p.NT + tile) * H * TK;
+    float2 v[8];
+    stamp_begin(1, c);
+#pragma unroll
+    for (int i = 0; i < 8; i++) v[i] = valid ? src[tid + T * i] : make_float2(0.f, 0.f);
+    float2 nyq;
+    col_v_transforms<H, false>(v, zbase, tid, p.twH, p.twUH, nyq);
     float2* dst = p.S2 + ((long)c * p.NT + tile) * H * TK;
     constexpr float inv = 1.0f / (float)H;
     if (valid) {
@@ -230,5 +245,78 @@
     stamp_end(1, c);
 }
 
-
-}
+struct ColRealParams {
+    const float* in;
+    long in_row_stride, in_plane_stride;
+    float* Yr;
+    float* N;
+    const float2 *twH, *twUH;
+    int W;
+};
+template <int H>
+__global__ void __launch_bounds__(H / 2, kColWaves) k_col_real_v(ColRealParams p)
+{
+    static_assert(H == 1024 || H == 512 || H == 256, "8, 4 or 2 waves");
+    extern __shared__ __attribute__((aligned(128))) char smem[];
+    const unsigned zbase = lds_addr(smem);
+    const int tid = threadIdx.x;
+    const int col = tid & 3, pp = tid >> 2;
+    const int b = blockIdx.x, c = blockIdx.y;
+    const int tile = (b & ~15) + 2 * (b & 7) + ((b >> 3) & 1);
+    const long x0 = 8 * tile + 2 * col;
+    const float* src = p.in + (long)c * p.in_plane_stride + (long)pp * p.in_row_stride + x0;
+    float2 v[8];
+    stamp_begin(1, c);
+#pragma unroll
+    for (int i = 0; i < 8; i++) v[i] = *(const float2*)(src + (long)(H / 8) * i * p.in_row_stride);
+    float2 nyq;
+    col_v_transforms<H, true>(v, zbase, tid, p.twH, p.twUH, nyq);
+    if (tid < 4) *(float2*)(p.N + (long)c * p.W + x0) = nyq;
+    float* dst = p.Yr + ((long)c * H + pp) * p.W + x0;
+    constexpr float inv = 1.0f / (float)H;
+#pragma unroll
+    for (int i = 0; i < 8; i++) spec_store8((float2*)(dst + (long)(H / 8) * i * p.W), cscale(v[i], inv));
+    stamp_end(1, c);
+}
+
+struct NyqRowParams {
+    const float* N;
+    const float* cot;
+    float* corr;
+    int W;
+    float invH;
+};
+__global__ void __launch_bounds__(256) k_col_nyq_row(NyqRowParams p)
+{
+    extern __shared__ __attribute__((aligned(16))) float nyq_lds[];
+    float* sN = nyq_lds;
+    float* sC = nyq_lds + p.W;
+    const int tid = threadIdx.x, c = blockIdx.y, W = p.W;
+    for (int i = tid; i < W; i += 256) sN[i] = p.N[(long)c * W + i];
+    for (int i = tid; i < W / 2; i += 256) sC[i] = p.cot[i];
+    __syncthreads();
+    const int x = blockIdx.x * 256 + tid;
+    float acc0 = 0.f, acc1 = 0.f;
+    for (int j = 0; j < W / 2; j += 2) {
+        acc0 = fmaf(sN[(x - 2 * j - 1) & (W - 1)], sC[j], acc0);
+        acc1 = fmaf(sN[(x - 2 * j - 3) & (W - 1)], sC[j + 1], acc1);
+    }
+    float* out = p.corr + (long)c * (W + 4);
+    out[x] = acc0 + acc1;
+    if (blockIdx.x == 0) {
+        float s0 = 0.f, sw = 0.f;
+        for (int i = tid; i < W; i += 256) { s0 += sN[i]; sw += (i & 1) ? -sN[i] : sN[i]; }
+#pragma unroll
+        for (int o = 32; o > 0; o >>= 1) { s0 += __shfl_down(s0, o); sw += __shfl_down(sw, o); }
+        __syncthreads();
+        if ((tid & 63) == 0) { sC[2 * (tid >> 6)] = s0; sC[2 * (tid >> 6) + 1] = sw; }
+        __syncthreads();
+        if (tid == 0) {
+            out[W] = (sC[0] + sC[2] + sC[4] + sC[6]) * p.invH;
+            out[W + 1] = (sC[1] + sC[3] + sC[5] + sC[7]) * p.invH;
+        }
+    }
+}
+
+
+}
diff --git a/vkresample_amd/csrc/kernels_pow2.hpp b/vkresample_amd/csrc/kernels_pow2.hpp
--- a/vkresample_amd/csrc/kernels_pow2.hpp
+++ b/vkresample_amd/csrc/kernels_pow2.hpp
@@ -307,6 +307,23 @@
         __syncthreads();
         reg_gather<N, E, 1>(v, b, p, 0);
         reg_fft_pp<N, E, DIR, S + 1>(v, c, z, p, tws, p0);
+    }
+}
+
+template <int N, int E, int DIR, int S = 0>
+__device__ __forceinline__ void reg_fft_pp_lds(float2 (&v)[E], float2* __restrict__ c, float2* __restrict__ z, int p, const TwSet<N, E, 8>& tws)
+{
+    constexpr int Ns = stage_ns(N, S, 8);
+    constexpr int R = stage_radix(N, Ns, 8);
+    constexpr int NSC = num_stages(N, 8);
+    static_assert(E % R == 0, "radix must divide the per-thread point count");
+    reg_butterflies<N, E, R, Ns, DIR>(v, tws.w[S > 0 ? S - 1 : 0]);
+    float2* __restrict__ b = ((NSC - 1 - S) % 2 == 0) ? c : z;
+    reg_scatter<N, E, R, Ns, 1>(v, b, p, 0);
+    __syncthreads();
+    if constexpr (Ns * R != N) {
+        reg_gather<N, E, 1>(v, b, p, 0);
+        reg_fft_pp_lds<N, E, DIR, S + 1>(v, c, z, p, tws);
     }
 }
 
@@ -720,6 +737,10 @@
     int pairs_per_strip;
     float upsq, coef;
     int u8_wrap;
+    const float* img;
+    long img_row, img_plane;
+    const float* Yr;
+    const float* corr;
 };
 __device__ __forceinline__ float absmin1(float x)
 {
@@ -1184,10 +1205,12 @@
     }
 }
 
-template <class PL, bool HALF, int TK, int U = 2, int D = 2 * U, bool OUT_U8 = false, int DD = 1>
+template <class PL, bool HALF, int TK, int U = 2, int D = 2 * U, bool OUT_U8 = false, int DD = 1, bool CF = false>
 __global__ void __launch_bounds__(PL::T, PL::WPE) k_c2r_sharpen_g(FusedParams p)
 {
     constexpr int UW = PL::UW, T = PL::T, R0 = PL::R0, NB0 = PL::NB0, NI = R0 * DD / D, KH = UW * DD / D;
+    static_assert(!CF || (U == 2 && D == 4 && DD == 1 && !HALF && !OUT_U8 && R0 == 8 && PL::VN == 8 && PL::NBUF == 3 && NB0 == T && T % 128 == 0),
+                  "columns first: u = 2 power-of-two plans on fp32 planes");
     static_assert((R0 * DD) % D == 0, "the first radix must be a multiple of 2u");
     static_assert(UW % 4 == 0, "the sharpen passes work on quads of pixels");
     constexpr int EOUT = PL::EOUT, SOUT = PL::SOUT, VN = PL::VN;
@@ -1251,7 +1274,7 @@
         constexpr bool MS = PL::MIRROR_SHARE;
         struct In { float2 a[NI], am[NI], b[NI], bm[NI]; float lka, lkb; };
         unsigned ko[NI], kom[NI];
-        const int jj = PL::first_index(lt);
+        const int jj = CF ? lt : PL::first_index(lt);
         {
 #pragma unroll
             for (int m = 0; m < NI; m++) { ko[m] = koff(jj + NB0 * m); kom[m] = koff(KH - jj - NB0 * m); }
@@ -1305,26 +1328,88 @@
                 }
             }
         };
+        constexpr int WF = UW / 2, TF = T / 2;
+        typedef const __attribute__((address_space(1))) float* gfptr_t;
+        float pf[CF ? 16 : 1];
+        float cHq[CF ? 8 : 1];
+        float s0H = 0.f, sWH = 0.f;
+        gptr_t cf_img = nullptr, cf_yr = nullptr;
+        if constexpr (CF) {
+            cf_img = (gptr_t)(p.img + (long)c * p.img_plane);
+            cf_yr = (gptr_t)(p.Yr + (long)c * (uH / 2) * WF);
+            const float* cr = p.corr + (long)c * (WF + 4);
+#pragma unroll
+            for (int i = 0; i < 8; i++) cHq[i] = cr[(lt & (TF - 1)) + TF * i];
+            s0H = cr[WF]; sWH = cr[WF + 1];
+        }
+        auto cf_rowbase = [&](int y) -> gptr_t {
+            const long off = (y & 1) ? (long)(y >> 1) * WF : (long)(y >> 1) * p.img_row;
+            gptr_t r = ((y & 1) ? cf_yr : cf_img) + off * (long)sizeof(float);
+            asm("" : "+s"(r));
+            return r;
+        };
+        auto cf_sign = [](int y) -> float { return (y & 1) ? ((y & 2) ? -1.f : 1.f) : 0.f; };
+        auto cf_prefetch = [&](int i0) __attribute__((always_inline)) {
+            if constexpr (CF) {
+                const int hw = __builtin_amdgcn_readfirstlane(lt / TF);
+                const int a = a0 + 2 * min(i0 + hw, npairs - 1);
+                const gptr_t ra = cf_rowbase(min(a, uH - 1)), rb = cf_rowbase(min(a + 1, uH - 1));
+                unsigned qo = (unsigned)(lt & (TF - 1)) * (unsigned)sizeof(float);
+                asm("" : "+v"(qo));
+#pragma unroll
+                for (int i = 0; i < 8; i++) {
+                    pf[i] = *(gfptr_t)(ra + qo + (unsigned)(TF * i * sizeof(float)));
+                    pf[8 + i] = *(gfptr_t)(rb + qo + (unsigned)(TF * i * sizeof(float)));
+                }
+            }
+        };
+        auto cf_settle = [&]() {
+            if constexpr (CF) {
+                __builtin_amdgcn_s_waitcnt(0x0F70);
+#pragma unroll
+                for (int i = 0; i < 16; i += 4) asm volatile("" : "+v"(pf[i]), "+v"(pf[i + 1]), "+v"(pf[i + 2]), "+v"(pf[i + 3]));
+            }
+        };
         if (need_corner) {
             float part = 0.f;
-            for (int kk = lt + 1; kk <= KH; kk += T) part += S2at(kk, rs).x;
+            if constexpr (CF) {
+                const gptr_t rr = cf_rowbase(rs);
+                const float* cr = p.corr + (long)c * (WF + 4);
+                const float sg = cf_sign(rs);
+                for (int x = lt; x < WF; x += T) {
+                    const float b = fmaf(sg, cr[x], *(gfptr_t)(rr + (unsigned)x * (unsigned)sizeof(float)));
+                    part += b;
+                    if (x == 0) part += (float)WF * b;
+                }
+                if (lt & 1) part = -part;
+            } else {
+                for (int kk = lt + 1; kk <= KH; kk += T) part += S2at(kk, rs).x;
+            }
 #pragma unroll
             for (int o = 32; o > 0; o >>= 1) part += __shfl_down(part, o);
             if ((lt & 63) == 0) red[lt >> 6] = part;
-            if (lt == T - 1) {
-                float2 d = S2at(0, rs), dp = S2at(0, rs ^ 1);
-                red[16] = (rs & 1) ? d.x + dp.y : d.x - dp.y;
-            }
-        }
-        In in = load_pair(0);
-        settle(in);
-        share(in);
+            if constexpr (!CF) {
+                if (lt == T - 1) {
+                    float2 d = S2at(0, rs), dp = S2at(0, rs ^ 1);
+                    red[16] = (rs & 1) ? d.x + dp.y : d.x - dp.y;
+                }
+            }
+        }
+        In in;
+        if constexpr (CF) {
+            cf_prefetch(0);
+            cf_settle();
+        } else {
+            in = load_pair(0);
+            settle(in);
+            share(in);
+        }
         __syncthreads();
         float corner = 0.f;
         if (need_corner) {
             float sum = 0.f;
             for (int w2 = 0; w2 < (T + 63) / 64; w2++) sum += red[w2];
-            corner = (red[16] + 2.0f * sum) * inv;
+            corner = CF ? sum * inv : (red[16] + 2.0f * sum) * inv;
         }
         if constexpr (PL::NBUF == 3) __syncthreads();
         float pn0 = 0.f, pn1 = 0.f;
@@ -1346,6 +1431,55 @@
             float2 v[VN];
 #pragma unroll
             for (int m = 0; m < VN; m++) v[m] = make_float2(0.f, 0.f);
+            if constexpr (CF) {
+                float2 zc[4];
+                if ((s & 1) == 0) {
+                    const int hw = __builtin_amdgcn_readfirstlane(lt / TF), q = lt & (TF - 1);
+                    const int ah = a0 + 2 * min(s + hw, npairs - 1);
+                    const float ca = cf_sign(min(ah, uH - 1)), cb = cf_sign(min(ah + 1, uH - 1));
+                    float2 w[8];
+#pragma unroll
+                    for (int i = 0; i < 8; i++) w[i] = make_float2(fmaf(ca, cHq[i], pf[i]), fmaf(cb, cHq[i], pf[8 + i]));
+                    TwSet<WF, 8> twf;
+                    constexpr int SF = num_stages(WF, 8);
+                    auto fwd_tw = [&](auto sc) __attribute__((always_inline)) {
+                        constexpr int st = decltype(sc)::value, Ns = stage_ns(WF, st, 8);
+                        float2 t = tws.t.w[st - 1];
+                        if constexpr (stage_radix(WF, Ns, 8) != stage_radix(UW, Ns, 8)) t = cmul_tw(t, t);
+                        if constexpr (Ns > TF) { if (hw) t = cmul_tw(t, twid<-1>(rot16<2>())); }
+                        asm volatile("" : "+v"(t.x), "+v"(t.y));
+                        twf.w[st - 1] = t;
+                    };
+                    fwd_tw(std::integral_constant<int, 1>{});
+                    if constexpr (SF > 2) fwd_tw(std::integral_constant<int, 2>{});
+                    if constexpr (SF > 3) fwd_tw(std::integral_constant<int, 3>{});
+                    static_assert(SF <= 4, "at most four forward stages");
+                    float2* ch = (float2*)smem + hw * lswz_size(WF);
+                    float2* zh = (float2*)(smem + L::ZOFF) + hw * lswz_size(WF);
+                    if constexpr (SF % 2 == 1) __syncthreads();
+                    reg_fft_pp_lds<WF, 8, +1>(w, ch, zh, q, twf);
+                    const unsigned z0 = lds_addr(smem) + 8u * (unsigned)lswz(lt), z1 = z0 + 8u * (unsigned)lswz_size(WF);
+#pragma unroll
+                    for (int m = 0; m < 4; m++) zc[m] = lds_get(z0, lswz_c(T * m));
+#pragma unroll
+                    for (int m = 0; m < 4; m++) { const float2 t = lds_get(z1, lswz_c(T * m)); pf[2 * m] = t.x; pf[2 * m + 1] = t.y; }
+                } else {
+#pragma unroll
+                    for (int m = 0; m < 4; m++) zc[m] = make_float2(pf[2 * m], pf[2 * m + 1]);
+                }
+                v[0] = zc[0]; v[1] = zc[1]; v[R0 - 2] = zc[2]; v[R0 - 1] = zc[3];
+                if (lt == 0) {
+                    const int ya = min(a, uH - 1), yb = min(a + 1, uH - 1);
+                    const float la = (ya & 1) ? 0.f : ((ya & 2) ? s0H : -s0H), lb = (yb & 1) ? 0.f : ((yb & 2) ? s0H : -s0H);
+                    const float dx = -cf_sign(yb) * sWH, dy = cf_sign(ya) * sWH;
+                    v[0] = make_float2(zc[0].x + la, zc[0].y + lb);
+                    v[NI] = make_float2(zc[2].x + dx, zc[2].y + dy);
+                    v[R0 - NI] = make_float2(zc[2].x - dx, zc[2].y - dy);
+                }
+                if ((s & 1) == 1 && s + 1 < npairs) cf_prefetch(s + 1);
+                PL::fft(v, buf, (float2*)(smem + L::ZOFF), lt, tws, jj);
+                cf_settle();
+            } else {
 #pragma unroll
             for (int m = 0; m < NI; m++) {
                 v[m] = cadd_i(in.a[m], in.b[m]);
@@ -1360,6 +1494,7 @@
             PL::fft(v, buf, (float2*)(smem + L::ZOFF), lt, tws, jj);
             settle(in);
             share(in);
+            }
             if constexpr (HALF) {
                 const h2v up2 = h2_splat(p.upsq), one2 = h2_splat(1.0f);
                 if (SOUT == T || lt < SOUT) {
diff --git a/vkresample_amd/csrc/plan.hpp b/vkresample_amd/csrc/plan.hpp
--- a/vkresample_amd/csrc/plan.hpp
+++ b/vkresample_amd/csrc/plan.hpp
@@ -66,7 +66,8 @@
     std::vector<uint8_t*> in_u8;
     std::vector<int> in_kind;
     struct Lane { hipStream_t stream = nullptr; float2 *S1 = nullptr, *S2 = nullptr; void* R = nullptr; hipEvent_t done = nullptr;
-                  void* T4 = nullptr; };
+                  void* T4 = nullptr;
+                  float *Yr = nullptr, *nyqN = nullptr, *nyqCorr = nullptr; };
     std::vector<Lane> lanes;
     int nlanes = 1;
     int last_lane = 0;
@@ -87,6 +88,9 @@
     uint32_t* png_crc_shift = nullptr;
     bool png_foreign_collector = false;
     float2 *twW = nullptr, *twH = nullptr, *twUW = nullptr, *twUH = nullptr;
+    const float* nyqCot = nullptr;
+    struct LastInput { const void* in = nullptr; long in_row = 0, in_plane = 0; int kind = 0; };
+    std::vector<LastInput> cf_last;
     float2 *rotW = nullptr, *rotH = nullptr, *rotUW = nullptr, *rotUH = nullptr;
     uint64_t device_bytes = 0;
     size_t r_bytes = 0;
diff --git a/vkresample_amd/csrc/plan_rules.cpp b/vkresample_amd/csrc/plan_rules.cpp
--- a/vkresample_amd/csrc/plan_rules.cpp
+++ b/vkresample_amd/csrc/plan_rules.cpp
@@ -509,6 +509,9 @@
     if (int rc = choose_family(G)) return rc;
     G.fused = (G.tuned || G.mixed) && !(G.cfg.flags & FFTUP_FLAG_UNFUSED_SHARPEN);
     G.u8out = G.fused && (G.cfg.flags & FFTUP_FLAG_FUSE_U8_STORE);
+    const bool cf_can = G.tuned && G.fused && !G.u8out && !G.half && !G.dbl && G.U == 2 && !(G.cfg.flags & FFTUP_FLAG_FUSE_U8_LOAD);
+    G.columns_first = cf_can && frames_overlap(G) && G.W == 2048 && G.H == 1024;
+    if (const char* e = fftup_jit::experiment("columns_first")) G.columns_first = cf_can && atoi(e) != 0;
     G.pairs_per_strip = strip_length(G, dev, fused_threads(G, jit));
     G.NT = (G.ncols + G.TK - 1) / G.TK;
     if (int rc = row_buffers(G, dev.lds_bytes)) return rc;
diff --git a/vkresample_amd/csrc/plan_rules.hpp b/vkresample_amd/csrc/plan_rules.hpp
--- a/vkresample_amd/csrc/plan_rules.hpp
+++ b/vkresample_amd/csrc/plan_rules.hpp
@@ -40,6 +40,7 @@
     bool tuned = false;
     bool fused = false;
     bool u8out = false;
+    bool columns_first = false;
     int mixed = 0;
     int U = 2;
     bool cplx = false;
```

After: 14420 frames/s. 0.905x the previous value.
